# TortillasAlfred/NeuralBarkCalculator

Hardware: AMD Instinct MI355X
Metric: 1024x1024 images/sec (whole node) + per-pixel label match vs CPU ref (higher is better)
Workload: dtype f16x2

## Files before the change

### include/nbc.h

```cpp
#ifndef NBC_H
#define NBC_H

#include <stddef.h>
#include <stdint.h>

#ifdef __cplusplus
extern "C" {
#endif

typedef struct nbc_ctx nbc_ctx;

enum {
  NBC_OK = 0,
  NBC_ERR_INVALID = -1,
  NBC_ERR_KEYS = -2,
  NBC_ERR_HIP = -3,
  NBC_ERR_STATE = -4,
  NBC_ERR_NOMEM = -5
};

enum {
  NBC_PREC_FP32 = 0,
  NBC_PREC_BF16 = 1,
  NBC_PREC_F16X2 = 2
};

enum {
  NBC_PACK_ROW_CLAMPED = 1,
  NBC_PACK_SCALE_RANGE = 2
};

enum {
  NBC_ARCH_FCN_RESNET50 = 0,
  NBC_ARCH_DEEPLABV3_RESNET50 = 1,
  NBC_ARCH_FCN_EFFICIENTNET_B0 = 16,
  NBC_ARCH_DEEPLABV3_EFFICIENTNET_B0 = 24
};

enum {
  NBC_BN_RUNNING = 0,
  NBC_BN_PER_IMAGE = 1
};

enum {
  NBC_IN_F32_NCHW = 0,
  NBC_IN_U8_NHWC = 1
};

enum {
  NBC_LABEL_U8 = 0,
  NBC_LABEL_I64 = 1
};

typedef struct {
  const char* name;
  const void* data;
  int64_t shape[4];
  int32_t ndim;
  int32_t dtype;
} nbc_tensor;

typedef struct {
  char name[64];
  char bn[64];
  int32_t cin, cout, k, stride, pad, dil;
  int32_t relu, bias, residual;
} nbc_conv_desc;

typedef struct {
  int32_t kind;
  int32_t pad_before;
  int32_t pad_after;
  int32_t act;
  int32_t cin_pad, cout_pad;
  int32_t block;
  int32_t in_swish;
  float eps;
} nbc_conv_ext;

typedef struct {
  char name[64];
  char kernel[32];
  float ms;
  int32_t calls;
  double flops;
  double bytes;
  int32_t kh, kw;
  int32_t cout;
  int32_t launches;
} nbc_op_record;

const char* nbc_last_error(void);
const char* nbc_version(void);

int nbc_num_convs(void);
int nbc_conv_info(int index, nbc_conv_desc* out);
int nbc_num_state_keys(void);
int nbc_state_key(int index, const char** name, int64_t shape[4], int32_t* ndim, int32_t* dtype);
int nbc_arch_num_convs(int arch);
int nbc_arch_conv_info(int arch, int index, nbc_conv_desc* out);
int nbc_arch_num_state_keys(int arch);
int nbc_arch_state_key(int arch, int index, const char** name, int64_t shape[4], int32_t* ndim, int32_t* dtype);
int nbc_arch_of_state_dict(const nbc_tensor* tensors, int n);
int nbc_lowres_size(int H, int W, int* h, int* w);
int nbc_arch_lowres_size(int arch, int H, int W, int* h, int* w);
int nbc_arch_conv_ext(int arch, int index, nbc_conv_ext* out);

int nbc_split_f16x2(const float* x, size_t n, uint16_t* h0, uint16_t* h1);

size_t nbc_packed_weights_bytes(int precision);
int nbc_pack_weights(const nbc_tensor* tensors, int n, int precision, void* blob, size_t blob_bytes);
int nbc_packed_weights_flags(const void* blob, size_t blob_bytes, int precision);
size_t nbc_arch_packed_weights_bytes(int precision, int arch);
int nbc_pack_weights_arch(const nbc_tensor* tensors, int n, int precision, int arch, void* blob, size_t blob_bytes);
int nbc_packed_weights_flags_arch(const void* blob, size_t blob_bytes, int precision, int arch);
int nbc_packed_weights_arch(const void* blob, size_t blob_bytes, int precision);

size_t nbc_arch_bn_affine_floats(int arch);
int nbc_pack_bn_affine(const nbc_tensor* tensors, int n, int arch, float* out, size_t count);

int nbc_create(nbc_ctx** out, int hip_device);
int nbc_destroy(nbc_ctx* ctx);
int nbc_attach_weights(nbc_ctx* ctx, const void* dev_blob, size_t bytes, int precision);
int nbc_attach_weights_arch(nbc_ctx* ctx, const void* dev_blob, size_t bytes, int precision, int arch);
int nbc_load_weights(nbc_ctx* ctx, const nbc_tensor* tensors, int n, int precision);
int nbc_load_weights_arch(nbc_ctx* ctx, const nbc_tensor* tensors, int n, int precision, int arch);
int nbc_weights_flags(nbc_ctx* ctx);
int nbc_activation_exponent(nbc_ctx* ctx, const char* name, int32_t* exponent);
int nbc_bcast_weights(nbc_ctx* ctx, void* rccl_comm, int root, int precision, void* hip_stream);
int nbc_attach_bn_affine(nbc_ctx* ctx, const float* dev_affine, size_t count);
int nbc_set_bn_statistics(nbc_ctx* ctx, int mode);
int nbc_set_normalization(nbc_ctx* ctx, const float mean[3], const float std[3]);
int nbc_reserve(nbc_ctx* ctx, int N, int H, int W);

int nbc_forward(nbc_ctx* ctx, const void* x_dev, int x_dtype, int N, int H, int W,
                float* logits_lowres_dev, float* logits_full_dev,
                void* labels_dev, int labels_dtype, int64_t* counts_dev,
                int exclude_nodes, void* hip_stream);

int nbc_upsample_argmax(nbc_ctx* ctx, const float* logits_lowres_dev, int N, int h, int w, int H, int W,
                        float* logits_full_dev, void* labels_dev, int labels_dtype,
                        int64_t* counts_dev, int exclude_nodes, void* hip_stream);

int nbc_remove_small_zones(nbc_ctx* ctx, void* labels_dev, int labels_dtype, int N, int H, int W, int min_pixels,
                           int exclude_nodes, int64_t* counts_dev, void* hip_stream);

int nbc_confusion(const void* labels_dev, int labels_dtype, const uint8_t* target_dev,
                  int N, int H, int W, int64_t* conf_dev, void* hip_stream);

int nbc_image_moments(const uint8_t* x_dev, int N, int H, int W, uint64_t* moments_dev, void* hip_stream);

int nbc_target_counts(const uint8_t* target_dev, int N, int H, int W, int64_t* counts_dev, void* hip_stream);

size_t nbc_lovasz_workspace_bytes(int N, int H, int W);
int nbc_lovasz_softmax(const float* logits_full_dev, const uint8_t* target_dev, int N, int H, int W,
                       void* workspace_dev, size_t workspace_bytes, double* terms_dev, int64_t* fg_counts_dev,
                       void* hip_stream);

size_t nbc_pixel_ce_workspace_bytes(int N, int H, int W);
int nbc_pixel_cross_entropy(const float* logits_full_dev, const uint8_t* target_dev, int N, int H, int W,
                            void* workspace_dev, size_t workspace_bytes, double* sums_dev, int64_t* counts_dev,
                            void* hip_stream);


int nbc_dropout_mask(uint64_t seed, uint64_t image_id, int draw, double p, uint64_t first_element, size_t count,
                     uint8_t* keep_host);
size_t nbc_dropout_workspace_bytes(int N, int H, int W, int draws_per_pass);
int nbc_dropout_draws(nbc_ctx* ctx, int N, int H, int W, const uint64_t* image_ids_host, double p, uint64_t seed,
                      int first_draw, int draws, int min_pixels, int exclude_nodes, float* logits_lowres_dev,
                      int64_t* counts_dev, void* workspace_dev, size_t workspace_bytes, void* hip_stream);

int nbc_resize_cubic_u8(nbc_ctx* ctx, const uint8_t* src_dev, int H, int W, float* dst_dev, int out_h, int out_w,
                        void* hip_stream);
int nbc_preprocess_u8(nbc_ctx* ctx, const uint8_t* src_dev, int H, int W, uint8_t* dst_u8_dev, int32_t* row_lit_dev,
                      int out_h, int out_w, void* hip_stream);

int nbc_set_conv_tile(nbc_ctx* ctx, int tile);

int nbc_autotune(nbc_ctx* ctx, const void* x_dev, int x_dtype, int N, int H, int W, int reps, int objective,
                 void* hip_stream);
int nbc_get_plan_tiles(nbc_ctx* ctx, int32_t* tiles, int capacity);
int nbc_default_conv_tile(int M, int Cout, int K, int precision);
int nbc_set_plan_tiles(nbc_ctx* ctx, const int32_t* tiles, int n);

int nbc_nonfinite_seen(nbc_ctx* ctx, int reset);
int nbc_nonfinite_peek_async(nbc_ctx* ctx, uint32_t* host_dst, void* hip_stream);

int nbc_set_keep_activations(nbc_ctx* ctx, int on);
int nbc_activation_peaks(nbc_ctx* ctx, float* peaks_host, int capacity);
int nbc_read_activation(nbc_ctx* ctx, const char* name, float* dst_host, size_t capacity,
                        int64_t shape[4]);
int nbc_set_profiling(nbc_ctx* ctx, int on);
int nbc_num_op_records(nbc_ctx* ctx);
int nbc_get_op_record(nbc_ctx* ctx, int index, nbc_op_record* out);

#ifdef __cplusplus
}
#endif
#endif
```

### neuralbarkcalculator_amd/_lib.py

```python
from __future__ import annotations

import ctypes as C
import os
from typing import Optional

_PKG = os.path.dirname(os.path.abspath(__file__))
LIB_PATH = os.path.join(_PKG, "libnbc_hip.so")

NBC_OK = 0
NBC_ERR_INVALID, NBC_ERR_KEYS, NBC_ERR_HIP, NBC_ERR_STATE, NBC_ERR_NOMEM = -1, -2, -3, -4, -5
PREC_FP32, PREC_BF16, PREC_F16X2 = 0, 1, 2
IN_F32_NCHW, IN_U8_NHWC = 0, 1
LABEL_U8, LABEL_I64 = 0, 1
PACK_ROW_CLAMPED, PACK_SCALE_RANGE = 1, 2
ARCH_FCN_RESNET50, ARCH_DEEPLABV3_RESNET50 = 0, 1
ARCH_FCN_EFFICIENTNET_B0, ARCH_DEEPLABV3_EFFICIENTNET_B0 = 16, 24
BN_RUNNING, BN_PER_IMAGE = 0, 1


class NbcTensor(C.Structure):
    _fields_ = [("name", C.c_char_p), ("data", C.c_void_p), ("shape", C.c_int64 * 4),
                ("ndim", C.c_int32), ("dtype", C.c_int32)]


class NbcConvDesc(C.Structure):
    _fields_ = [("name", C.c_char * 64), ("bn", C.c_char * 64),
                ("cin", C.c_int32), ("cout", C.c_int32), ("k", C.c_int32), ("stride", C.c_int32),
                ("pad", C.c_int32), ("dil", C.c_int32),
                ("relu", C.c_int32), ("bias", C.c_int32), ("residual", C.c_int32)]


class NbcConvExt(C.Structure):
    _fields_ = [("kind", C.c_int32), ("pad_before", C.c_int32), ("pad_after", C.c_int32), ("act", C.c_int32),
                ("cin_pad", C.c_int32), ("cout_pad", C.c_int32), ("block", C.c_int32), ("in_swish", C.c_int32),
                ("eps", C.c_float)]


class NbcOpRecord(C.Structure):
    _fields_ = [("name", C.c_char * 64), ("kernel", C.c_char * 32), ("ms", C.c_float), ("calls", C.c_int32),
                ("flops", C.c_double), ("bytes", C.c_double), ("kh", C.c_int32), ("kw", C.c_int32),
                ("cout", C.c_int32), ("launches", C.c_int32)]


SIGNATURES = {
    "nbc_last_error": (C.c_char_p, []),
    "nbc_version": (C.c_char_p, []),
    "nbc_num_convs": (C.c_int, []),
    "nbc_conv_info": (C.c_int, [C.c_int, C.POINTER(NbcConvDesc)]),
    "nbc_num_state_keys": (C.c_int, []),
    "nbc_state_key": (C.c_int, [C.c_int, C.POINTER(C.c_char_p), C.POINTER(C.c_int64 * 4),
                                C.POINTER(C.c_int32), C.POINTER(C.c_int32)]),
    "nbc_arch_num_convs": (C.c_int, [C.c_int]),
    "nbc_arch_conv_info": (C.c_int, [C.c_int, C.c_int, C.POINTER(NbcConvDesc)]),
    "nbc_arch_num_state_keys": (C.c_int, [C.c_int]),
    "nbc_arch_state_key": (C.c_int, [C.c_int, C.c_int, C.POINTER(C.c_char_p), C.POINTER(C.c_int64 * 4),
                                     C.POINTER(C.c_int32), C.POINTER(C.c_int32)]),
    "nbc_arch_of_state_dict": (C.c_int, [C.POINTER(NbcTensor), C.c_int]),
    "nbc_lowres_size": (C.c_int, [C.c_int, C.c_int, C.POINTER(C.c_int), C.POINTER(C.c_int)]),
    "nbc_arch_lowres_size": (C.c_int, [C.c_int, C.c_int, C.c_int, C.POINTER(C.c_int), C.POINTER(C.c_int)]),
    "nbc_arch_conv_ext": (C.c_int, [C.c_int, C.c_int, C.POINTER(NbcConvExt)]),
    "nbc_packed_weights_bytes": (C.c_size_t, [C.c_int]),
    "nbc_split_f16x2": (C.c_int, [C.c_void_p, C.c_size_t, C.c_void_p, C.c_void_p]),
    "nbc_pack_weights": (C.c_int, [C.POINTER(NbcTensor), C.c_int, C.c_int, C.c_void_p, C.c_size_t]),
    "nbc_packed_weights_flags": (C.c_int, [C.c_void_p, C.c_size_t, C.c_int]),
    "nbc_arch_packed_weights_bytes": (C.c_size_t, [C.c_int, C.c_int]),
    "nbc_pack_weights_arch": (C.c_int, [C.POINTER(NbcTensor), C.c_int, C.c_int, C.c_int, C.c_void_p, C.c_size_t]),
    "nbc_packed_weights_flags_arch": (C.c_int, [C.c_void_p, C.c_size_t, C.c_int, C.c_int]),
    "nbc_packed_weights_arch": (C.c_int, [C.c_void_p, C.c_size_t, C.c_int]),
    "nbc_arch_bn_affine_floats": (C.c_size_t, [C.c_int]),
    "nbc_pack_bn_affine": (C.c_int, [C.POINTER(NbcTensor), C.c_int, C.c_int, C.c_void_p, C.c_size_t]),
    "nbc_attach_bn_affine": (C.c_int, [C.c_void_p, C.c_void_p, C.c_size_t]),
    "nbc_set_bn_statistics": (C.c_int, [C.c_void_p, C.c_int]),
    "nbc_weights_flags": (C.c_int, [C.c_void_p]),
    "nbc_activation_exponent": (C.c_int, [C.c_void_p, C.c_char_p, C.POINTER(C.c_int32)]),
    "nbc_create": (C.c_int, [C.POINTER(C.c_void_p), C.c_int]),
    "nbc_destroy": (C.c_int, [C.c_void_p]),
    "nbc_attach_weights": (C.c_int, [C.c_void_p, C.c_void_p, C.c_size_t, C.c_int]),
    "nbc_load_weights": (C.c_int, [C.c_void_p, C.POINTER(NbcTensor), C.c_int, C.c_int]),
    "nbc_attach_weights_arch": (C.c_int, [C.c_void_p, C.c_void_p, C.c_size_t, C.c_int, C.c_int]),
    "nbc_load_weights_arch": (C.c_int, [C.c_void_p, C.POINTER(NbcTensor), C.c_int, C.c_int, C.c_int]),
    "nbc_set_normalization": (C.c_int, [C.c_void_p, C.POINTER(C.c_float), C.POINTER(C.c_float)]),
    "nbc_reserve": (C.c_int, [C.c_void_p, C.c_int, C.c_int, C.c_int]),
    "nbc_nonfinite_seen": (C.c_int, [C.c_void_p, C.c_int]),
    "nbc_nonfinite_peek_async": (C.c_int, [C.c_void_p, C.c_void_p, C.c_void_p]),
    "nbc_forward": (C.c_int, [C.c_void_p, C.c_void_p, C.c_int, C.c_int, C.c_int, C.c_int,
                              C.c_void_p, C.c_void_p, C.c_void_p, C.c_int, C.c_void_p, C.c_int,
                              C.c_void_p]),
    "nbc_upsample_argmax": (C.c_int, [C.c_void_p, C.c_void_p, C.c_int, C.c_int, C.c_int, C.c_int, C.c_int,
                                      C.c_void_p, C.c_void_p, C.c_int, C.c_void_p, C.c_int, C.c_void_p]),
    "nbc_remove_small_zones": (C.c_int, [C.c_void_p, C.c_void_p, C.c_int, C.c_int, C.c_int, C.c_int, C.c_int, C.c_int,
                                         C.c_void_p, C.c_void_p]),
    "nbc_confusion": (C.c_int, [C.c_void_p, C.c_int, C.c_void_p, C.c_int, C.c_int, C.c_int, C.c_void_p, C.c_void_p]),
    "nbc_image_moments": (C.c_int, [C.c_void_p, C.c_int, C.c_int, C.c_int, C.c_void_p, C.c_void_p]),
    "nbc_target_counts": (C.c_int, [C.c_void_p, C.c_int, C.c_int, C.c_int, C.c_void_p, C.c_void_p]),
    "nbc_lovasz_workspace_bytes": (C.c_size_t, [C.c_int, C.c_int, C.c_int]),
    "nbc_lovasz_softmax": (C.c_int, [C.c_void_p, C.c_void_p, C.c_int, C.c_int, C.c_int, C.c_void_p, C.c_size_t, C.c_void_p,
                                     C.c_void_p, C.c_void_p]),
    "nbc_pixel_ce_workspace_bytes": (C.c_size_t, [C.c_int, C.c_int, C.c_int]),
    "nbc_pixel_cross_entropy": (C.c_int, [C.c_void_p, C.c_void_p, C.c_int, C.c_int, C.c_int, C.c_void_p, C.c_size_t, C.c_void_p,
                                          C.c_void_p, C.c_void_p]),
    "nbc_dropout_mask": (C.c_int, [C.c_uint64, C.c_uint64, C.c_int, C.c_double, C.c_uint64, C.c_size_t, C.c_void_p]),
    "nbc_dropout_workspace_bytes": (C.c_size_t, [C.c_int, C.c_int, C.c_int, C.c_int]),
    "nbc_dropout_draws": (C.c_int, [C.c_void_p, C.c_int, C.c_int, C.c_int, C.c_void_p, C.c_double, C.c_uint64, C.c_int, C.c_int,
                                    C.c_int, C.c_int, C.c_void_p, C.c_void_p, C.c_void_p, C.c_size_t, C.c_void_p]),
    "nbc_resize_cubic_u8": (C.c_int, [C.c_void_p, C.c_void_p, C.c_int, C.c_int, C.c_void_p, C.c_int, C.c_int, C.c_void_p]),
    "nbc_preprocess_u8": (C.c_int, [C.c_void_p, C.c_void_p, C.c_int, C.c_int, C.c_void_p, C.c_void_p, C.c_int, C.c_int,
                                    C.c_void_p]),
    "nbc_autotune": (C.c_int, [C.c_void_p, C.c_void_p, C.c_int, C.c_int, C.c_int, C.c_int, C.c_int, C.c_int,
                               C.c_void_p]),
    "nbc_get_plan_tiles": (C.c_int, [C.c_void_p, C.POINTER(C.c_int32), C.c_int]),
    "nbc_set_plan_tiles": (C.c_int, [C.c_void_p, C.POINTER(C.c_int32), C.c_int]),
    "nbc_default_conv_tile": (C.c_int, [C.c_int, C.c_int, C.c_int, C.c_int]),
    "nbc_bcast_weights": (C.c_int, [C.c_void_p, C.c_void_p, C.c_int, C.c_int, C.c_void_p]),
    "nbc_set_conv_tile": (C.c_int, [C.c_void_p, C.c_int]),
    "nbc_set_keep_activations": (C.c_int, [C.c_void_p, C.c_int]),
    "nbc_activation_peaks": (C.c_int, [C.c_void_p, C.POINTER(C.c_float), C.c_int]),
    "nbc_read_activation": (C.c_int, [C.c_void_p, C.c_char_p, C.c_void_p, C.c_size_t,
                                      C.POINTER(C.c_int64 * 4)]),
    "nbc_set_profiling": (C.c_int, [C.c_void_p, C.c_int]),
    "nbc_num_op_records": (C.c_int, [C.c_void_p]),
    "nbc_get_op_record": (C.c_int, [C.c_void_p, C.c_int, C.POINTER(NbcOpRecord)]),
}

_lib: Optional[C.CDLL] = None


def load() -> C.CDLL:
    global _lib
    if _lib is not None:
        return _lib
    if not os.path.exists(LIB_PATH):
        raise RuntimeError(
            f"{LIB_PATH} is missing: the HIP library is the only implementation of this path. "
            "Build it with `python -m neuralbarkcalculator_amd.build` (needs hipcc).")
    lib = C.CDLL(LIB_PATH)
    for name, (res, args) in SIGNATURES.items():
        fn = getattr(lib, name)
        fn.restype = res
        fn.argtypes = args
    _lib = lib
    return lib


def last_error() -> str:
    return load().nbc_last_error().decode("utf-8", "replace")


def check(rc: int, what: str = "") -> None:
    if rc == NBC_OK:
        return
    msg = last_error()
    raise RuntimeError(f"{what + ': ' if what else ''}{msg} (nbc error {rc})")
```

### neuralbarkcalculator_amd/build.py

```python
from __future__ import annotations

import os
import shutil
import subprocess
import sys
from concurrent.futures import ThreadPoolExecutor

PKG = os.path.dirname(os.path.abspath(__file__))
CSRC = os.path.join(PKG, "csrc")
OBJ = os.path.join(CSRC, "_obj")
LIB = os.path.join(PKG, "libnbc_hip.so")
SOURCES = ["nbc_net.cpp", "nbc_plan.cpp", "conv_igemm_dma.hip", "conv3x3_rows.hip", "pointwise.hip", "small_zones.hip", "nbc_api.hip", "confusion.hip",
           "aspp.hip", "bn_stats.hip", "efficientnet.hip", "lovasz.hip", "dataset_stats.hip", "pixel_ce.hip", "dropout_head.hip"]
ARCH = "gfx950"


def _hipcc() -> str:
    exe = shutil.which("hipcc") or "/opt/rocm/bin/hipcc"
    if not os.path.exists(exe):
        raise RuntimeError("hipcc not found: cannot build libnbc_hip.so")
    return exe


def _deps_newer(target: str, deps) -> bool:
    if not os.path.exists(target):
        return True
    t = os.path.getmtime(target)
    return any(os.path.getmtime(d) > t for d in deps)


def build(force: bool = False, verbose: bool = True) -> str:
    os.makedirs(OBJ, exist_ok=True)
    hipcc = _hipcc()
    headers = [os.path.join(CSRC, f) for f in os.listdir(CSRC) if f.endswith(".hpp")]
    headers.append(os.path.join(os.path.dirname(PKG), "include", "nbc.h"))
    common = ["-O3", "-std=c++17", "-fPIC", f"--offload-arch={ARCH}", "-Wall", "-Wno-unused-function"]

    def compile_one(src: str) -> str:
        path = os.path.join(CSRC, src)
        obj = os.path.join(OBJ, src + ".o")
        if force or _deps_newer(obj, [path] + headers):
            cmd = [hipcc] + common + (["-x", "hip"] if src.endswith(".hip") else ["-ffp-contract=off"]) + ["-c", path, "-o", obj]
            if verbose:
                print("[nbc build]", " ".join(cmd), flush=True)
            subprocess.run(cmd, check=True)
        return obj

    with ThreadPoolExecutor(max_workers=6) as ex:
        objs = list(ex.map(compile_one, SOURCES))
    if force or _deps_newer(LIB, objs):
        cmd = [hipcc, "-shared", "-fPIC", f"--offload-arch={ARCH}", "-o", LIB] + objs
        if verbose:
            print("[nbc build]", " ".join(cmd), flush=True)
        subprocess.run(cmd, check=True)
    return LIB


if __name__ == "__main__":
    print(build(force="--force" in sys.argv))
```

### neuralbarkcalculator_amd/csrc/conv_igemm_dma.hip

```cpp
#include <atomic>

#include "nbc_kernels.hpp"
#include "split16.hpp"

namespace nbc {
namespace {

typedef __attribute__((ext_vector_type(8))) __bf16 bf16x8;
typedef __attribute__((ext_vector_type(16))) float f32x16;
typedef __attribute__((ext_vector_type(4))) float f32x4;

__device__ __forceinline__ int lds_off(int row, int chunk) {
  return row * 128 + ((chunk ^ ((row >> 1) & 7)) << 4);
}
__device__ __forceinline__ float bf16_bits_to_f32(unsigned short b) {
  return __builtin_bit_cast(float, (unsigned)b << 16);
}
__device__ __forceinline__ unsigned short f32_to_bf16_bits(float f) {
  __bf16 b = (__bf16)f;
  return __builtin_bit_cast(unsigned short, b);
}

__device__ __forceinline__ void dma16(const void* gsrc, unsigned lds_base) {
  unsigned keep;
  asm volatile(
      "s_mov_b32 %0, m0\n\t"
      "s_mov_b32 m0, %2\n\t"
      "s_nop 0\n\t"
      "global_load_lds_dwordx4 %1, off\n\t"
      "s_mov_b32 m0, %0"
      : "=&s"(keep)
      : "v"(gsrc), "s"(lds_base)
      : "memory");
}

typedef __amdgpu_buffer_rsrc_t rsrc_t;
constexpr unsigned kOutOfRange = 0x80000000u;
__device__ __forceinline__ void dma16_buf(unsigned voff, rsrc_t rsrc, unsigned lds_base, unsigned soff) {
  asm volatile(
      "s_mov_b32 m0, %2\n\t"
      "s_nop 0\n\t"
      "buffer_load_dwordx4 %0, %1, %3 offen lds"
      :
      : "v"(voff), "s"(rsrc), "s"(lds_base), "s"(soff)
      : "memory");
}

#ifdef NBC_STAMPS
#define NBC_STAMP(i)                                                                                   \
  do {                                                                                                 \
    if (p.stamps && threadIdx.x == 0) p.stamps[(size_t)blockIdx.x * 64 + (i)] = __builtin_amdgcn_s_memrealtime(); \
  } while (0)
#define NBC_STAMP_CLK(i)                                                                               \
  do {                                                                                                 \
    if (p.stamps && threadIdx.x == 0) p.stamps[(size_t)blockIdx.x * 64 + (i)] = __builtin_amdgcn_s_memtime(); \
  } while (0)
#define NBC_WAIT_COUNTERS() unsigned long long st_vm = 0, st_bar = 0
#define NBC_WAIT_BEGIN() const unsigned long long st0 = __builtin_amdgcn_s_memtime()
#define NBC_WAIT_MID() const unsigned long long st1 = __builtin_amdgcn_s_memtime()
#define NBC_WAIT_END(count)                                                                            \
  do {                                                                                                 \
    if (count) { st_vm += st1 - st0; st_bar += __builtin_amdgcn_s_memtime() - st1; }                  \
  } while (0)
#define NBC_STAMP_WAVE_WAITS()                                                                         \
  do {                                                                                                 \
    if (p.stamps && lane == 0) { p.stamps[(size_t)blockIdx.x * 64 + 16 + wave] = st_vm; p.stamps[(size_t)blockIdx.x * 64 + 32 + wave] = st_bar; } \
  } while (0)
#define NBC_STAMP_BLOCK_END()                                                                          \
  do {                                                                                                 \
    NBC_STAMP(5);                                                          \
    wait_vmcnt<0>();                                                                                   \
    NBC_STAMP(6);                                                    \
    if (p.stamps && threadIdx.x == 0)                       \
      p.stamps[(size_t)blockIdx.x * 64 + 7] =                                                          \
          ((unsigned long long)__builtin_amdgcn_s_getreg(20 | (31 << 11)) << 32) | __builtin_amdgcn_s_getreg(4 | (31 << 11)); \
  } while (0)
#else
#define NBC_STAMP(i) do { } while (0)
#define NBC_STAMP_CLK(i) do { } while (0)
#define NBC_WAIT_COUNTERS()
#define NBC_WAIT_BEGIN()
#define NBC_WAIT_MID()
#define NBC_WAIT_END(count) do { } while (0)
#define NBC_STAMP_WAVE_WAITS() do { } while (0)
#define NBC_STAMP_BLOCK_END() do { } while (0)
#endif

template <int N>
__device__ __forceinline__ void wait_vmcnt() {
  asm volatile("s_waitcnt vmcnt(%0)" ::"n"(N) : "memory");
}

constexpr int ring_bytes(int prec, int wm, int wn, int mt, int nt, int s) {
  const int ring = s * (wm * mt * 32 + wn * nt * 32) * 128;
  const int scratch = wm * wn * 32 * (nt * 32 * 4 + 16);
  return ring > scratch ? ring : scratch;
}
constexpr int min_waves_per_simd(int prec, int wm, int wn, int mt, int nt, int s) {
  return (wm * wn >= 8 && (wm * wn >= 16 || ring_bytes(prec, wm, wn, mt, nt, s) + 2048 <= 80 * 1024)) ? 4 : 2;
}

constexpr int kVarDefault = 0;
constexpr int kVarBf16Mfma32 = 1;
constexpr int kVarLoaderWaves = 8;

typedef unsigned nt_u32x4 __attribute__((ext_vector_type(4)));
constexpr int loader_waves(int var) { return var == kVarLoaderWaves ? 4 : 0; }
template <int PREC, int WM, int WN, int MT, int NT, int S, bool STEM, int VAR, bool BIGW>
__global__ __launch_bounds__((WM * WN + loader_waves(VAR)) * 64, VAR == kVarLoaderWaves ? (WM * WN + loader_waves(VAR)) / 4 : min_waves_per_simd(PREC, WM, WN, MT, NT, S)) void conv_dma_kernel(const ConvArgs p) {
  extern __shared__ __attribute__((aligned(16))) unsigned char smem[];
  constexpr int EB = PREC == 1 ? 2 : 4;
  constexpr bool X2 = (PREC == 2);
  constexpr int CW = WM * WN;
  constexpr int LW = loader_waves(VAR);
  constexpr bool SPEC = LW > 0;
  constexpr int THREADS = (SPEC ? LW : CW) * 64;
  constexpr int BM = WM * MT * 32;
  constexpr int BN = WN * NT * 32;
  constexpr int A_BYTES = BM * 128;
  constexpr int B_BYTES = BN * 128;
  constexpr int STAGE_BYTES = A_BYTES + B_BYTES;
  constexpr int TABLE_OFF = ring_bytes(PREC, WM, WN, MT, NT, S);
  constexpr int ROWS_PER_PASS = THREADS / 8;
  constexpr int A_PASSES = BM / ROWS_PER_PASS;
  constexpr int B_PASSES = BN / ROWS_PER_PASS;
  constexpr int L = A_PASSES + B_PASSES;
  static_assert(BM % ROWS_PER_PASS == 0 && BN % ROWS_PER_PASS == 0, "tile rows must fill whole passes");
  static_assert(S >= 2 && S <= 4, "2..4 LDS stages");

  const int tid = threadIdx.x;
  const int lane = tid & 63;
  const int wave = __builtin_amdgcn_readfirstlane(tid >> 6);
  const bool is_loader = SPEC && wave >= CW;
  const bool loads = !SPEC || is_loader, computes = !SPEC || !is_loader;
  constexpr bool STAGGER = (PREC == 2) && !STEM && CW >= 8 && (LW > 0 || MT * NT >= 4);
  const bool late_half = STAGGER && wave >= CW / 2 && wave < CW;
  NBC_STAMP(0);

  const int tiles_n = p.Co / BN;
  const int tiles_m = (p.M + BM - 1) / BM;
  const int nblk = tiles_m * tiles_n;
  int bid = blockIdx.x;
  {
    const int q = nblk >> 3, rr = nblk & 7, xcd = bid & 7;
    bid = (xcd < rr ? xcd * (q + 1) : rr * (q + 1) + (xcd - rr) * q) + (bid >> 3);
  }
  int tile_n = bid % tiles_n, tile_m = bid / tiles_n;
  if (BIGW && (tiles_n & 1) == 0 && (tiles_m & 3) == 0) {
    const int xcd = blockIdx.x & 7, li = blockIdx.x >> 3, rows = tiles_m >> 2, hc = tiles_n >> 1;
    tile_m = (xcd >> 1) * rows + li / hc;
    tile_n = (xcd & 1) * hc + li % hc;
  }
  const int m0 = tile_m * BM;
  const int n0 = tile_n * BN;

  const int ltid = SPEC ? ((tid - CW * 64) & (THREADS - 1)) : tid;
  const int ps = ltid & 7;
  const int lr = ltid >> 3;
  const rsrc_t xrsrc = __builtin_amdgcn_make_buffer_rsrc(const_cast<void*>(p.x), 0, p.x_bytes, 0x00020000);
  const rsrc_t wrsrc = __builtin_amdgcn_make_buffer_rsrc(const_cast<void*>(p.w), 0, p.w_bytes, 0x00020000);
  const int pix_bytes = p.Ci * EB;
  const unsigned wrow_bytes = (unsigned)p.ksteps * 128u;

  int a_iy0[A_PASSES], a_ix0[A_PASSES], a_img[A_PASSES], a_coff[A_PASSES];
  {
    const int hw = p.Ho * p.Wo;
#pragma unroll
    for (int i = 0; i < A_PASSES; ++i) {
      const int row = lr + ROWS_PER_PASS * i;
      const int m = m0 + row;
      a_coff[i] = (ps ^ ((row >> 1) & 7)) * 16;
      if (m < p.M) {
        const int img = p.N == 1 ? 0 : (p.hw_shift >= 0 ? (m >> p.hw_shift) : m / hw);
        const int rem = m - img * hw;
        const int oy = p.wo_shift >= 0 ? (rem >> p.wo_shift) : rem / p.Wo;
        const int ox = rem - oy * p.Wo;
        a_iy0[i] = oy * p.stride - p.pad;
        a_ix0[i] = ox * p.stride - p.pad;
        a_img[i] = img * p.Hi * p.Wi;
      } else {
        a_iy0[i] = -(1 << 24);
        a_ix0[i] = 0;
        a_img[i] = 0;
      }
    }
  }
  unsigned w_off[B_PASSES];
#pragma unroll
  for (int i = 0; i < B_PASSES; ++i) {
    const int row = lr + ROWS_PER_PASS * i;
    w_off[i] = (unsigned)(n0 + row) * wrow_bytes + (unsigned)(ps ^ ((row >> 1) & 7)) * 16u;
  }

  typedef __attribute__((address_space(3))) unsigned char lds_u8;
  const unsigned smem_base = (unsigned)(size_t)(lds_u8*)smem;
  const unsigned wave_off = (unsigned)(SPEC ? ((wave - CW) & (LW - 1)) : wave) * 1024u;
  const int cblocks = STEM ? 1 : pix_bytes / 128;
  int ld_kh = 0, ld_kw = 0, ld_cb = 0;
  int st_kh = 0, st_kw = 0;
  if constexpr (STEM) st_kw = a_coff[0] >> 4;

  unsigned a_off[A_PASSES];
  auto set_tap = [&](int kh, int kw) __attribute__((always_inline)) {
    const int dy = kh * p.dil, dx = kw * p.dil;
#pragma unroll
    for (int i = 0; i < A_PASSES; ++i) {
      const int iy = a_iy0[i] + dy, ix = a_ix0[i] + dx;
      const bool ok = (unsigned)iy < (unsigned)p.Hi && (unsigned)ix < (unsigned)p.Wi;
      const unsigned off = (unsigned)(a_img[i] + iy * p.Wi + ix) * (unsigned)pix_bytes + (unsigned)a_coff[i];
      a_off[i] = ok ? off : kOutOfRange;
    }
  };
  if constexpr (!STEM) set_tap(0, 0);

  auto issue_one = [&](int d, int t, unsigned sa) __attribute__((always_inline)) {
    if (d < A_PASSES) {
      const int i = d;
      if constexpr (!STEM) {
        dma16_buf(a_off[i], xrsrc, sa + (unsigned)(ROWS_PER_PASS * 128 * i), (unsigned)ld_cb * 128u);
      } else {
        const int iy = a_iy0[i] + st_kh * p.dil, ix = a_ix0[i] + st_kw * p.dil;
        const bool ok = st_kw < p.KW && (unsigned)iy < (unsigned)p.Hi && (unsigned)ix < (unsigned)p.Wi;
        const unsigned off = (unsigned)(a_img[i] + iy * p.Wi + ix) * 16u;
        dma16_buf(ok ? off : kOutOfRange, xrsrc, sa + (unsigned)(ROWS_PER_PASS * 128 * i), 0u);
      }
    } else {
      const int i = d - A_PASSES;
      dma16_buf(w_off[i], wrsrc, sa + (unsigned)(A_BYTES + ROWS_PER_PASS * 128 * i), (unsigned)t * 128u);
    }
  };
  auto issue_part = [&](int part, int t, int stage) __attribute__((always_inline)) {
    const unsigned sa = smem_base + (unsigned)stage * STAGE_BYTES + wave_off;
#pragma unroll
    for (int d = 0; d < L; ++d)
      if (d * 4 / L == part) issue_one(d, t, sa);
    if constexpr (STEM) {
      if (part == 3) ++st_kh;
    }
    if constexpr (!STEM) {
      if (part == 3) {
        if (++ld_cb == cblocks) {
          ld_cb = 0;
          if (++ld_kw == p.KW) { ld_kw = 0; ++ld_kh; }
          if (ld_kh < p.KH) set_tap(ld_kh, ld_kw);
        }
      }
    }
  };
  auto issue_step = [&](int t, int stage) __attribute__((always_inline)) {
#pragma unroll
    for (int part = 0; part < 4; ++part) issue_part(part, t, stage);
  };

  const int r = lane & 31, h = lane >> 5;
  const int wm = wave % WM, wn = wave / WM;
  constexpr bool M16 = (PREC == 1 && VAR == kVarDefault) || X2;
  constexpr int MT16 = 2 * MT, NT16 = 2 * NT;
  const int r16 = lane & 15, q16 = lane >> 4;
  constexpr bool F32 = (PREC == 0);
  constexpr bool PREFETCH = F32 && S >= 3;
  f32x16 acc[M16 ? 1 : NT][M16 ? 1 : MT];
  f32x16 accI[F32 ? NT : 1][F32 ? MT : 1];
  f32x4 acc16[M16 ? NT16 : 1][M16 ? MT16 : 1];
  f32x4 accI2[X2 ? NT16 : 1][X2 ? MT16 : 1];
  if constexpr (X2) {
#pragma unroll
    for (int j = 0; j < NT16; ++j)
#pragma unroll
      for (int i = 0; i < MT16; ++i)
#pragma unroll
        for (int e = 0; e < 4; ++e) accI2[j][i][e] = 0.f;
  }
  if constexpr (M16) {
#pragma unroll
    for (int j = 0; j < NT16; ++j)
#pragma unroll
      for (int i = 0; i < MT16; ++i)
#pragma unroll
        for (int e = 0; e < 4; ++e) acc16[j][i][e] = 0.f;
  } else {
#pragma unroll
    for (int j = 0; j < NT; ++j)
#pragma unroll
      for (int i = 0; i < MT; ++i)
#pragma unroll
        for (int e = 0; e < 16; ++e) acc[j][i][e] = 0.f;
  }

  NBC_WAIT_COUNTERS();
  uint4 fpf[F32 ? 2 : 1][F32 ? MT : 1], fwf[F32 ? 2 : 1][F32 ? NT : 1];
  auto load_frags32 = [&](int stage, int ks, uint4 (&pfr)[F32 ? MT : 1], uint4 (&wfr)[F32 ? NT : 1]) __attribute__((always_inline)) {
    if constexpr (F32) {
      const unsigned char* sa = smem + stage * STAGE_BYTES;
      const unsigned char* sb = sa + A_BYTES;
      const int chunk = 2 * ks + h;
#pragma unroll
      for (int i = 0; i < MT; ++i)
        pfr[i] = *reinterpret_cast<const uint4*>(sa + lds_off((wm * MT + i) * 32 + r, chunk));
#pragma unroll
      for (int j = 0; j < NT; ++j)
        wfr[j] = *reinterpret_cast<const uint4*>(sb + lds_off((wn * NT + j) * 32 + r, chunk));
    }
  };
  constexpr int NTILES = NT * MT;
  constexpr int FLUSH = 8;
  const bool late = WM * WN >= 8 && wave >= WM * WN / 2;
  if constexpr (F32) {
#pragma unroll
    for (int n = 0; n < NTILES; ++n)
#pragma unroll
      for (int e = 0; e < 16; ++e) accI[n / MT][n % MT][e] = 0.f;
  }
  auto compute32 = [&](bool flush, int stage, bool more, bool all_issued, int next_stage, bool do_issue, int t_issue, int issue_stage)
      __attribute__((always_inline)) {
    if constexpr (F32) {
      if constexpr (!PREFETCH) load_frags32(stage, 0, fpf[0], fwf[0]);
      if (flush) {
#pragma unroll
        for (int n = 0; n < NTILES; ++n) {
          acc[n / MT][n % MT] += accI[n / MT][n % MT];
#pragma unroll
          for (int e = 0; e < 16; ++e) accI[n / MT][n % MT][e] = 0.f;
        }
      }
#pragma unroll
      for (int ks = 0; ks < 4; ++ks) {
        if (PREFETCH && ks == 2 && more) {
          NBC_WAIT_BEGIN();
          if (S > 3 && all_issued) wait_vmcnt<(S - 3) * L>();
          else wait_vmcnt<0>();
          NBC_WAIT_MID();
          __builtin_amdgcn_s_barrier();
          NBC_WAIT_END(true);
        }
        if (ks + 1 < 4) load_frags32(stage, ks + 1, fpf[(ks + 1) & 1], fwf[(ks + 1) & 1]);
        else if (PREFETCH && more) load_frags32(next_stage, 0, fpf[0], fwf[0]);
#pragma unroll
        for (int n = 0; n < NTILES; ++n) {
          const int j = n / MT, i = n % MT;
          const float4 wv = __builtin_bit_cast(float4, fwf[ks & 1][j]);
          const float4 pv = __builtin_bit_cast(float4, fpf[ks & 1][i]);
          accI[j][i] = __builtin_amdgcn_mfma_f32_32x32x2f32(wv.x, pv.x, accI[j][i], 0, 0, 0);
          accI[j][i] = __builtin_amdgcn_mfma_f32_32x32x2f32(wv.y, pv.y, accI[j][i], 0, 0, 0);
          accI[j][i] = __builtin_amdgcn_mfma_f32_32x32x2f32(wv.z, pv.z, accI[j][i], 0, 0, 0);
          accI[j][i] = __builtin_amdgcn_mfma_f32_32x32x2f32(wv.w, pv.w, accI[j][i], 0, 0, 0);
          if (PREFETCH && ks >= 2 && do_issue && (ks == 3) == late) {
#pragma unroll
            for (int part = 0; part < 4; ++part)
              if (part * NTILES / 4 == n) issue_part(part, t_issue, issue_stage);
          }
        }
      }
    }
  };
  auto step32 = [&](int t, int stage, bool more, bool all_issued, int next_stage, bool do_issue, int t_issue, int issue_stage)
      __attribute__((always_inline)) {
    compute32(t > 0 && (t & (FLUSH - 1)) == 0, stage, more, all_issued, next_stage, do_issue, t_issue, issue_stage);
  };

  constexpr bool X2F = X2 && !STEM;
  constexpr int XM = X2F ? MT16 : 1, XN = X2F ? NT16 : 1;
  constexpr bool X2_STAG = STAGGER;
  uint4 sp0[X2_STAG ? XM : 1], sp1[X2_STAG ? XM : 1], sw0[X2_STAG ? XN : 1], sw1[X2_STAG ? XN : 1];
  auto x2_flush = [&](int t) __attribute__((always_inline)) {
    if constexpr (X2) {
      if (t > 0 && (t & 7) == 0) {
#pragma unroll
        for (int n = 0; n < NT16 * MT16; ++n) {
          acc16[n / MT16][n % MT16] += accI2[n / MT16][n % MT16];
#pragma unroll
          for (int e = 0; e < 4; ++e) accI2[n / MT16][n % MT16][e] = 0.f;
        }
      }
    }
  };
  auto x2_read = [&](int stage, uint4 (&xp0)[XM], uint4 (&xp1)[XM], uint4 (&xw0)[XN], uint4 (&xw1)[XN]) __attribute__((always_inline)) {
    if constexpr (X2F) {
      const unsigned char* sa = smem + stage * STAGE_BYTES;
      const unsigned char* sb = sa + A_BYTES;
#pragma unroll
      for (int i = 0; i < MT16; ++i) {
        xp0[i] = *reinterpret_cast<const uint4*>(sa + lds_off(wm * MT * 32 + i * 16 + r16, q16));
        xp1[i] = *reinterpret_cast<const uint4*>(sa + lds_off(wm * MT * 32 + i * 16 + r16, 4 + q16));
      }
#pragma unroll
      for (int j = 0; j < NT16; ++j) {
        xw0[j] = *reinterpret_cast<const uint4*>(sb + lds_off(wn * NT * 32 + j * 16 + r16, q16));
        xw1[j] = *reinterpret_cast<const uint4*>(sb + lds_off(wn * NT * 32 + j * 16 + r16, 4 + q16));
      }
    }
  };
  auto x2_mfma = [&](int t, bool do_issue, int t_issue, int issue_stage, uint4 (&xp0)[XM], uint4 (&xp1)[XM], uint4 (&xw0)[XN], uint4 (&xw1)[XN])
      __attribute__((always_inline)) {
    if constexpr (X2F) {
      constexpr int NTI = NT16 * MT16;
      const f16x8 kLow = {kH1UnscaleH, kH1UnscaleH, kH1UnscaleH, kH1UnscaleH, kH1UnscaleH, kH1UnscaleH, kH1UnscaleH, kH1UnscaleH};
#pragma unroll
      for (int idx = 0; idx < 3 * NTI; ++idx) {
        const int prod = idx / NTI, n = idx % NTI, j = n / MT16, i = n % MT16;
        if (prod == 0)
          accI2[j][i] = __builtin_amdgcn_mfma_f32_16x16x32_f16(__builtin_bit_cast(f16x8, xw0[j]), __builtin_bit_cast(f16x8, xp0[i]), accI2[j][i], 0, 0, 0);
        else if (prod == 1)
          accI2[j][i] = __builtin_amdgcn_mfma_f32_16x16x32_f16(__builtin_bit_cast(f16x8, xw1[j]), __builtin_bit_cast(f16x8, xp0[i]), accI2[j][i], 0, 0, 0);
        else {
          if (i == 0) xw0[j] = __builtin_bit_cast(uint4, __builtin_bit_cast(f16x8, xw0[j]) * kLow);
          accI2[j][i] = __builtin_amdgcn_mfma_f32_16x16x32_f16(__builtin_bit_cast(f16x8, xw0[j]), __builtin_bit_cast(f16x8, xp1[i]), accI2[j][i], 0, 0, 0);
        }
        if (do_issue && (idx + 1) % (3 * NTI / 4) == 0) issue_part((idx + 1) / (3 * NTI / 4) - 1, t_issue, issue_stage);
      }
    }
  };

  auto compute = [&](int t, int stage, bool do_issue, int t_issue, int issue_stage) __attribute__((always_inline)) {
    const unsigned char* sa = smem + stage * STAGE_BYTES;
    const unsigned char* sb = sa + A_BYTES;
    if constexpr (X2) {
      constexpr int NTI = NT16 * MT16;
      if constexpr (!STEM) {
        uint4 p0[XM], p1[XM], w0[XN], w1[XN];
        x2_flush(t);
        x2_read(stage, p0, p1, w0, w1);
        x2_mfma(t, do_issue, t_issue, issue_stage, p0, p1, w0, w1);
      } else {
        x2_flush(t);
        const f16x8 kLow = {kH1UnscaleH, kH1UnscaleH, kH1UnscaleH, kH1UnscaleH, kH1UnscaleH, kH1UnscaleH, kH1UnscaleH, kH1UnscaleH};
#pragma unroll
        for (int half = 0; half < 2; ++half) {
          uint4 px[MT16], wa[NT16], wb[NT16];
#pragma unroll
          for (int i = 0; i < MT16; ++i) px[i] = *reinterpret_cast<const uint4*>(sa + lds_off(wm * MT * 32 + i * 16 + r16, 4 * half + q16));
#pragma unroll
          for (int j = 0; j < NT16; ++j) {
            const uint4 wv = *reinterpret_cast<const uint4*>(sb + lds_off(wn * NT * 32 + j * 16 + r16, 4 * half + q16));
            const uint4 lo = __builtin_bit_cast(uint4, __builtin_bit_cast(f16x8, wv) * kLow);
            wa[j] = make_uint4(wv.x, wv.y, lo.x, lo.y);
            wb[j] = make_uint4(wv.z, wv.w, 0u, 0u);
          }
#pragma unroll
          for (int idx = 0; idx < 2 * NTI; ++idx) {
            const int prod = idx / NTI, n = idx % NTI, j = n / MT16, i = n % MT16;
            accI2[j][i] = __builtin_amdgcn_mfma_f32_16x16x32_f16(__builtin_bit_cast(f16x8, prod == 0 ? wa[j] : wb[j]), __builtin_bit_cast(f16x8, px[i]), accI2[j][i], 0, 0, 0);
            if (do_issue && (idx + 1) % NTI == 0) issue_part(2 * half + (idx + 1) / NTI - 1, t_issue, issue_stage);
          }
        }
      }
      return;
    }
    if constexpr (M16) {
      constexpr bool DBUF = (MT16 + NT16) * 8 <= 64;
      uint4 pf[DBUF ? 2 : 1][MT16], wf[DBUF ? 2 : 1][NT16];
      auto load_half = [&](int half, uint4 (&pfr)[MT16], uint4 (&wfr)[NT16]) {
        const int chunk = 4 * half + q16;
#pragma unroll
        for (int i = 0; i < MT16; ++i)
          pfr[i] = *reinterpret_cast<const uint4*>(sa + lds_off(wm * MT * 32 + i * 16 + r16, chunk));
#pragma unroll
        for (int j = 0; j < NT16; ++j)
          wfr[j] = *reinterpret_cast<const uint4*>(sb + lds_off(wn * NT * 32 + j * 16 + r16, chunk));
      };
      load_half(0, pf[0], wf[0]);
#pragma unroll
      for (int half = 0; half < 2; ++half) {
        const int cur = DBUF ? half : 0;
        if (DBUF && half == 0) load_half(1, pf[DBUF ? 1 : 0], wf[DBUF ? 1 : 0]);
#pragma unroll
        for (int sub = 0; sub < 2; ++sub) {
#pragma unroll
          for (int j = sub * NT16 / 2; j < (sub + 1) * NT16 / 2; ++j)
#pragma unroll
            for (int i = 0; i < MT16; ++i)
              acc16[j][i] = __builtin_amdgcn_mfma_f32_16x16x32_bf16(
                  __builtin_bit_cast(bf16x8, wf[cur][j]), __builtin_bit_cast(bf16x8, pf[cur][i]), acc16[j][i], 0, 0, 0);
          if (do_issue) issue_part(2 * half + sub, t_issue, issue_stage);
        }
        if (!DBUF && half == 0) load_half(1, pf[0], wf[0]);
      }
      return;
    }
    uint4 pf[2][MT], wf[2][NT];
    auto load_frags = [&](int ks, uint4 (&pfr)[MT], uint4 (&wfr)[NT]) {
      const int chunk = 2 * ks + h;
#pragma unroll
      for (int i = 0; i < MT; ++i)
        pfr[i] = *reinterpret_cast<const uint4*>(sa + lds_off((wm * MT + i) * 32 + r, chunk));
#pragma unroll
      for (int j = 0; j < NT; ++j)
        wfr[j] = *reinterpret_cast<const uint4*>(sb + lds_off((wn * NT + j) * 32 + r, chunk));
    };
    load_frags(0, pf[0], wf[0]);
#pragma unroll
    for (int ks = 0; ks < 4; ++ks) {
      if (ks + 1 < 4) load_frags(ks + 1, pf[(ks + 1) & 1], wf[(ks + 1) & 1]);
#pragma unroll
      for (int j = 0; j < NT; ++j)
#pragma unroll
        for (int i = 0; i < MT; ++i) {
          acc[j][i] = __builtin_amdgcn_mfma_f32_32x32x16_bf16(
              __builtin_bit_cast(bf16x8, wf[ks & 1][j]), __builtin_bit_cast(bf16x8, pf[ks & 1][i]),
              acc[j][i], 0, 0, 0);
        }
      if (do_issue) issue_part(ks, t_issue, issue_stage);
    }
  };

  constexpr int SLAB_CH = NT * 32;
  constexpr int PITCH = SLAB_CH * 4 + 16;
  constexpr int OUT_CH = X2 ? 8 : 16 / EB;
  constexpr int CPR = SLAB_CH / OUT_CH;
  constexpr int PIX_PER_PASS = 64 / CPR;
  constexpr int PASSES = 32 / PIX_PER_PASS;
  constexpr bool RES_PREFETCH = (MT * PASSES <= 16) && !(PREC == 1 && VAR == kVarDefault && MT * NT >= 8) && !X2;
  static_assert(WM * WN * 32 * PITCH <= TABLE_OFF, "epilogue scratch must fit below the scale/shift table");
  const int o_pix = lane / CPR, o_chunk = lane % CPR;
  const int n_slab = n0 + wn * SLAB_CH;
  const unsigned row_bytes = (unsigned)p.Co * EB;
  const size_t tile_off = ((size_t)m0 * p.Co + n_slab) * EB;
  unsigned char* ytile = static_cast<unsigned char*>(p.y) + tile_off;
  const unsigned char* rtile = p.res ? static_cast<const unsigned char*>(p.res) + tile_off : nullptr;
  const int rows_valid = p.M - m0;
  const int row0 = wm * MT * 32 + o_pix;
  const unsigned lane_chunk = X2 ? (unsigned)(o_chunk >> 2) * 128u + (unsigned)(o_chunk & 3) * 16u : (unsigned)o_chunk * 16u;
  uint4 rpre[RES_PREFETCH ? MT : 1][RES_PREFETCH ? PASSES : 1];
  constexpr bool RES_PREFETCH2 = X2 && MT * PASSES * 2 <= 16;
  uint4 rpre2[RES_PREFETCH2 ? MT : 1][RES_PREFETCH2 ? PASSES : 1][2];

  const int T = p.ksteps;
  auto prefetch_identity = [&]() {
    if constexpr (RES_PREFETCH) {
      if (rtile) {
#pragma unroll
        for (int i = 0; i < MT; ++i)
#pragma unroll
          for (int ps2 = 0; ps2 < PASSES; ++ps2) {
            int row = row0 + i * 32 + ps2 * PIX_PER_PASS;
            row = row < rows_valid ? row : rows_valid - 1;
            rpre[i][ps2] = *reinterpret_cast<const uint4*>(rtile + ((unsigned)row * row_bytes + lane_chunk));
          }
      }
    }
  };

  NBC_STAMP(8);
  if (wave == (SPEC ? CW : 0) && lane < BN / 4) {
    dma16(p.scale + n0 + lane * 4, smem_base + (unsigned)TABLE_OFF);
    dma16(p.shift + n0 + lane * 4, smem_base + (unsigned)TABLE_OFF + 1024u);
  }
  if (loads) {
#pragma unroll
    for (int s = 0; s < S - 1; ++s)
      if (s < T) issue_step(s, s);
  }
  NBC_STAMP(1);
  if constexpr (PREFETCH) {
    if (S - 2 < T) wait_vmcnt<(S - 2) * L>();
    else wait_vmcnt<0>();
    __builtin_amdgcn_s_barrier();
    load_frags32(0, 0, fpf[0], fwf[0]);
    NBC_STAMP(2); NBC_STAMP_CLK(11);
    for (int t = 0; t < T - 1; ++t)
      step32(t, t % S, true, t + S - 2 < T, (t + 1) % S, t + S - 1 < T, t + S - 1, (t + S - 1) % S);
    NBC_STAMP(3);
    NBC_STAMP_CLK(12);
    NBC_STAMP_WAVE_WAITS();
    prefetch_identity();
    step32(T - 1, (T - 1) % S, false, false, 0, false, 0, 0);
  } else {
  auto loop_top = [&](int t) __attribute__((always_inline)) {
    NBC_WAIT_BEGIN();
    if (t + (S - 2) < T) wait_vmcnt<(S - 2) * L>();
    else wait_vmcnt<0>();
    NBC_WAIT_MID();
    __builtin_amdgcn_s_barrier();
    NBC_WAIT_END(t > 0);
    if (t == 0) { NBC_STAMP(2); NBC_STAMP_CLK(11); }
  };
  if constexpr (STAGGER) {
    if (is_loader) {
      for (int t = 0; t < T - 1; ++t) {
        loop_top(t);
        if (t + S - 1 < T) issue_step(t + S - 1, (t + S - 1) % S);
      }
    } else if (!late_half) {
      for (int t = 0; t < T - 1; ++t) {
        loop_top(t);
        if constexpr (!SPEC && S == 2) { if (t + S - 1 < T) issue_step(t + S - 1, (t + S - 1) % S); }
        x2_flush(t);
        x2_read(t % S, sp0, sp1, sw0, sw1);
        x2_mfma(t, !SPEC && S > 2 && t + S - 1 < T, t + S - 1, (t + S - 1) % S, sp0, sp1, sw0, sw1);
      }
    } else {
      if constexpr (MT * NT >= 2) __builtin_amdgcn_s_setprio(1);
      if (T > 1) {
        loop_top(0);
        if constexpr (!SPEC) { if (S - 1 < T) issue_step(S - 1, (S - 1) % S); }
        x2_read(0, sp0, sp1, sw0, sw1);
        asm volatile("s_waitcnt lgkmcnt(0)" ::: "memory");
      }
      for (int t = 1; t < T - 1; ++t) {
        loop_top(t);
        if constexpr (!SPEC && S == 2) { if (t + S - 1 < T) issue_step(t + S - 1, (t + S - 1) % S); }
        x2_flush(t - 1);
        x2_mfma(t - 1, !SPEC && S > 2 && t + S - 1 < T, t + S - 1, (t + S - 1) % S, sp0, sp1, sw0, sw1);
        x2_read(t % S, sp0, sp1, sw0, sw1);
        asm volatile("s_waitcnt lgkmcnt(0)" ::: "memory");
      }
      if constexpr (MT * NT >= 2) __builtin_amdgcn_s_setprio(0);
    }
  } else {
  for (int t = 0; t < T - 1; ++t) {
    loop_top(t);
    if constexpr (SPEC) {
      if (is_loader) { if (t + S - 1 < T) issue_step(t + S - 1, (t + S - 1) % S); }
      else compute(t, t % S, false, 0, 0);
    } else if constexpr (S == 2) {
      if (t + S - 1 < T) issue_step(t + S - 1, (t + S - 1) % S);
      if constexpr (F32) step32(t, t % S, false, false, 0, false, 0, 0);
      else compute(t, t % S, false, 0, 0);
    } else {
      compute(t, t % S, t + S - 1 < T, t + S - 1, (t + S - 1) % S);
    }
  }
  }
  wait_vmcnt<0>();
  __builtin_amdgcn_s_barrier();
  NBC_STAMP(3);
  NBC_STAMP_CLK(12);
  NBC_STAMP_WAVE_WAITS();
  if (computes) prefetch_identity();
  if constexpr (F32) step32(T - 1, (T - 1) % S, false, false, 0, false, 0, 0);
  else if constexpr (STAGGER) {
    if (computes) {
      if (late_half && T > 1) { x2_flush(T - 2); x2_mfma(T - 2, false, 0, 0, sp0, sp1, sw0, sw1); }
      x2_flush(T - 1);
      x2_read((T - 1) % S, sp0, sp1, sw0, sw1);
      x2_mfma(T - 1, false, 0, 0, sp0, sp1, sw0, sw1);
    }
  } else if (computes) compute(T - 1, (T - 1) % S, false, 0, 0);
  }
  if constexpr (RES_PREFETCH2) {
    if (rtile && computes) {
#pragma unroll
      for (int i = 0; i < MT; ++i)
#pragma unroll
        for (int ps2 = 0; ps2 < PASSES; ++ps2) {
          int row = row0 + i * 32 + ps2 * PIX_PER_PASS;
          row = row < rows_valid ? row : rows_valid - 1;
          const unsigned char* rp = rtile + ((unsigned)row * row_bytes + lane_chunk);
          if constexpr (BIGW) {
            rpre2[i][ps2][0] = __builtin_bit_cast(uint4, __builtin_nontemporal_load(reinterpret_cast<const nt_u32x4*>(rp)));
            rpre2[i][ps2][1] = __builtin_bit_cast(uint4, __builtin_nontemporal_load(reinterpret_cast<const nt_u32x4*>(rp + 64)));
          } else {
            rpre2[i][ps2][0] = *reinterpret_cast<const uint4*>(rp);
            rpre2[i][ps2][1] = *reinterpret_cast<const uint4*>(rp + 64);
          }
        }
    }
  }

  if constexpr (F32) {
#pragma unroll
    for (int n = 0; n < NTILES; ++n) acc[n / MT][n % MT] += accI[n / MT][n % MT];
  }
  if constexpr (X2) {
#pragma unroll
    for (int n = 0; n < NT16 * MT16; ++n) acc16[n / MT16][n % MT16] += accI2[n / MT16][n % MT16];
  }

  __syncthreads();
  if (!computes) return;
  NBC_STAMP(4);
  unsigned char* scr = smem + wave * (32 * PITCH);
  const unsigned char* table = smem + TABLE_OFF + wn * SLAB_CH * 4;
  const bool relu = p.relu != 0;
  typedef __attribute__((ext_vector_type(2))) float f32x2;
  typedef __attribute__((ext_vector_type(2))) __bf16 bf16x2;
#pragma unroll
  for (int i = 0; i < MT; ++i) {
    if constexpr (M16) {
#pragma unroll
      for (int j0 = 0; j0 < NT16; j0 += 4) {
        float4 sc[4], sh[4];
#pragma unroll
        for (int jj = 0; jj < 4 && j0 + jj < NT16; ++jj) {
          const int nl = (j0 + jj) * 16 + 4 * q16;
          sc[jj] = *reinterpret_cast<const float4*>(table + nl * 4);
          sh[jj] = *reinterpret_cast<const float4*>(table + 1024 + nl * 4);
        }
#pragma unroll
        for (int i2 = 0; i2 < 2; ++i2)
#pragma unroll
          for (int jj = 0; jj < 4 && j0 + jj < NT16; ++jj) {
            const int nl = (j0 + jj) * 16 + 4 * q16;
            const f32x4 a = acc16[j0 + jj][2 * i + i2];
            float4 v;
            v.x = __builtin_fmaf(a[0], sc[jj].x, sh[jj].x);
            v.y = __builtin_fmaf(a[1], sc[jj].y, sh[jj].y);
            v.z = __builtin_fmaf(a[2], sc[jj].z, sh[jj].z);
            v.w = __builtin_fmaf(a[3], sc[jj].w, sh[jj].w);
            *reinterpret_cast<float4*>(scr + (i2 * 16 + r16) * PITCH + nl * 4) = v;
          }
      }
    } else {
#pragma unroll
      for (int j = 0; j < NT; ++j) {
        float4 sc[4], sh[4];
#pragma unroll
        for (int g = 0; g < 4; ++g) {
          const int nl = j * 32 + 8 * g + 4 * h;
          sc[g] = *reinterpret_cast<const float4*>(table + nl * 4);
          sh[g] = *reinterpret_cast<const float4*>(table + 1024 + nl * 4);
        }
#pragma unroll
        for (int g = 0; g < 4; ++g) {
          const int nl = j * 32 + 8 * g + 4 * h;
          float4 v;
          v.x = __builtin_fmaf(acc[j][i][4 * g + 0], sc[g].x, sh[g].x);
          v.y = __builtin_fmaf(acc[j][i][4 * g + 1], sc[g].y, sh[g].y);
          v.z = __builtin_fmaf(acc[j][i][4 * g + 2], sc[g].z, sh[g].z);
          v.w = __builtin_fmaf(acc[j][i][4 * g + 3], sc[g].w, sh[g].w);
          *reinterpret_cast<float4*>(scr + r * PITCH + nl * 4) = v;
        }
      }
    }
    if (i == 0) NBC_STAMP(9);
    float v[PASSES][OUT_CH];
#pragma unroll
    for (int ps2 = 0; ps2 < PASSES; ++ps2) {
      const float4* sp = reinterpret_cast<const float4*>(scr + (ps2 * PIX_PER_PASS + o_pix) * PITCH + o_chunk * OUT_CH * 4);
#pragma unroll
      for (int q = 0; q < OUT_CH / 4; ++q) {
        const float4 t4 = sp[q];
        v[ps2][4 * q] = t4.x; v[ps2][4 * q + 1] = t4.y; v[ps2][4 * q + 2] = t4.z; v[ps2][4 * q + 3] = t4.w;
      }
    }
#pragma unroll
    for (int ps2 = 0; ps2 < PASSES; ++ps2) {
      const int row = row0 + i * 32 + ps2 * PIX_PER_PASS;
      const unsigned loff = (unsigned)row * row_bytes + lane_chunk;
      if constexpr (X2) {
        if (rtile) {
          float idv[8];
          if constexpr (RES_PREFETCH2) {
            join16x8(rpre2[i][ps2][0], rpre2[i][ps2][1], idv);
          } else {
            const unsigned char* rp = rtile + ((unsigned)(row < rows_valid ? row : rows_valid - 1) * row_bytes + lane_chunk);
            join16x8(*reinterpret_cast<const uint4*>(rp), *reinterpret_cast<const uint4*>(rp + 64), idv);
          }
#pragma unroll
          for (int q = 0; q < 8; ++q) v[ps2][q] += idv[q];
        }
      } else if (rtile) {
        uint4 rv;
        if constexpr (RES_PREFETCH) rv = rpre[i][ps2];
        else rv = *reinterpret_cast<const uint4*>(rtile + ((unsigned)(row < rows_valid ? row : rows_valid - 1) * row_bytes + lane_chunk));
        const unsigned u[4] = {rv.x, rv.y, rv.z, rv.w};
        if constexpr (PREC == 0) {
#pragma unroll
          for (int q = 0; q < 4; ++q) v[ps2][q] += __builtin_bit_cast(float, u[q]);
        } else {
#pragma unroll
          for (int q = 0; q < 4; ++q) {
            v[ps2][2 * q] += __builtin_bit_cast(float, u[q] << 16);
            v[ps2][2 * q + 1] += __builtin_bit_cast(float, u[q] & 0xffff0000u);
          }
        }
      }
      if (relu) {
#pragma unroll
        for (int e = 0; e < OUT_CH; ++e) v[ps2][e] = __builtin_elementwise_maximum(v[ps2][e], 0.f);
      }
      uint4 o;
      if constexpr (X2) {
        uint4 o1;
        split16x8(v[ps2], o, o1);
        if (row < rows_valid) *reinterpret_cast<uint4*>(ytile + loff + 64) = o1;
      } else if constexpr (PREC == 0) {
        o.x = __builtin_bit_cast(unsigned, v[ps2][0]); o.y = __builtin_bit_cast(unsigned, v[ps2][1]);
        o.z = __builtin_bit_cast(unsigned, v[ps2][2]); o.w = __builtin_bit_cast(unsigned, v[ps2][3]);
      } else {
        unsigned pk[4];
#pragma unroll
        for (int q = 0; q < 4; ++q) {
          const f32x2 pr = {v[ps2][(2 * q) % OUT_CH], v[ps2][(2 * q + 1) % OUT_CH]};
          pk[q] = __builtin_bit_cast(unsigned, __builtin_convertvector(pr, bf16x2));
        }
        o.x = pk[0]; o.y = pk[1]; o.z = pk[2]; o.w = pk[3];
      }
      if (row < rows_valid) *reinterpret_cast<uint4*>(ytile + loff) = o;
    }
    if (i == 0) NBC_STAMP(10);
  }
  NBC_STAMP_BLOCK_END();
}

template <int PREC, int WM, int WN, int MT, int NT, int S, bool STEM, int VAR = kVarDefault, bool BIGW = false>
hipError_t launch_cfg(const ConvArgs& a, hipStream_t s) {
  constexpr int BM = WM * MT * 32, BN = WN * NT * 32;
  constexpr int smem = ring_bytes(PREC, WM, WN, MT, NT, S) + 2048;
  static std::atomic<unsigned long long> attr_done{0};
  auto kern = &conv_dma_kernel<PREC, WM, WN, MT, NT, S, STEM, VAR, BIGW>;
  int dev = 0;
  if (hipGetDevice(&dev) != hipSuccess || dev < 0 || dev > 63) return hipErrorInvalidDevice;
  if (!((attr_done.load(std::memory_order_acquire) >> dev) & 1ull)) {
    hipError_t e = hipFuncSetAttribute(reinterpret_cast<const void*>(kern),
                                       hipFuncAttributeMaxDynamicSharedMemorySize, smem);
    if (e != hipSuccess) return e;
    attr_done.fetch_or(1ull << dev, std::memory_order_release);
  }
  if (a.Co % BN != 0) return hipErrorInvalidValue;
  const int tiles = ((a.M + BM - 1) / BM) * (a.Co / BN);
  hipLaunchKernelGGL(kern, dim3(tiles), dim3((WM * WN + loader_waves(VAR)) * 64), smem, s, a);
  return hipGetLastError();
}

template <int PREC, bool STEM, int VAR>
hipError_t launch_tile(const ConvArgs& a, int tile, hipStream_t s) {
  if constexpr (PREC == 2) {
    if constexpr (!STEM) {
      if (a.res != nullptr && a.w_bytes >= (3u << 20)) {
        if (tile == 17) return launch_cfg<PREC, 2, 4, 2, 1, 2, false, VAR, true>(a, s);
        if (tile == 1) return launch_cfg<PREC, 2, 2, 2, 2, 2, false, VAR, true>(a, s);
        if (tile == 14) return launch_cfg<PREC, 2, 4, 2, 1, 3, false, kVarLoaderWaves, true>(a, s);
      }
    }
    switch (tile) {
      case 0: return launch_cfg<PREC, 2, 2, 2, 1, 3, STEM, VAR>(a, s);
      case 1: return launch_cfg<PREC, 2, 2, 2, 2, 2, STEM, VAR>(a, s);
      case 5: return launch_cfg<PREC, 2, 4, 2, 2, 3, STEM, VAR>(a, s);
      case 16: return launch_cfg<PREC, 2, 2, 2, 2, 3, STEM, STEM ? VAR : kVarLoaderWaves>(a, s);
      case 17: return launch_cfg<PREC, 2, 4, 2, 1, 2, STEM, VAR>(a, s);
      case 6: return launch_cfg<PREC, 4, 2, 2, 1, 3, STEM, VAR>(a, s);
      case 7: return launch_cfg<PREC, 2, 2, 2, 1, 2, STEM, VAR>(a, s);
      case 8: return launch_cfg<PREC, 1, 4, 2, 1, 2, STEM, VAR>(a, s);
      case 9: return launch_cfg<PREC, 4, 2, 1, 2, 3, STEM, VAR>(a, s);
      case 10: return launch_cfg<PREC, 4, 2, 1, 1, 3, STEM, VAR>(a, s);
      case 13: return launch_cfg<PREC, 2, 4, 2, 1, 3, STEM, VAR>(a, s);
      case 14: return launch_cfg<PREC, 2, 4, 2, 1, 3, STEM, STEM ? VAR : kVarLoaderWaves>(a, s);
      case 15: return launch_cfg<PREC, 4, 2, 1, 1, 3, STEM, STEM ? VAR : kVarLoaderWaves>(a, s);
      default: return hipErrorInvalidValue;
    }
  } else
  switch (tile) {
    case 0: return launch_cfg<PREC, 2, 2, 2, 1, 3, STEM, VAR>(a, s);
    case 1: return launch_cfg<PREC, 2, 2, 2, 2, 2, STEM, VAR>(a, s);
    case 2: return launch_cfg<PREC, 4, 2, 2, 2, 3, STEM, VAR>(a, s);
    case 3:
      if constexpr (PREC == 0) return hipErrorInvalidValue;
      else return launch_cfg<PREC, 2, 4, 4, 2, 2, STEM, VAR>(a, s);
    case 4: return launch_cfg<PREC, 2, 2, 2, 2, 4, STEM, VAR>(a, s);
    case 5: return launch_cfg<PREC, 2, 4, 2, 2, 3, STEM, VAR>(a, s);
    case 6: return launch_cfg<PREC, 4, 2, 2, 1, 3, STEM, VAR>(a, s);
    case 7: return launch_cfg<PREC, 2, 2, 2, 1, 2, STEM, VAR>(a, s);
    case 8: return launch_cfg<PREC, 1, 4, 2, 1, 2, STEM, VAR>(a, s);
    case 9: return launch_cfg<PREC, 4, 2, 1, 2, PREC == 0 ? 3 : 2, STEM, VAR>(a, s);
    case 10: return launch_cfg<PREC, 4, 2, 1, 1, PREC == 0 ? 3 : 2, STEM, VAR>(a, s);
    case 11: return launch_cfg<PREC, 4, 4, 2, 1, 2, STEM, VAR>(a, s);
    case 12:
      if constexpr (PREC == 0) return hipErrorInvalidValue;
      else return launch_cfg<PREC, 4, 4, 2, 2, 2, STEM, VAR>(a, s);
    case 13: return launch_cfg<PREC, 2, 4, 2, 1, 3, STEM, VAR>(a, s);
    default: return hipErrorInvalidValue;
  }
}

constexpr int kTileRows[CONV_TILE_COUNT] = {128, 128, 256, 256, 128, 128, 256, 128, 64, 128, 128, 256, 256, 128, 128, 128, 128, 128, 128, 128, 256};
constexpr int kTileCols[CONV_TILE_COUNT] = {64, 128, 128, 256, 128, 256, 64, 64, 128, 128, 64, 128, 256, 128, 128, 64, 128, 128, 128, 64, 64};

}

int conv_tile_rows(int tile) { return tile >= 0 && tile < CONV_TILE_COUNT ? kTileRows[tile] : 0; }
int conv_tile_cols(int tile) { return tile >= 0 && tile < CONV_TILE_COUNT ? kTileCols[tile] : 0; }

bool conv_tile_ok(int precision, int tile, int Co, int rows_kind) {
  if (tile < 0 || tile >= CONV_TILE_COUNT) return false;
  const int tile_kind = tile < CONV_TILE_ROWS_FIRST ? 0 : tile == 19 ? 2 : 1;
  if (rows_kind != tile_kind) return false;
  if (rows_kind != 0) return precision == 2 && Co % kTileCols[tile] == 0;
  if (precision == 0 && (tile == 3 || tile == 12)) return false;
  if (precision == 2 && (tile == 2 || tile == 3 || tile == 4 || tile == 11 || tile == 12)) return false;
  if (precision != 2 && tile >= 14) return false;
  return Co % kTileCols[tile] == 0;
}

namespace {
struct TileModel {
  double cu_flops_per_us;
  double eff[CONV_TILE_COUNT], eff1[CONV_TILE_COUNT], ovh_us[CONV_TILE_COUNT], cb[CONV_TILE_COUNT];
  int cap[CONV_TILE_COUNT];
};
constexpr TileModel kTileModel[3] = {
    {157.3e6 / 256.0,
     {0.85, 0.85, 0.85, 0.85, 0.85, 0.896, 0.722, 0.811, 0.894, 0.85, 0.85, 0.85, 0.85, 0.80, 0.80, 0.80, 0.80, 0.80, 0.80, 0.80, 0.80},
     {0.85, 0.85, 0.85, 0.85, 0.85, 0.896, 0.722, 0.811, 0.894, 0.85, 0.85, 0.85, 0.85, 0.80, 0.80, 0.80, 0.80, 0.80, 0.80, 0.80, 0.80},
     {4.0, 4.0, 4.0, 4.0, 4.0, 4.0, 5.08, 3.14, 0.76, 4.0, 4.0, 4.0, 4.0, 4.0, 4.0, 4.0, 4.0, 4.0, 4.0, 4.0, 4.0},
     {0, 0, 0, 0, 0, 0, 0, 0, 0, 0, 0, 0, 0, 0, 0, 0, 0, 0, 0, 0, 0},
     {1, 1, 1, 1, 1, 1, 1, 1, 1, 1, 1, 1, 1, 1, 1, 1, 1, 1, 1, 1, 1}},
    {1400.0e6 / 256.0,
     {0.888, 0.85, 0.85, 0.897, 0.85, 0.911, 0.85, 0.85, 0.85, 0.754, 0.85, 0.85, 0.85, 0.80, 0.80, 0.80, 0.80, 0.80, 0.80, 0.80, 0.80},
     {0.888, 0.85, 0.85, 0.897, 0.85, 0.911, 0.85, 0.85, 0.85, 0.754, 0.85, 0.85, 0.85, 0.80, 0.80, 0.80, 0.80, 0.80, 0.80, 0.80, 0.80},
     {1.19, 4.0, 4.0, 2.78, 4.0, 4.0, 4.0, 0.0, 4.0, 0.5, 4.0, 4.0, 3.61, 4.0, 4.0, 4.0, 4.0, 4.0, 4.0, 4.0, 4.0},
     {0.91, 1.0, 1.0, 1.07, 1.0, 0.78, 1.0, 1.03, 1.0, 0.68, 1.0, 1.0, 1.0, 1.0, 1.0, 1.0, 1.0, 1.0, 1.0, 1.0, 1.0},
     {1, 1, 1, 1, 1, 1, 1, 1, 1, 1, 1, 1, 1, 1, 1, 1, 1, 1, 1, 1, 1}},
    {839.0e6 / 256.0,
     {0.421, 0.52, 0.5, 0.5, 0.5, 0.535, 0.42, 0.476, 0.42, 0.42, 0.455, 0.5, 0.5, 0.44, 0.47, 0.4, 0.448, 0.501, 0.50, 0.45, 0.515},
     {0.38, 0.36, 0.5, 0.5, 0.5, 0.535, 0.42, 0.383, 0.36, 0.42, 0.392, 0.5, 0.5, 0.44, 0.47, 0.4, 0.448, 0.36, 0.50, 0.45, 0.515},
     {3, 3, 3, 3, 3, 3.45, 3.007, 3, 2.746, 3, 2.868, 3, 3, 2.518, 3.874, 3, 3, 3.321, 4.0, 3.0, 4.0},
     {0.3, 0.3, 0.3, 0.3, 0.3, 0.3, 0.309, 0.31, 0.272, 0.3, 0.3, 0.3, 0.3, 0.3, 0.3, 0.3, 0.3, 0.195, 0.2, 0.3, 0.2},
     {2, 2, 1, 1, 1, 1, 1, 3, 3, 1, 2, 1, 1, 1, 1, 1, 1, 2, 1, 1, 1}}};
}

int choose_conv_tile(int M, int Co, int K, int precision, int rows_kind) {
  if (precision < 0 || precision > 2) return -1;
  const TileModel& tm = kTileModel[precision];
  const double eb = precision == 1 ? 2.0 : 4.0;
  int best = -1;
  double best_cost = 0.0;
  for (int t = 0; t < CONV_TILE_COUNT; ++t) {
    if (!conv_tile_ok(precision, t, Co, rows_kind)) continue;
    const double trows = kTileRows[t], cols = kTileCols[t];
    const long long blocks = (long long)((M + kTileRows[t] - 1) / kTileRows[t]) * (Co / kTileCols[t]);
    const long long b = (blocks + 255) / 256;
    const int cap = tm.cap[t];
    const long long g = b / cap, rest = b % cap;
    const double eff_r = cap > 1 && rest > 0 ? tm.eff1[t] + (tm.eff[t] - tm.eff1[t]) * (double)(rest - 1) / (double)(cap - 1) : tm.eff[t];
    const double flops = trows * cols * 2.0 * K;
    const double prows = t == 20 ? trows / 4.0 * 1.125 : t >= CONV_TILE_ROWS_FIRST ? trows / 3.0 * 1.125 : trows;
    const double bytes = (prows + cols) * K * eb + trows * cols * eb * 2.0;
    const double cost = ((double)(g * cap) / tm.eff[t] + (double)rest / eff_r) * flops / tm.cu_flops_per_us +
                        (double)b * bytes * tm.cb[t] / 50.0e3 + (double)((b + cap - 1) / cap) * tm.ovh_us[t];
    if (best < 0 || cost < best_cost * (1.0 - 1e-9) ||
        (cost <= best_cost * (1.0 + 1e-9) && trows * cols > (double)kTileRows[best] * kTileCols[best])) {
      best = t;
      best_cost = cost;
    }
  }
  return best;
}

hipError_t launch_conv_dma(const ConvArgs& a, int precision, int tile, hipStream_t s) {
  const int eb = precision == 1 ? 2 : 4;
  if (a.M <= 0 || a.Co % 64 != 0 || a.ksteps <= 0 || a.x_bytes == 0 || a.x_bytes >= kOutOfRange || a.w_bytes == 0 ||
      a.w_bytes >= kOutOfRange)
    return hipErrorInvalidValue;
  if (a.stem) {
    if (a.Ci * eb != 16 || a.ksteps != a.KH || a.KW > 8) return hipErrorInvalidValue;
  } else {
    if ((a.Ci * eb) % 128 != 0 || a.ksteps != a.KH * a.KW * (a.Ci * eb / 128)) return hipErrorInvalidValue;
  }
  const int rows = (!a.stem && a.KW == a.KH && a.M == a.N * a.Ho * a.Wo)
                       ? conv_rows_kind(precision, a.KH, a.stride, a.pad, a.dil, a.Hi, a.Wi, a.Ho, a.Wo, a.Ci, a.Co, a.res != nullptr) : 0;
  if (tile < 0) tile = choose_conv_tile(a.M, a.Co, a.ksteps * (128 / eb), precision, rows);
  if (!conv_tile_ok(precision, tile, a.Co, rows)) return hipErrorInvalidValue;
  if (rows != 0) return launch_conv3x3_rows(a, tile - CONV_TILE_ROWS_FIRST, s);
  if (precision == 0) return a.stem ? launch_tile<0, true, kVarDefault>(a, tile, s) : launch_tile<0, false, kVarDefault>(a, tile, s);
  if (precision == 2) return a.stem ? launch_tile<2, true, kVarDefault>(a, tile, s) : launch_tile<2, false, kVarDefault>(a, tile, s);
  if (a.stem) return launch_tile<1, true, kVarDefault>(a, tile, s);
  if (a.res != nullptr) return launch_tile<1, false, kVarBf16Mfma32>(a, tile, s);
  return launch_tile<1, false, kVarDefault>(a, tile, s);
}

}
```

### neuralbarkcalculator_amd/csrc/nbc_api.hip

```cpp
#include <dlfcn.h>
#include <hip/hip_runtime.h>

#include <algorithm>
#include <cmath>
#include <cstdio>
#include <cstring>
#include <map>
#include <string>
#include <vector>

#include "../../include/nbc.h"
#include "nbc_internal.hpp"
#include "nbc_kernels.hpp"
#include "nbc_net.hpp"
#include "nbc_plan.hpp"
#include "philox.hpp"
#include "reduce.hpp"

using namespace nbc;

#define NBC_HIP(expr)                                                                         \
  do {                                                                                        \
    hipError_t _e = (expr);                                                                   \
    if (_e != hipSuccess)                                                                     \
      return set_error(NBC_ERR_HIP, std::string(#expr) + ": " + hipGetErrorString(_e));       \
  } while (0)

struct nbc_ctx {
  int device = 0;
  int precision = -1;
  int arch = kArchFcn;
  const unsigned char* weights = nullptr;
  void* owned_weights = nullptr;
  PackedLayout layout;
  float mean[3] = {0.7399f, 0.6139f, 0.4401f};
  float stdv[3] = {0.1068f, 0.1272f, 0.1271f};
  Plan plan;
  std::vector<Plan> plan_cache;
  std::vector<void*> bufs;
  std::vector<size_t> buf_cap;
  float* lowres = nullptr;
  size_t lowres_cap = 0;
  int conv_tile = -1;
  bool keep = false;
  bool profiling = false;
  std::vector<std::vector<hipEvent_t>> prof_sets;
  size_t prof_used = 0;
  std::vector<Op> prof_ops;
  int prof_arch = kArchFcn;
  std::vector<nbc_op_record> records;
  std::map<std::string, int> act_of;
  void* scratch256 = nullptr;
  int pack_flags = 0;
  std::vector<int> act_exp;
  unsigned* nonfinite = nullptr;
  void* zones_ws = nullptr;
  size_t zones_px = 0;
  int bn_mode = NBC_BN_RUNNING;
  const float* bn_affine = nullptr;
  size_t bn_affine_count = 0;
  void* owned_affine = nullptr;
  float* bn_unit = nullptr;
  void* bn_ws = nullptr;
  size_t bn_ws_cap = 0;
  bool fwd_valid = false;
  int fwd_N = 0, fwd_H = 0, fwd_W = 0;
};

namespace {

constexpr size_t kPlanCacheEntries = 64;

PlanKey plan_key(const nbc_ctx* c, int N, int H, int W) {
  PlanKey k;
  k.N = N; k.H = H; k.W = W; k.precision = c->precision; k.arch = c->arch; k.keep = c->keep; k.bn = c->bn_mode;
  return k;
}

void stash_plan(nbc_ctx* c) {
  Plan& cur = c->plan;
  c->fwd_valid = false;
  if (cur.N == 0) return;
  for (Plan& p : c->plan_cache)
    if (same_shape(p, cur)) {
      p = cur; cur = Plan(); return;
    }
  if (c->plan_cache.size() >= kPlanCacheEntries) c->plan_cache.erase(c->plan_cache.begin());
  c->plan_cache.push_back(cur);
  cur = Plan();
}

int ensure_buffers(nbc_ctx* c) {
  const Plan& P = c->plan;
  if (c->bufs.size() < P.buf_bytes.size()) { c->bufs.resize(P.buf_bytes.size(), nullptr); c->buf_cap.resize(P.buf_bytes.size(), 0); }
  for (size_t i = 0; i < P.buf_bytes.size(); ++i) {
    if (c->buf_cap[i] < P.buf_bytes[i]) {
      const size_t grown = c->buf_cap[i] + c->buf_cap[i] / 2;
      if (c->bufs[i]) NBC_HIP(hipFree(c->bufs[i]));
      c->bufs[i] = nullptr; c->buf_cap[i] = 0;
      size_t want = std::max(P.buf_bytes[i], grown);
      hipError_t e = hipMalloc(&c->bufs[i], want);
      if (e != hipSuccess && want > P.buf_bytes[i]) {
        (void)hipGetLastError();
        want = P.buf_bytes[i];
        e = hipMalloc(&c->bufs[i], want);
      }
      if (e != hipSuccess) return set_error(NBC_ERR_NOMEM, std::string("hipMalloc(workspace): ") + hipGetErrorString(e));
      c->buf_cap[i] = want;
    }
  }
  if (P.bn == NBC_BN_PER_IMAGE) {
    if (!c->bn_unit) {
      std::vector<float> unit(4096, 0.f);
      std::fill(unit.begin(), unit.begin() + 2048, 1.f);
      NBC_HIP(hipMalloc((void**)&c->bn_unit, unit.size() * sizeof(float)));
      NBC_HIP(hipMemcpy(c->bn_unit, unit.data(), unit.size() * sizeof(float), hipMemcpyHostToDevice));
    }
    if (c->bn_ws_cap < P.bn_ws_bytes) {
      if (c->bn_ws) NBC_HIP(hipFree(c->bn_ws));
      c->bn_ws = nullptr; c->bn_ws_cap = 0;
      NBC_HIP(hipMalloc(&c->bn_ws, P.bn_ws_bytes));
      c->bn_ws_cap = P.bn_ws_bytes;
    }
  }
  const size_t lr = (size_t)P.N * kNumClasses * P.h * P.w * sizeof(float);
  if (c->lowres_cap < lr) {
    if (c->lowres) NBC_HIP(hipFree(c->lowres));
    c->lowres = nullptr; c->lowres_cap = 0;
    NBC_HIP(hipMalloc((void**)&c->lowres, lr));
    c->lowres_cap = lr;
  }
  c->act_of.clear();
  for (size_t i = 0; i < P.ops.size(); ++i) c->act_of[P.ops[i].name] = (int)i;
  return NBC_OK;
}

struct UnitPtrs {
  const float* w;
  const float* scale;
  const float* shift;
};
UnitPtrs unit_ptrs(const nbc_ctx* c, int unit) {
  const PackedConv& pc = c->layout.convs[unit];
  return {reinterpret_cast<const float*>(c->weights + pc.w_off), reinterpret_cast<const float*>(c->weights + pc.scale_off),
          reinterpret_cast<const float*>(c->weights + pc.shift_off)};
}

int launch_conv_op(nbc_ctx* c, const Op& o, int N, int tile, hipStream_t s, hipError_t* err) {
  const ConvUnit& u = conv_units(c->arch)[o.unit];
  const PackedConv& pc = c->layout.convs[o.unit];
  const UnitPtrs p = unit_ptrs(c, o.unit);
  const int prec = c->precision;
  const size_t eb = elem_bytes(prec);
  ConvArgs a{};
  a.x = c->bufs[o.in_buf];
  a.w = p.w;
  a.scale = p.scale;
  a.shift = p.shift;
  a.res = o.res_buf >= 0 ? c->bufs[o.res_buf] : nullptr;
  if (o.raw) {
    if (o.Co > 2048) return set_error(NBC_ERR_STATE, "raw convolution wider than the unit table at " + o.name);
    a.scale = c->bn_unit;
    a.shift = c->bn_unit + 2048;
    a.res = nullptr;
  }
  a.y = c->bufs[o.out_buf];
  a.N = N; a.Hi = o.Hi; a.Wi = o.Wi; a.Ci = o.Ci;
  a.Ho = o.Ho; a.Wo = o.Wo; a.Co = o.Co;
  a.KH = u.k; a.KW = u.k; a.stride = u.stride; a.pad = u.pad; a.dil = u.dil;
  a.M = N * o.Ho * o.Wo;
  a.ksteps = pc.ksteps;
  a.relu = u.relu && !o.raw ? 1 : 0;
  a.stem = pc.stem ? 1 : 0;
  a.wo_shift = -1;
  a.hw_shift = -1;
  for (int sft = 0; sft < 31; ++sft) {
    if ((1 << sft) == o.Wo) a.wo_shift = sft;
    if ((1 << sft) == o.Ho * o.Wo) a.hw_shift = sft;
  }
  if (o.Ci != pc.cin_pad) return set_error(NBC_ERR_STATE, "plan/channel mismatch at " + o.name);
  const size_t xb = (size_t)N * o.Hi * o.Wi * o.Ci * eb;
  const size_t wbts = (size_t)o.Co * pc.ksteps * kKStepBytes;
  if (xb >= 0x80000000ull || wbts >= 0x80000000ull)
    return set_error(NBC_ERR_INVALID, "activation of " + o.name + " exceeds 2 GiB: lower the batch size");
  a.x_bytes = (unsigned)xb;
  a.w_bytes = (unsigned)wbts;
  if (o.gate_buf >= 0) {
    const size_t xi = (size_t)o.Hi * o.Wi * o.Ci * eb, yi = (size_t)o.Ho * o.Wo * o.Co * eb;
    a.N = 1;
    a.M = o.Ho * o.Wo;
    a.x_bytes = (unsigned)xi;
    for (int n = 0; n < N; ++n) {
      a.x = static_cast<const unsigned char*>(c->bufs[o.in_buf]) + n * xi;
      a.w = static_cast<const unsigned char*>(c->bufs[o.gate_buf]) + n * wbts;
      a.res = o.res_buf >= 0 ? static_cast<const unsigned char*>(c->bufs[o.res_buf]) + n * yi : nullptr;
      a.y = static_cast<unsigned char*>(c->bufs[o.out_buf]) + n * yi;
      *err = launch_conv_dma(a, prec, tile, s);
      if (*err != hipSuccess) break;
    }
    return NBC_OK;
  }
  *err = launch_conv_dma(a, prec, tile, s);
  return NBC_OK;
}

const char* kernel_name(OpKind k) {
  switch (k) {
    case OP_INGEST: return "ingest";
    case OP_CONV: return "conv_dma";
    case OP_MAXPOOL: return "maxpool";
    case OP_HEAD1X1: return "head1x1";
    case OP_ASPP_POOL: return "aspp_pool";
    case OP_CONCAT: return "concat";
    case OP_BN_STATS: return "bn_stats";
    case OP_BN_APPLY: return "bn_apply";
    case OP_DWCONV: return "dwconv";
    case OP_SE_EXCITE: return "se_excite";
    case OP_GATE_WEIGHTS: return "gate_weights";
    case OP_SWISH: return "swish";
    case OP_POOL_ANY: return "pool";
    default: return "upsample_argmax";
  }
}

}

extern "C" {

int nbc_create(nbc_ctx** out, int hip_device) {
  if (!out) return set_error(NBC_ERR_INVALID, "nbc_create: null out");
  int ndev = 0;
  hipError_t e = hipGetDeviceCount(&ndev);
  if (e != hipSuccess || ndev <= 0)
    return set_error(NBC_ERR_HIP, std::string("nbc_create: no HIP device (") + hipGetErrorString(e) + ")");
  if (hip_device < 0 || hip_device >= ndev) return set_error(NBC_ERR_INVALID, "nbc_create: bad device index");
  NBC_HIP(hipSetDevice(hip_device));
  hipDeviceProp_t prop;
  NBC_HIP(hipGetDeviceProperties(&prop, hip_device));
  if (std::strncmp(prop.gcnArchName, "gfx950", 6) != 0)
    return set_error(NBC_ERR_HIP, std::string("nbc_create: kernels are built for gfx950 only, device is ") + prop.gcnArchName);
  nbc_ctx* c = new nbc_ctx();
  c->device = hip_device;
  *out = c;
  return NBC_OK;
}

int nbc_destroy(nbc_ctx* c) {
  if (!c) return NBC_OK;
  (void)hipSetDevice(c->device);
  for (void* b : c->bufs) if (b) (void)hipFree(b);
  if (c->lowres) (void)hipFree(c->lowres);
  if (c->zones_ws) (void)hipFree(c->zones_ws);
  if (c->scratch256) (void)hipFree(c->scratch256);
  if (c->nonfinite) (void)hipFree(c->nonfinite);
  if (c->owned_weights) (void)hipFree(c->owned_weights);
  if (c->owned_affine) (void)hipFree(c->owned_affine);
  if (c->bn_unit) (void)hipFree(c->bn_unit);
  if (c->bn_ws) (void)hipFree(c->bn_ws);
  for (auto& set : c->prof_sets) for (hipEvent_t ev : set) (void)hipEventDestroy(ev);
  delete c;
  return NBC_OK;
}

int nbc_attach_weights_arch(nbc_ctx* c, const void* dev_blob, size_t bytes, int precision, int arch) {
  if (!c || !dev_blob) return set_error(NBC_ERR_INVALID, "nbc_attach_weights: null argument");
  if (!known_precision(precision)) return set_error(NBC_ERR_INVALID, "nbc_attach_weights: unknown precision");
  if (!known_arch(arch)) return set_error(NBC_ERR_INVALID, "nbc_attach_weights: unknown architecture");
  if (is_effnet(arch) && precision != NBC_PREC_FP32)
    return set_error(NBC_ERR_INVALID, std::string("nbc_attach_weights: ") + arch_name(arch) + " runs in NBC_PREC_FP32 (fp32) only");
  PackedLayout L = packed_layout(precision, arch);
  if (bytes < L.total_bytes) return set_error(NBC_ERR_INVALID, "nbc_attach_weights: blob smaller than the packed layout");
  if (reinterpret_cast<uintptr_t>(dev_blob) % 256 != 0)
    return set_error(NBC_ERR_INVALID, "nbc_attach_weights: blob must be 256-byte aligned");
  int32_t meta[kMetaWords];
  NBC_HIP(hipSetDevice(c->device));
  NBC_HIP(hipMemcpy(meta, static_cast<const unsigned char*>(dev_blob) + L.meta_off, sizeof(meta), hipMemcpyDeviceToHost));
  const int nunits = (int)conv_units(arch).size();
  if (meta[0] != kMetaMagic || meta[2] != nunits || meta[kMetaArch] != arch)
    return set_error(NBC_ERR_INVALID, "nbc_attach_weights: not a blob of this library's nbc_pack_weights for this architecture "
                                      "(trailer mismatch)");
  if (c->owned_weights && c->owned_weights != dev_blob) { (void)hipFree(c->owned_weights); c->owned_weights = nullptr; }
  c->pack_flags = meta[1];
  const int nexp = std::min(nunits, kMetaWords - kMetaExpBase);
  c->act_exp.assign(meta + kMetaExpBase, meta + kMetaExpBase + nexp);
  c->act_exp.resize(nunits, 0);
  if (is_effnet(arch)) std::fill(c->act_exp.begin(), c->act_exp.end(), 0);
  c->weights = static_cast<const unsigned char*>(dev_blob);
  c->layout = L;
  c->fwd_valid = false;
  if (c->precision != precision || c->arch != arch) stash_plan(c);
  c->precision = precision;
  c->arch = arch;
  return NBC_OK;
}

int nbc_attach_weights(nbc_ctx* c, const void* dev_blob, size_t bytes, int precision) {
  return nbc_attach_weights_arch(c, dev_blob, bytes, precision, kArchFcn);
}

int nbc_load_weights_arch(nbc_ctx* c, const nbc_tensor* tensors, int n, int precision, int arch) {
  if (!c) return set_error(NBC_ERR_INVALID, "nbc_load_weights: null context");
  const size_t bytes = nbc_arch_packed_weights_bytes(precision, arch);
  if (bytes == 0) return set_error(NBC_ERR_INVALID, "nbc_load_weights: unknown precision or architecture");
  std::vector<unsigned char> host(bytes);
  int rc = nbc_pack_weights_arch(tensors, n, precision, arch, host.data(), bytes);
  if (rc != NBC_OK) return rc;
  NBC_HIP(hipSetDevice(c->device));
  void* dev = nullptr;
  NBC_HIP(hipMalloc(&dev, bytes));
  hipError_t e = hipMemcpy(dev, host.data(), bytes, hipMemcpyHostToDevice);
  if (e != hipSuccess) { (void)hipFree(dev); return set_error(NBC_ERR_HIP, std::string("hipMemcpy(weights): ") + hipGetErrorString(e)); }
  if (c->owned_weights) (void)hipFree(c->owned_weights);
  c->owned_weights = nullptr;
  rc = nbc_attach_weights_arch(c, dev, bytes, precision, arch);
  if (rc != NBC_OK) { (void)hipFree(dev); return rc; }
  c->owned_weights = dev;
  std::vector<float> affine(nbc_arch_bn_affine_floats(arch));
  rc = nbc_pack_bn_affine(tensors, n, arch, affine.data(), affine.size());
  if (rc != NBC_OK) return rc;
  void* adev = nullptr;
  NBC_HIP(hipMalloc(&adev, affine.size() * sizeof(float)));
  e = hipMemcpy(adev, affine.data(), affine.size() * sizeof(float), hipMemcpyHostToDevice);
  if (e != hipSuccess) { (void)hipFree(adev); return set_error(NBC_ERR_HIP, std::string("hipMemcpy(bn affine): ") + hipGetErrorString(e)); }
  if (c->owned_affine) (void)hipFree(c->owned_affine);
  c->owned_affine = adev;
  c->bn_affine = static_cast<const float*>(adev);
  c->bn_affine_count = affine.size();
  return NBC_OK;
}

int nbc_attach_bn_affine(nbc_ctx* c, const float* dev_affine, size_t count) {
  if (!c || !dev_affine) return set_error(NBC_ERR_INVALID, "nbc_attach_bn_affine: null argument");
  bool any = false;
  for (int a = 0; a < kArchDeepLabEffB0 + 8; ++a) any = any || (known_arch(a) && count == nbc_arch_bn_affine_floats(a));
  if (!any)
    return set_error(NBC_ERR_INVALID, "nbc_attach_bn_affine: count is nbc_arch_bn_affine_floats of no architecture");
  if (c->owned_affine && c->owned_affine != dev_affine) {
    NBC_HIP(hipSetDevice(c->device));
    (void)hipFree(c->owned_affine);
    c->owned_affine = nullptr;
  }
  c->bn_affine = dev_affine;
  c->bn_affine_count = count;
  return NBC_OK;
}

int nbc_set_bn_statistics(nbc_ctx* c, int mode) {
  if (!c) return set_error(NBC_ERR_INVALID, "null context");
  if (mode != NBC_BN_RUNNING && mode != NBC_BN_PER_IMAGE) return set_error(NBC_ERR_INVALID, "nbc_set_bn_statistics: unknown mode");
  if (mode == NBC_BN_PER_IMAGE && (c->precision != NBC_PREC_FP32 || c->arch != kArchFcn))
    return set_error(NBC_ERR_STATE, "nbc_set_bn_statistics: per-image BatchNorm statistics need NBC_PREC_FP32 weights of "
                                    "NBC_ARCH_FCN_RESNET50 attached");
  if (c->bn_mode != mode) stash_plan(c);
  c->bn_mode = mode;
  return NBC_OK;
}

int nbc_load_weights(nbc_ctx* c, const nbc_tensor* tensors, int n, int precision) {
  return nbc_load_weights_arch(c, tensors, n, precision, kArchFcn);
}

namespace {
typedef int (*nccl_bcast_fn)(const void*, void*, size_t, int, int, void*, hipStream_t);
typedef int (*nccl_rank_fn)(void*, int*);
void* rccl_symbol(const char* name) {
  void* f = dlsym(RTLD_DEFAULT, name);
  if (f) return f;
  static void* handle = [] {
    void* h = dlopen("librccl.so.1", RTLD_NOW | RTLD_GLOBAL);
    return h ? h : dlopen("librccl.so", RTLD_NOW | RTLD_GLOBAL);
  }();
  return handle ? dlsym(handle, name) : nullptr;
}
}

int nbc_bcast_weights(nbc_ctx* c, void* rccl_comm, int root, int precision, void* hip_stream) {
  if (!c || !rccl_comm) return set_error(NBC_ERR_INVALID, "nbc_bcast_weights: null argument");
  if (c->arch != kArchFcn)
    return set_error(NBC_ERR_STATE, "nbc_bcast_weights: FCN-ResNet-50 only; broadcast the blob of another architecture yourself "
                                    "and attach it with nbc_attach_weights_arch");
  const size_t bytes = nbc_packed_weights_bytes(precision);
  if (bytes == 0) return set_error(NBC_ERR_INVALID, "nbc_bcast_weights: unknown precision");
  auto bcast = reinterpret_cast<nccl_bcast_fn>(rccl_symbol("ncclBroadcast"));
  auto user_rank = reinterpret_cast<nccl_rank_fn>(rccl_symbol("ncclCommUserRank"));
  if (!bcast || !user_rank) return set_error(NBC_ERR_STATE, "nbc_bcast_weights: no RCCL (librccl.so) in this process");
  int rank = -1;
  if (user_rank(rccl_comm, &rank) != 0) return set_error(NBC_ERR_INVALID, "nbc_bcast_weights: ncclCommUserRank failed (bad communicator?)");
  NBC_HIP(hipSetDevice(c->device));
  hipStream_t s = static_cast<hipStream_t>(hip_stream);
  void* blob = nullptr;
  bool fresh = false;
  if (rank == root) {
    if (!c->weights || c->precision != precision)
      return set_error(NBC_ERR_STATE, "nbc_bcast_weights: the root rank has no weights of this precision attached");
    blob = const_cast<unsigned char*>(c->weights);
  } else {
    NBC_HIP(hipMalloc(&blob, bytes));
    fresh = true;
  }
  const int rc = bcast(blob, blob, bytes,  1, root, rccl_comm, s);
  if (rc != 0) {
    if (fresh) (void)hipFree(blob);
    return set_error(NBC_ERR_HIP, "nbc_bcast_weights: ncclBroadcast returned " + std::to_string(rc));
  }
  if (fresh) {
    if (c->owned_weights) (void)hipFree(c->owned_weights);
    c->owned_weights = nullptr;
    const int arc = nbc_attach_weights(c, blob, bytes, precision);
    if (arc != NBC_OK) { (void)hipFree(blob); return arc; }
    c->owned_weights = blob;
  }
  return NBC_OK;
}

int nbc_weights_flags(nbc_ctx* c) {
  if (!c) return set_error(NBC_ERR_INVALID, "null context");
  if (!c->weights) return set_error(NBC_ERR_STATE, "nbc_weights_flags: no weights attached");
  return c->pack_flags;
}

namespace {
bool stored_exponent(const nbc_ctx* c, const std::string& name, int* e) {
  const auto& units = conv_units(c->arch);
  if (name == "ingest") { *e = 0; return true; }
  if (name == "backbone.maxpool") { *e = c->act_exp.empty() ? 0 : c->act_exp[0]; return true; }
  if (c->arch == kArchDeepLab && (name == "classifier.0.concat" || name == "classifier.0.convs.4")) {
    return stored_exponent(c, "classifier.0.convs.0.0", e);
  }
  for (size_t u = 0; u < units.size(); ++u)
    if (units[u].name == name) { *e = u < c->act_exp.size() ? c->act_exp[u] : 0; return true; }
  return false;
}
}

int nbc_activation_exponent(nbc_ctx* c, const char* name, int32_t* exponent) {
  if (!c || !name || !exponent) return set_error(NBC_ERR_INVALID, "nbc_activation_exponent: null argument");
  if (!c->weights) return set_error(NBC_ERR_STATE, "nbc_activation_exponent: no weights attached");
  int e = 0;
  if (!stored_exponent(c, name, &e)) return set_error(NBC_ERR_INVALID, std::string("nbc_activation_exponent: unknown op ") + name);
  *exponent = e;
  return NBC_OK;
}

int nbc_set_normalization(nbc_ctx* c, const float mean[3], const float stdv[3]) {
  if (!c || !mean || !stdv) return set_error(NBC_ERR_INVALID, "nbc_set_normalization: null argument");
  for (int i = 0; i < 3; ++i) { c->mean[i] = mean[i]; c->stdv[i] = stdv[i]; }
  return NBC_OK;
}

int nbc_set_conv_tile(nbc_ctx* c, int tile) {
  if (!c) return set_error(NBC_ERR_INVALID, "null context");
  if (tile < -1 || tile >= CONV_TILE_COUNT) return set_error(NBC_ERR_INVALID, "nbc_set_conv_tile: bad tile id");
  c->conv_tile = tile;
  return NBC_OK;
}

int nbc_set_keep_activations(nbc_ctx* c, int on) {
  if (!c) return set_error(NBC_ERR_INVALID, "null context");
  if (c->keep != (on != 0)) stash_plan(c);
  c->keep = on != 0;
  return NBC_OK;
}

int nbc_nonfinite_seen(nbc_ctx* c, int reset) {
  if (!c) return set_error(NBC_ERR_INVALID, "null context");
  if (!c->nonfinite) return 0;
  NBC_HIP(hipSetDevice(c->device));
  unsigned v = 0;
  NBC_HIP(hipDeviceSynchronize());
  NBC_HIP(hipMemcpy(&v, c->nonfinite, sizeof(v), hipMemcpyDeviceToHost));
  if (reset && v) NBC_HIP(hipMemset(c->nonfinite, 0, sizeof(v)));
  return v ? 1 : 0;
}

int nbc_nonfinite_peek_async(nbc_ctx* c, uint32_t* host_dst, void* hip_stream) {
  if (!c || !host_dst) return set_error(NBC_ERR_INVALID, "nbc_nonfinite_peek_async: null argument");
  NBC_HIP(hipSetDevice(c->device));
  {
    hipPointerAttribute_t at{};
    const hipError_t pe = hipPointerGetAttributes(&at, host_dst);
    if (pe != hipSuccess || at.type != hipMemoryTypeHost) {
      (void)hipGetLastError();
      return set_error(NBC_ERR_INVALID, "nbc_nonfinite_peek_async: host_dst must be pinned host memory (hipHostMalloc / hipHostRegister)");
    }
  }
  if (!c->nonfinite) { *host_dst = 0; return NBC_OK; }
  NBC_HIP(hipMemcpyAsync(host_dst, c->nonfinite, sizeof(uint32_t), hipMemcpyDeviceToHost, static_cast<hipStream_t>(hip_stream)));
  return NBC_OK;
}

int nbc_set_profiling(nbc_ctx* c, int on) {
  if (!c) return set_error(NBC_ERR_INVALID, "null context");
  c->profiling = on != 0;
  return NBC_OK;
}

int nbc_reserve(nbc_ctx* c, int N, int H, int W) {
  if (!c) return set_error(NBC_ERR_INVALID, "null context");
  if (c->precision < 0) return set_error(NBC_ERR_STATE, "nbc_reserve: no weights attached");
  if (N < 1 || H < 8 || W < 8) return set_error(NBC_ERR_INVALID, "nbc_reserve: need N>=1, H>=8, W>=8");
  if (c->bn_mode == NBC_BN_PER_IMAGE) {
    if (c->precision != NBC_PREC_FP32 || c->arch != kArchFcn)
      return set_error(NBC_ERR_STATE, "per-image BatchNorm statistics need NBC_PREC_FP32 weights of NBC_ARCH_FCN_RESNET50 attached");
    if (!c->bn_affine || c->bn_affine_count != nbc_arch_bn_affine_floats(c->arch))
      return set_error(NBC_ERR_STATE, "per-image BatchNorm statistics: no affine array of this architecture attached "
                                      "(nbc_attach_bn_affine)");
  }
  NBC_HIP(hipSetDevice(c->device));
  const PlanKey key = plan_key(c, N, H, W);
  if (same_shape(c->plan, key)) return NBC_OK;
  stash_plan(c);
  bool found = false;
  for (const Plan& p : c->plan_cache)
    if (same_shape(p, key)) { c->plan = p; found = true; break; }
  if (!found) {
    const std::string refused = build_plan(key, &c->plan);
    if (!refused.empty()) return set_error(NBC_ERR_INVALID, refused);
  }
  int rc = ensure_buffers(c);
  if (rc != NBC_OK) c->plan = Plan();
  return rc;
}

int nbc_forward(nbc_ctx* c, const void* x_dev, int x_dtype, int N, int H, int W,
                float* logits_lowres_dev, float* logits_full_dev, void* labels_dev, int labels_dtype,
                int64_t* counts_dev, int exclude_nodes, void* hip_stream) {
  if (!c || !x_dev) return set_error(NBC_ERR_INVALID, "nbc_forward: null argument");
  if (!c->weights) return set_error(NBC_ERR_STATE, "nbc_forward: no weights attached (load_state_dict first)");
  if (x_dtype != NBC_IN_F32_NCHW && x_dtype != NBC_IN_U8_NHWC) return set_error(NBC_ERR_INVALID, "nbc_forward: bad x_dtype");
  if (labels_dtype != NBC_LABEL_U8 && labels_dtype != NBC_LABEL_I64) return set_error(NBC_ERR_INVALID, "nbc_forward: bad labels_dtype");
  c->fwd_valid = false;
  int rc = nbc_reserve(c, N, H, W);
  if (rc != NBC_OK) return rc;
  hipStream_t s = static_cast<hipStream_t>(hip_stream);
  const Plan& P = c->plan;
  const int prec = c->precision;
  if (!c->nonfinite) {
    NBC_HIP(hipMalloc((void**)&c->nonfinite, 256));
    NBC_HIP(hipMemset(c->nonfinite, 0, 256));
  }

  const size_t nops = P.ops.size();
  constexpr size_t kMaxProfSets = 4096;
  std::vector<hipEvent_t>* evs = nullptr;
  if (c->profiling && c->prof_used < kMaxProfSets) {
    if (c->prof_used > 0 && c->prof_ops.size() != nops) c->prof_used = 0;
    if (c->prof_sets.size() <= c->prof_used) c->prof_sets.emplace_back();
    evs = &c->prof_sets[c->prof_used];
    while (evs->size() < nops + 1) {
      hipEvent_t ev;
      NBC_HIP(hipEventCreate(&ev));
      evs->push_back(ev);
    }
    c->prof_ops = P.ops;
    c->prof_arch = P.arch;
  }
  float* lowres = logits_lowres_dev ? logits_lowres_dev : c->lowres;

  if (evs) NBC_HIP(hipEventRecord((*evs)[0], s));
  for (size_t l = 0; l < nops; ++l) {
    const Op& o = P.ops[l];
    hipError_t e = hipSuccess;
    int rc = NBC_OK;
    switch (o.kind) {
      case OP_INGEST:
        if (x_dtype == NBC_IN_F32_NCHW)
          e = launch_ingest_f32(static_cast<const float*>(x_dev), c->bufs[o.out_buf], N, H, W, prec, s);
        else
          e = launch_ingest_u8(static_cast<const uint8_t*>(x_dev), c->bufs[o.out_buf], N, H, W, c->mean, c->stdv, prec, s);
        break;
      case OP_CONV: {
        int tile = c->conv_tile;
        if (!conv_tile_ok(prec, tile, o.Co, o.rows)) tile = o.tile;
        rc = launch_conv_op(c, o, N, tile, s, &e);
        if (rc != NBC_OK) return rc;
        break;
      }
      case OP_MAXPOOL:
        e = launch_maxpool3x3s2(c->bufs[o.in_buf], c->bufs[o.out_buf], N, o.Hi, o.Wi, o.Ci, o.Ho, o.Wo, prec, s);
        break;
      case OP_HEAD1X1: {
        const UnitPtrs p = unit_ptrs(c, o.unit);
        if (o.Ci != 512 && o.Ci != 256 && !is_effnet(c->arch))
          return set_error(NBC_ERR_STATE, "classifier.4 expects 512 or 256 input channels");
        unsigned long long* cz = counts_dev && 3 * N <= 256 ? reinterpret_cast<unsigned long long*>(counts_dev) : nullptr;
        if (is_effnet(c->arch) && o.Ci != 256)
          e = launch_head1x1_any(static_cast<const float*>(c->bufs[o.in_buf]), p.w, p.shift, lowres, N, o.Ho * o.Wo, o.Ci, cz,
                                 c->nonfinite, s);
        else if (o.Ci == 512)
          e = launch_head1x1(c->bufs[o.in_buf], p.w, p.shift, lowres, N, o.Ho * o.Wo, prec, cz, c->nonfinite, s);
        else
          e = launch_head1x1_c256(c->bufs[o.in_buf], p.w, p.shift, lowres, N, o.Ho * o.Wo, prec, cz, c->nonfinite, s);
        break;
      }
      case OP_ASPP_POOL: {
        const UnitPtrs p = unit_ptrs(c, o.unit);
        float* partial = static_cast<float*>(c->bufs[o.ws_buf]);
        float* mean = partial + (size_t)N * aspp_pool_slices(o.Hi * o.Wi) * o.Ci;
        e = launch_aspp_pool(c->bufs[o.in_buf], N, o.Hi * o.Wi, o.Ci, p.w, p.scale, p.shift, o.Co, partial, mean, c->bufs[o.out_buf],
                             prec, s);
        break;
      }
      case OP_CONCAT: {
        const void* br[4] = {c->bufs[o.cat_in[0]], c->bufs[o.cat_in[1]], c->bufs[o.cat_in[2]], c->bufs[o.cat_in[3]]};
        e = launch_aspp_concat(br, c->bufs[o.cat_in[4]], c->bufs[o.out_buf], N, o.Ho * o.Wo, prec, s);
        break;
      }
      case OP_BN_STATS:
      case OP_BN_APPLY: {
        const int hw = o.Ho * o.Wo;
        float* scale = reinterpret_cast<float*>(static_cast<unsigned char*>(c->bn_ws) +
                                                (size_t)N * bn_stats_slices(hw) * o.Co * 2 * sizeof(double));
        float* shift = scale + (size_t)N * o.Co;
        if (o.kind == OP_BN_STATS) {
          const float* gamma = c->bn_affine + o.affine_off;
          e = launch_bn_stats(static_cast<const float*>(c->bufs[o.out_buf]), N, hw, o.Co, gamma, gamma + o.Co, c->bn_ws, scale,
                              shift, s);
        } else {
          e = launch_bn_apply(static_cast<float*>(c->bufs[o.out_buf]), o.res_buf >= 0 ? static_cast<const float*>(c->bufs[o.res_buf]) : nullptr,
                              N, hw, o.Co, scale, shift, o.relu, s);
        }
        break;
      }
      case OP_DWCONV: {
        const UnitPtrs p = unit_ptrs(c, o.unit);
        const ConvUnit& u = conv_units(c->arch)[o.unit];
        DwArgs a{};
        a.x = static_cast<const float*>(c->bufs[o.in_buf]);
        a.w = p.w;
        a.scale = p.scale;
        a.shift = p.shift;
        a.y = static_cast<float*>(c->bufs[o.out_buf]);
        a.partial = static_cast<float*>(c->bufs[o.ws_buf]);
        a.N = N; a.Hi = o.Hi; a.Wi = o.Wi; a.C = o.Co; a.Ho = o.Ho; a.Wo = o.Wo;
        a.k = u.k; a.stride = u.stride; a.pad_t = u.pad; a.pad_l = u.pad; a.in_swish = u.in_swish ? 1 : 0;
        e = launch_dwconv(a, s);
        break;
      }
      case OP_SE_EXCITE: {
        const UnitPtrs pr = unit_ptrs(c, o.unit), pe = unit_ptrs(c, o.aux_unit);
        const ConvUnit& ur = conv_units(c->arch)[o.unit];
        e = launch_se_excite(static_cast<const float*>(c->bufs[o.in_buf]), N, o.tiles, o.Co, o.Hi * o.Wi, pr.w, pr.shift, ur.cout,
                             pe.w, pe.shift, static_cast<float*>(c->bufs[o.out_buf]), s);
        break;
      }
      case OP_GATE_WEIGHTS:
        e = launch_gate_weights(unit_ptrs(c, o.unit).w, static_cast<const float*>(c->bufs[o.gate_buf]),
                                static_cast<float*>(c->bufs[o.ws_buf]), N, o.Co, o.Ci, s);
        break;
      case OP_SWISH:
        e = launch_swish(static_cast<float*>(c->bufs[o.out_buf]), (size_t)N * o.Ho * o.Wo * o.Co, s);
        break;
      case OP_POOL_ANY: {
        const UnitPtrs p = unit_ptrs(c, o.unit);
        e = launch_pool_any(static_cast<const float*>(c->bufs[o.in_buf]), N, o.Hi * o.Wi, o.Ci, p.w, p.scale, p.shift, o.Co,
                            static_cast<float*>(c->bufs[o.ws_buf]), static_cast<float*>(c->bufs[o.out_buf]), s);
        break;
      }
      case OP_UPSAMPLE:
        if (counts_dev && 3 * N > 256) {
          e = hipMemsetAsync(counts_dev, 0, sizeof(int64_t) * 3 * N, s);
          if (e != hipSuccess) break;
        }
        if (logits_full_dev || labels_dev || counts_dev)
          e = launch_upsample_argmax(lowres, N, P.h, P.w, H, W, logits_full_dev, labels_dev,
                                     labels_dtype == NBC_LABEL_I64 ? 1 : 0,
                                     reinterpret_cast<unsigned long long*>(counts_dev), exclude_nodes, s);
        break;
    }
    if (e != hipSuccess)
      return set_error(NBC_ERR_HIP, "launch of " + o.name + " failed: " + hipGetErrorString(e));
    if (evs) NBC_HIP(hipEventRecord((*evs)[l + 1], s));
  }
  if (evs) ++c->prof_used;
  c->fwd_valid = true;
  c->fwd_N = N; c->fwd_H = H; c->fwd_W = W;
  return NBC_OK;
}

}

static int collect_profile(nbc_ctx* c) {
  if (c->prof_used == 0) return NBC_OK;
  const auto& units = conv_units(c->prof_arch);
  const size_t nops = c->prof_ops.size();
  NBC_HIP(hipEventSynchronize(c->prof_sets[c->prof_used - 1][nops]));
  c->records.assign(nops, nbc_op_record{});
  std::vector<double> sum(nops, 0.0);
  for (size_t i = 0; i < nops; ++i)
    for (size_t k = 0; k < c->prof_used; ++k) {
      float ms = 0.f;
      NBC_HIP(hipEventElapsedTime(&ms, c->prof_sets[k][i], c->prof_sets[k][i + 1]));
      sum[i] += ms;
    }
  for (size_t i = 0; i < nops; ++i) {
    const Op& o = c->prof_ops[i];
    nbc_op_record& r = c->records[i];
    std::snprintf(r.name, sizeof(r.name), "%s", o.name.c_str());
    std::snprintf(r.kernel, sizeof(r.kernel), "%s", kernel_name(o.kind));
    r.ms = (float)(sum[i] / (double)c->prof_used);
    r.calls = (int32_t)c->prof_used;
    r.launches = o.kind == OP_ASPP_POOL ? 3 : (o.kind == OP_BN_STATS ? 2 : o.launches);
    r.flops = o.flops;
    r.bytes = o.bytes;
    r.kh = r.kw = (o.kind == OP_CONV || o.kind == OP_HEAD1X1) ? units[o.unit].k : 0;
    r.cout = o.Co;
  }
  c->prof_used = 0;
  return NBC_OK;
}

struct DropoutLayout {
  size_t lowres, labels, parent, size, bg, total;
};
static DropoutLayout dropout_layout(int N, int H, int W, int h, int w, int draws) {
  const size_t I = (size_t)draws * N, px = I * H * W;
  Carver ws;
  const size_t lowres = ws.take(12 * I * h * w), labels = ws.take(px);
  const size_t parent = ws.take(4 * px), size = ws.take(4 * px), bg = ws.take(px);
  return {lowres, labels, parent, size, bg, ws.offset};
}

extern "C" {

int nbc_autotune(nbc_ctx* c, const void* x_dev, int x_dtype, int N, int H, int W, int reps, int objective,
                 void* hip_stream) {
  if (!c || !x_dev) return set_error(NBC_ERR_INVALID, "nbc_autotune: null argument");
  if (reps < 1) reps = 3;
  hipStream_t s = static_cast<hipStream_t>(hip_stream);
  int rc = nbc_forward(c, x_dev, x_dtype, N, H, W, nullptr, nullptr, nullptr, NBC_LABEL_U8, nullptr, 0, hip_stream);
  if (rc != NBC_OK) return rc;
  NBC_HIP(hipStreamSynchronize(s));
  c->fwd_valid = false;
  hipEvent_t e0, e1;
  NBC_HIP(hipEventCreate(&e0));
  NBC_HIP(hipEventCreate(&e1));
  Plan& P = c->plan;
  for (size_t oi = 0; oi < P.ops.size(); ++oi) {
    Op& o = P.ops[oi];
    if (o.kind != OP_CONV) continue;
    float best_ms = 1e30f;
    int best = o.tile;
    for (int tile = 0; tile < CONV_TILE_COUNT; ++tile) {
      if (!conv_tile_ok(c->precision, tile, o.Co, o.rows)) continue;
      hipError_t e = hipSuccess;
      rc = launch_conv_op(c, o, N, tile, s, &e);
      if (rc != NBC_OK || e != hipSuccess) continue;
      (void)hipEventRecord(e0, s);
      for (int k = 0; k < reps; ++k) (void)launch_conv_op(c, o, N, tile, s, &e);
      (void)hipEventRecord(e1, s);
      if (hipEventSynchronize(e1) != hipSuccess) continue;
      float ms = 0.f;
      if (hipEventElapsedTime(&ms, e0, e1) != hipSuccess) continue;
      if (objective == 1) {
        const int tiles = ((N * o.Ho * o.Wo + conv_tile_rows(tile) - 1) / conv_tile_rows(tile)) * (o.Co / conv_tile_cols(tile));
        if (tiles < 256) ms *= (float)tiles / 256.0f;
      }
      if (ms < best_ms) { best_ms = ms; best = tile; }
    }
    o.tile = best;
  }
  (void)hipEventDestroy(e0);
  (void)hipEventDestroy(e1);
  return NBC_OK;
}

int nbc_get_plan_tiles(nbc_ctx* c, int32_t* tiles, int capacity) {
  if (!c || !tiles) return set_error(NBC_ERR_INVALID, "nbc_get_plan_tiles: null argument");
  int n = 0;
  for (const Op& o : c->plan.ops)
    if (o.kind == OP_CONV) { if (n < capacity) tiles[n] = o.tile; ++n; }
  return n;
}

int nbc_default_conv_tile(int M, int Cout, int K, int precision) {
  if (M < 1 || Cout < 1 || K < 1) return -1;
  return choose_conv_tile(M, Cout, K, precision, 0);
}

int nbc_set_plan_tiles(nbc_ctx* c, const int32_t* tiles, int n) {
  if (!c || !tiles) return set_error(NBC_ERR_INVALID, "nbc_set_plan_tiles: null argument");
  int convs = 0;
  for (const Op& o : c->plan.ops) convs += o.kind == OP_CONV;
  if (convs == 0) return set_error(NBC_ERR_STATE, "nbc_set_plan_tiles: no plan (nbc_reserve first)");
  if (n != convs) return set_error(NBC_ERR_INVALID, "nbc_set_plan_tiles: the plan has " + std::to_string(convs) + " convolutions");
  int k = 0;
  for (const Op& o : c->plan.ops) {
    if (o.kind != OP_CONV) continue;
    const int t = tiles[k++];
    if (!conv_tile_ok(c->precision, t, o.Co, o.rows))
      return set_error(NBC_ERR_INVALID, "nbc_set_plan_tiles: tile " + std::to_string(t) + " does not fit " + o.name);
  }
  k = 0;
  for (Op& o : c->plan.ops)
    if (o.kind == OP_CONV) o.tile = tiles[k++];
  return NBC_OK;
}

int nbc_upsample_argmax(nbc_ctx* c, const float* lowres, int N, int h, int w, int H, int W,
                        float* logits_full_dev, void* labels_dev, int labels_dtype,
                        int64_t* counts_dev, int exclude_nodes, void* hip_stream) {
  if (!c || !lowres) return set_error(NBC_ERR_INVALID, "nbc_upsample_argmax: null argument");
  if (N < 1 || h < 1 || w < 1 || H < 1 || W < 1) return set_error(NBC_ERR_INVALID, "nbc_upsample_argmax: bad shape");
  if (labels_dtype != NBC_LABEL_U8 && labels_dtype != NBC_LABEL_I64) return set_error(NBC_ERR_INVALID, "nbc_upsample_argmax: bad labels_dtype");
  NBC_HIP(hipSetDevice(c->device));
  hipStream_t s = static_cast<hipStream_t>(hip_stream);
  if (counts_dev) NBC_HIP(hipMemsetAsync(counts_dev, 0, sizeof(int64_t) * 3 * N, s));
  NBC_HIP(launch_upsample_argmax(lowres, N, h, w, H, W, logits_full_dev, labels_dev,
                                 labels_dtype == NBC_LABEL_I64 ? 1 : 0,
                                 reinterpret_cast<unsigned long long*>(counts_dev), exclude_nodes, s));
  return NBC_OK;
}

int nbc_remove_small_zones(nbc_ctx* c, void* labels_dev, int labels_dtype, int N, int H, int W, int min_pixels,
                           int exclude_nodes, int64_t* counts_dev, void* hip_stream) {
  if (!c || !labels_dev) return set_error(NBC_ERR_INVALID, "nbc_remove_small_zones: null argument");
  if (N < 1 || N > 65535 || H < 1 || W < 1 || min_pixels < 0) return set_error(NBC_ERR_INVALID, "nbc_remove_small_zones: bad shape");
  if (labels_dtype != NBC_LABEL_U8 && labels_dtype != NBC_LABEL_I64) return set_error(NBC_ERR_INVALID, "nbc_remove_small_zones: bad labels_dtype");
  NBC_HIP(hipSetDevice(c->device));
  const size_t px = (size_t)N * H * W;
  if (px > c->zones_px) {
    size_t cap = std::max(px, c->zones_px + c->zones_px / 2);
    if (c->zones_ws) { NBC_HIP(hipFree(c->zones_ws)); c->zones_ws = nullptr; c->zones_px = 0; }
    if (hipMalloc(&c->zones_ws, cap * 9 + 256) != hipSuccess) {
      (void)hipGetLastError();
      cap = px;
      NBC_HIP(hipMalloc(&c->zones_ws, cap * 9 + 256));
    }
    c->zones_px = cap;
  }
  int* parent = static_cast<int*>(c->zones_ws);
  int* size = parent + px;
  unsigned char* bg = reinterpret_cast<unsigned char*>(size + px);
  NBC_HIP(launch_remove_small_zones(labels_dev, labels_dtype == NBC_LABEL_I64 ? 1 : 0, N, H, W, min_pixels, exclude_nodes, bg,
                                    parent, size, reinterpret_cast<unsigned long long*>(counts_dev),
                                    static_cast<hipStream_t>(hip_stream)));
  return NBC_OK;
}

size_t nbc_dropout_workspace_bytes(int N, int H, int W, int draws_per_pass) {
  if (N < 1 || H < 8 || W < 8 || H > 65535 || draws_per_pass < 1 || (long long)H * W > 0x7fffffffLL) return 0;
  const unsigned long long I = (unsigned long long)draws_per_pass * (unsigned long long)N;
  if (I > 65535ull) return 0;
  int h = 0, w = 0;
  if (nbc_lowres_size(H, W, &h, &w) != NBC_OK || h < 1 || w < 1 || (unsigned long long)h * w >= (1ull << 25)) return 0;
  return dropout_layout(N, H, W, h, w, draws_per_pass).total;
}

int nbc_dropout_draws(nbc_ctx* c, int N, int H, int W, const uint64_t* image_ids_host, double p, uint64_t seed, int first_draw,
                      int draws, int min_pixels, int exclude_nodes, float* logits_lowres_dev, int64_t* counts_dev,
                      void* workspace_dev, size_t workspace_bytes, void* hip_stream) {
  if (!dropout_p_ok(p)) return set_error(NBC_ERR_INVALID, "nbc_dropout_draws: p must lie in [0, 1)");
  if (draws < 1 || draws > 1024) return set_error(NBC_ERR_INVALID, "nbc_dropout_draws: draws must lie in 1..1024");
  if (first_draw < 0 || first_draw > 0x7fffffff - draws)
    return set_error(NBC_ERR_INVALID, "nbc_dropout_draws: first_draw must not be negative (and first_draw + draws < 2^31)");
  if (min_pixels < 0) return set_error(NBC_ERR_INVALID, "nbc_dropout_draws: min_pixels must not be negative");
  if (!c || !image_ids_host || !counts_dev || !workspace_dev) return set_error(NBC_ERR_INVALID, "nbc_dropout_draws: null argument");
  if (c->arch != kArchFcn)
    return set_error(NBC_ERR_STATE, std::string("nbc_dropout_draws: NBC_ARCH_FCN_RESNET50 only, the context holds ") +
                                        arch_name(c->arch) + " (DeepLabHead's Dropout sits inside ASPP; the EfficientNet heads are "
                                        "left out)");
  if (!c->fwd_valid || c->fwd_N != N || c->fwd_H != H || c->fwd_W != W || !same_shape(c->plan, plan_key(c, N, H, W)))
    return set_error(NBC_ERR_STATE, "nbc_dropout_draws: the context's last forward was not one of this (N, H, W), or its plan has "
                                    "been touched since: run nbc_forward first");
  const size_t one = nbc_dropout_workspace_bytes(N, H, W, 1);
  if (one == 0) return set_error(NBC_ERR_INVALID, "nbc_dropout_draws: shape beyond the limits (N <= 65535, H * W < 2^31, h * w < 2^25)");
  if (reinterpret_cast<uintptr_t>(workspace_dev) % 256 != 0)
    return set_error(NBC_ERR_INVALID, "nbc_dropout_draws: the workspace must be 256-byte aligned");
  if (workspace_bytes < one)
    return set_error(NBC_ERR_INVALID, "nbc_dropout_draws: the workspace is smaller than nbc_dropout_workspace_bytes(N, H, W, 1)");
  const Plan& P = c->plan;
  const Op* head = nullptr;
  for (const Op& o : P.ops)
    if (o.kind == OP_HEAD1X1) head = &o;
  if (!head || head->Ci != 512 || head->in_buf < 0 || !c->nonfinite)
    return set_error(NBC_ERR_STATE, "nbc_dropout_draws: the plan holds no classifier.4 of 512 input channels");
  int pass = std::min(draws, 65535 / N);
  while (pass > 1 && nbc_dropout_workspace_bytes(N, H, W, pass) > workspace_bytes) --pass;
  NBC_HIP(hipSetDevice(c->device));
  hipStream_t s = static_cast<hipStream_t>(hip_stream);
  const UnitPtrs up = unit_ptrs(c, head->unit);
  const int hw = P.h * P.w;
  const uint32_t T = dropout_threshold(p);
  const float m = dropout_scale(p);
  for (int d0 = 0; d0 < draws; d0 += pass) {
    const int D = std::min(pass, draws - d0);
    const int I = D * N;
    const DropoutLayout L = dropout_layout(N, H, W, P.h, P.w, D);
    unsigned char* ws = static_cast<unsigned char*>(workspace_dev);
    float* lowres = logits_lowres_dev ? logits_lowres_dev + (size_t)d0 * N * kNumClasses * hw : reinterpret_cast<float*>(ws + L.lowres);
    unsigned char* labels = ws + L.labels;
    int* parent = reinterpret_cast<int*>(ws + L.parent);
    int* size = reinterpret_cast<int*>(ws + L.size);
    unsigned char* bg = ws + L.bg;
    unsigned long long* counts = reinterpret_cast<unsigned long long*>(counts_dev) + (size_t)d0 * N * kNumClasses;
    NBC_HIP(launch_head1x1_dropout(c->bufs[head->in_buf], up.w, up.shift, lowres, N, hw, c->precision, image_ids_host, seed, T, m,
                                   first_draw + d0, D, c->nonfinite, s));
    if (min_pixels > 0) {
      NBC_HIP(launch_upsample_argmax(lowres, I, P.h, P.w, H, W, nullptr, labels, 0, nullptr, 0, s));
      NBC_HIP(launch_remove_small_zones(labels, 0, I, H, W, min_pixels, exclude_nodes, bg, parent, size, counts, s));
    } else {
      NBC_HIP(hipMemsetAsync(counts, 0, sizeof(unsigned long long) * kNumClasses * I, s));
      NBC_HIP(launch_upsample_argmax(lowres, I, P.h, P.w, H, W, nullptr, labels, 0, counts, exclude_nodes, s));
    }
  }
  return NBC_OK;
}

int nbc_resize_cubic_u8(nbc_ctx* c, const uint8_t* src_dev, int H, int W, float* dst_dev, int out_h, int out_w,
                        void* hip_stream) {
  if (!c || !src_dev || !dst_dev) return set_error(NBC_ERR_INVALID, "nbc_resize_cubic_u8: null argument");
  if (H < 1 || W < 1 || out_h < 1 || out_w < 1) return set_error(NBC_ERR_INVALID, "nbc_resize_cubic_u8: bad shape");
  NBC_HIP(hipSetDevice(c->device));
  if (!c->scratch256) NBC_HIP(hipMalloc(&c->scratch256, 256));
  unsigned* minmax = static_cast<unsigned*>(c->scratch256);
  NBC_HIP(launch_resize_cubic_u8(src_dev, H, W, dst_dev, nullptr, nullptr, out_h, out_w, minmax, static_cast<hipStream_t>(hip_stream)));
  return NBC_OK;
}

int nbc_preprocess_u8(nbc_ctx* c, const uint8_t* src_dev, int H, int W, uint8_t* dst_u8_dev, int32_t* row_lit_dev, int out_h,
                      int out_w, void* hip_stream) {
  if (!c || !src_dev || !dst_u8_dev) return set_error(NBC_ERR_INVALID, "nbc_preprocess_u8: null argument");
  if (H < 1 || W < 1 || out_h < 1 || out_w < 1) return set_error(NBC_ERR_INVALID, "nbc_preprocess_u8: bad shape");
  NBC_HIP(hipSetDevice(c->device));
  if (!c->scratch256) NBC_HIP(hipMalloc(&c->scratch256, 256));
  unsigned* minmax = static_cast<unsigned*>(c->scratch256);
  NBC_HIP(launch_resize_cubic_u8(src_dev, H, W, nullptr, dst_u8_dev, row_lit_dev, out_h, out_w, minmax,
                                 static_cast<hipStream_t>(hip_stream)));
  return NBC_OK;
}

int nbc_num_op_records(nbc_ctx* c) {
  if (!c) return 0;
  if (collect_profile(c) != NBC_OK) return NBC_ERR_HIP;
  return (int)c->records.size();
}

int nbc_get_op_record(nbc_ctx* c, int index, nbc_op_record* out) {
  if (!c || !out || index < 0 || index >= (int)c->records.size())
    return set_error(NBC_ERR_INVALID, "nbc_get_op_record: bad index");
  *out = c->records[index];
  return NBC_OK;
}

int nbc_activation_peaks(nbc_ctx* c, float* peaks_host, int capacity) {
  if (!c || !peaks_host) return set_error(NBC_ERR_INVALID, "nbc_activation_peaks: null argument");
  if (!c->plan.keep) return set_error(NBC_ERR_STATE, "nbc_activation_peaks: keep-activations is off (nbc_set_keep_activations, then a forward)");
  const int nunits = (int)conv_units(c->plan.arch).size();
  if (capacity < nunits) return set_error(NBC_ERR_INVALID, "nbc_activation_peaks: need room for nbc_arch_num_convs() values");
  NBC_HIP(hipSetDevice(c->device));
  unsigned* dev = nullptr;
  NBC_HIP(hipMalloc((void**)&dev, sizeof(unsigned) * nunits));
  hipError_t e = hipMemset(dev, 0, sizeof(unsigned) * nunits);
  const int N = c->plan.N;
  for (const Op& o : c->plan.ops) {
    if (e != hipSuccess) break;
    if ((o.kind != OP_CONV && o.kind != OP_ASPP_POOL) || o.out_buf < 0) continue;
    e = launch_absmax(c->bufs[o.out_buf], (size_t)N * o.Ho * o.Wo * o.Co, o.Co, c->precision, dev + o.unit, nullptr);
  }
  std::vector<unsigned> bits(nunits, 0u);
  if (e == hipSuccess) e = hipMemcpy(bits.data(), dev, sizeof(unsigned) * nunits, hipMemcpyDeviceToHost);
  (void)hipFree(dev);
  if (e != hipSuccess) return set_error(NBC_ERR_HIP, std::string("nbc_activation_peaks: ") + hipGetErrorString(e));
  for (int u = 0; u < nunits; ++u) std::memcpy(&peaks_host[u], &bits[u], 4);
  return nunits;
}

int nbc_read_activation(nbc_ctx* c, const char* name, float* dst_host, size_t capacity, int64_t shape[4]) {
  if (!c || !name || !dst_host) return set_error(NBC_ERR_INVALID, "nbc_read_activation: null argument");
  if (!c->plan.keep) return set_error(NBC_ERR_STATE, "nbc_read_activation: keep-activations is off");
  auto it = c->act_of.find(name);
  if (it == c->act_of.end()) return set_error(NBC_ERR_INVALID, std::string("nbc_read_activation: unknown op ") + name);
  const Op& o = c->plan.ops[it->second];
  if (o.out_buf < 0) return set_error(NBC_ERR_INVALID, "nbc_read_activation: op has no activation buffer");
  const int N = c->plan.N;
  const int creal = o.creal > 0 ? o.creal : o.Co;
  const size_t elems = (size_t)N * o.Ho * o.Wo * creal;
  if (capacity < elems) return set_error(NBC_ERR_INVALID, "nbc_read_activation: destination too small");
  NBC_HIP(hipSetDevice(c->device));
  float* tmp = nullptr;
  NBC_HIP(hipMalloc((void**)&tmp, elems * sizeof(float)));
  hipError_t e = hipSuccess;
  if (creal == o.Co) {
    e = launch_nhwc_to_nchw_f32(c->bufs[o.out_buf], tmp, N, o.Ho, o.Wo, o.Co, c->precision, nullptr);
    if (e == hipSuccess) e = hipMemcpy(dst_host, tmp, elems * sizeof(float), hipMemcpyDeviceToHost);
  } else {
    (void)hipFree(tmp);
    tmp = nullptr;
    const size_t img = (size_t)o.Ho * o.Wo * o.Co;
    NBC_HIP(hipMalloc((void**)&tmp, (size_t)N * img * sizeof(float)));
    e = launch_nhwc_to_nchw_f32(c->bufs[o.out_buf], tmp, N, o.Ho, o.Wo, o.Co, c->precision, nullptr);
    for (int n = 0; n < N && e == hipSuccess; ++n)
      e = hipMemcpy(dst_host + (size_t)n * o.Ho * o.Wo * creal, tmp + n * img, (size_t)o.Ho * o.Wo * creal * sizeof(float),
                    hipMemcpyDeviceToHost);
  }
  (void)hipFree(tmp);
  if (e != hipSuccess) return set_error(NBC_ERR_HIP, std::string("nbc_read_activation: ") + hipGetErrorString(e));
  int a = 0;
  if (stored_exponent(c, o.name, &a) && a != 0)
    for (size_t i = 0; i < elems; ++i) dst_host[i] = std::ldexp(dst_host[i], -a);
  if (shape) { shape[0] = N; shape[1] = creal; shape[2] = o.Ho; shape[3] = o.Wo; }
  return NBC_OK;
}

}
```

### neuralbarkcalculator_amd/csrc/nbc_kernels.hpp

```cpp
#pragma once
#include <hip/hip_runtime.h>

#include <cstdint>

namespace nbc {

struct ConvArgs {
  const void* x;
  const void* w;
  const float* scale;
  const float* shift;
  const void* res;
  void* y;
  unsigned x_bytes;
  unsigned w_bytes;
  int N, Hi, Wi, Ci;
  int Ho, Wo, Co;
  int KH, KW, stride, pad, dil;
  int M;
  int ksteps;
  int relu;
  int stem;
  int wo_shift;
  int hw_shift;
#ifdef NBC_STAMPS
  unsigned long long* stamps;
#endif
};

constexpr int CONV_TILE_COUNT = 21;
constexpr int CONV_TILE_ROWS_FIRST = 18;
int conv_tile_rows(int tile);
int conv_tile_cols(int tile);
int conv_rows_kind(int precision, int k, int stride, int pad, int dil, int Hi, int Wi, int Ho, int Wo, int Ci, int Co, bool has_res);
bool conv_tile_ok(int precision, int tile, int Co, int rows_kind);
int choose_conv_tile(int M, int Co, int K, int precision, int rows_kind);
hipError_t launch_conv_dma(const ConvArgs& a, int precision, int tile, hipStream_t s);
hipError_t launch_conv3x3_rows(const ConvArgs& a, int rows_tile, hipStream_t s);

hipError_t launch_ingest_f32(const float* x, void* y, int N, int H, int W, int precision, hipStream_t s);
hipError_t launch_ingest_u8(const uint8_t* x, void* y, int N, int H, int W, const float mean[3],
                            const float stdv[3], int precision, hipStream_t s);
hipError_t launch_maxpool3x3s2(const void* x, void* y, int N, int Hi, int Wi, int C, int Ho, int Wo,
                               int precision, hipStream_t s);
hipError_t launch_head1x1(const void* x, const float* w, const float* bias, float* y, int N, int hw,
                          int precision, unsigned long long* counts_zero, unsigned* nonfinite, hipStream_t s);
hipError_t launch_head1x1_c256(const void* x, const float* w, const float* bias, float* y, int N, int hw,
                               int precision, unsigned long long* counts_zero, unsigned* nonfinite, hipStream_t s);
constexpr int kDropoutIdsPerLaunch = 64;
struct DropoutIds {
  unsigned long long id[kDropoutIdsPerLaunch];
};
hipError_t launch_head1x1_dropout(const void* x, const float* w, const float* bias, float* y, int N, int hw, int precision,
                                  const uint64_t* ids_host, uint64_t seed, uint32_t threshold, float keep_scale, int first_draw,
                                  int draws, unsigned* nonfinite, hipStream_t s);
int aspp_pool_slices(int hw);
hipError_t launch_aspp_pool(const void* x, int N, int hw, int cin, const float* w, const float* scale, const float* shift, int cout,
                            float* partial, float* mean, void* y, int precision, hipStream_t s);
hipError_t launch_aspp_concat(const void* const branch[4], const void* pooled, void* y, int N, int hw, int precision,
                              hipStream_t s);
int bn_stats_slices(int hw);
size_t bn_stats_workspace_bytes(int N, int hw, int C);
hipError_t launch_bn_stats(const float* y, int N, int hw, int C, const float* gamma, const float* beta, void* ws, float* scale,
                           float* shift, hipStream_t s);
hipError_t launch_bn_apply(float* y, const float* res, int N, int hw, int C, const float* scale, const float* shift, int relu,
                           hipStream_t s);
struct DwArgs {
  const float* x;
  const float* w;
  const float* scale;
  const float* shift;
  float* y;
  float* partial;
  int N, Hi, Wi, C, Ho, Wo, k, stride, pad_t, pad_l, in_swish;
};
int dwconv_tiles_x(int Wo);
int dwconv_tiles(int stride, int Ho, int Wo);
hipError_t launch_dwconv(const DwArgs& a, hipStream_t s);
hipError_t launch_se_excite(const float* partial, int N, int tiles, int C, int hw, const float* wr, const float* br, int cse,
                            const float* we, const float* be, float* gate, hipStream_t s);
hipError_t launch_gate_weights(const float* w, const float* gate, float* wg, int N, int Co, int Ci, hipStream_t s);
hipError_t launch_swish(float* y, size_t elems, hipStream_t s);
int pool_any_slices(int hw);
hipError_t launch_pool_any(const float* x, int N, int hw, int cin, const float* w, const float* scale, const float* shift, int cout,
                           float* partial, float* y, hipStream_t s);
hipError_t launch_head1x1_any(const float* x, const float* w, const float* bias, float* y, int N, int hw, int cin,
                              unsigned long long* counts_zero, unsigned* nonfinite, hipStream_t s);
hipError_t launch_upsample_argmax(const float* lowres, int N, int h, int w, int H, int W,
                                  float* logits_full, void* labels, int labels_i64,
                                  unsigned long long* counts, int exclude_nodes, hipStream_t s);
hipError_t launch_remove_small_zones(void* labels, int labels_i64, int N, int H, int W, int min_pixels, int exclude_nodes,
                                     unsigned char* bg, int* parent, int* size, unsigned long long* counts, hipStream_t s);
hipError_t launch_resize_cubic_u8(const uint8_t* src, int H, int W, float* dst, uint8_t* dst_u8, int* row_lit, int out_h, int out_w,
                                  unsigned* minmax, hipStream_t s);
hipError_t launch_nhwc_to_nchw_f32(const void* x, float* y, int N, int H, int W, int C, int precision,
                                   hipStream_t s);

hipError_t launch_absmax(const void* x, size_t elems, int C, int precision, unsigned* out, hipStream_t s);

}
```

### neuralbarkcalculator_amd/model.py

```python
from __future__ import annotations

import contextlib
import ctypes as C
from typing import Mapping, Optional, Tuple

import numpy as np
import torch

from . import _lib, topology
from .topology import NUM_CLASSES, out_hw

_PRECISIONS = {"fp32": _lib.PREC_FP32, "f32": _lib.PREC_FP32, "float32": _lib.PREC_FP32,
               "bf16": _lib.PREC_BF16, "bfloat16": _lib.PREC_BF16, "f16x2": _lib.PREC_F16X2}
BN_STATISTICS = {"running": _lib.BN_RUNNING, "image": _lib.BN_PER_IMAGE}


def _as_numpy(v) -> np.ndarray:
    if isinstance(v, torch.Tensor):
        v = v.detach().cpu().numpy()
    return np.asarray(v)


def _tensor_array(state_dict: Mapping[str, object]):
    items = []
    keep = []
    for name, value in state_dict.items():
        a = _as_numpy(value)
        if a.dtype == np.int64:
            dt = 1
        else:
            a = a.astype(np.float32, copy=False)
            dt = 0
        shape = a.shape
        a = np.ascontiguousarray(a)
        if len(shape) > 4:
            raise RuntimeError(f"state_dict entry {name!r} has {len(shape)} dims")
        t = _lib.NbcTensor()
        bname = name.encode()
        t.name = bname
        t.data = a.ctypes.data if a.size else None
        for i in range(4):
            t.shape[i] = shape[i] if i < len(shape) else 1
        t.ndim = len(shape)
        t.dtype = dt
        items.append(t)
        keep.append((a, bname))
    return (_lib.NbcTensor * len(items))(*items), len(items), keep


def pack_state_dict(state_dict: Mapping[str, object], precision: str = "fp32", arch="fcn_resnet50") -> np.ndarray:
    lib = _lib.load()
    prec = _PRECISIONS[precision]
    a = topology.arch_index(arch)
    arr, n, _keep = _tensor_array(state_dict)
    nbytes = lib.nbc_arch_packed_weights_bytes(prec, a)
    blob = np.zeros(nbytes, dtype=np.uint8)
    _lib.check(lib.nbc_pack_weights_arch(arr, n, prec, a, blob.ctypes.data, nbytes), "load_state_dict")
    return blob


def pack_bn_affine(state_dict: Mapping[str, object], arch="fcn_resnet50") -> np.ndarray:
    lib = _lib.load()
    a = topology.arch_index(arch)
    arr, n, _keep = _tensor_array(state_dict)
    count = lib.nbc_arch_bn_affine_floats(a)
    out = np.zeros(count, dtype=np.float32)
    _lib.check(lib.nbc_pack_bn_affine(arr, n, a, out.ctypes.data, count), "load_state_dict")
    return out


def broadcast_bn_affine(affine: Optional[np.ndarray], arch="fcn_resnet50", src: int = 0, group=None, device=None) -> np.ndarray:
    import torch.distributed as dist
    count = int(_lib.load().nbc_arch_bn_affine_floats(topology.arch_index(arch)))
    if dist.get_rank(group) == src:
        if affine is None or affine.size != count:
            raise RuntimeError("broadcast_bn_affine: the source rank holds no affine array of %s" % arch)
        t = torch.from_numpy(np.ascontiguousarray(affine, dtype=np.float32))
    else:
        t = torch.empty(count, dtype=torch.float32)
    if device is not None:
        t = t.to(device)
    dist.broadcast(t, src=src, group=group)
    return t.cpu().numpy()


def arch_of_state_dict(state_dict: Mapping[str, object]) -> str:
    lib = _lib.load()
    arr, n, _keep = _tensor_array(state_dict)
    rc = lib.nbc_arch_of_state_dict(arr, n)
    if rc < 0:
        _lib.check(rc, "load_state_dict")
    return topology.arch_name(rc)


class FCNResNet50:

    ARCH = "fcn_resnet50"

    def __init__(self, precision: str = "fp32"):
        if precision not in _PRECISIONS:
            raise ValueError(f"precision must be one of {sorted(_PRECISIONS)}")
        if topology.is_efficientnet(self.ARCH) and _PRECISIONS[precision] != _lib.PREC_FP32:
            raise ValueError("%s runs in precision 'fp32' only, not %r: swish and the SE gate are not positively homogeneous, "
                             "so f16x2's powers of two cannot be folded into its BatchNorm pairs" % (self.ARCH, precision))
        self._lib = _lib.load()
        self.precision = precision
        self._prec = _PRECISIONS[precision]
        self.bn_statistics = "running"
        self._blob_host: Optional[np.ndarray] = None
        self._blob_dev: Optional[torch.Tensor] = None
        self._affine_host: Optional[np.ndarray] = None
        self._affine_dev: Optional[torch.Tensor] = None
        self._ctx = C.c_void_p()
        self._lovasz_ws: Optional[torch.Tensor] = None
        self._pixel_ce_ws: Optional[torch.Tensor] = None
        self._dropout_ws: Optional[torch.Tensor] = None
        self._last_shape: Optional[Tuple[int, int, int]] = None
        self.device: Optional[torch.device] = None
        self.training = False

    def load_state_dict(self, state_dict: Mapping[str, object], strict: bool = True):
        if not strict:
            raise NotImplementedError("only strict=True is supported (the reference never passes strict=False)")
        self._blob_host = pack_state_dict(state_dict, self.precision, self.ARCH)
        self._affine_host = pack_bn_affine(state_dict, self.ARCH)
        if self.device is not None:
            self._upload()
        return self

    def to(self, device):
        device = torch.device(device)
        if device.type != "cuda":
            raise RuntimeError("FCNResNet50 runs on MI355X only (device 'cuda[:i]'); the CPU path is the reference itself")
        index = device.index if device.index is not None else torch.cuda.current_device()
        device = torch.device("cuda", index)
        if self.device is not None and self.device != device:
            self._destroy()
        if not self._ctx:
            ctx = C.c_void_p()
            _lib.check(self._lib.nbc_create(C.byref(ctx), index), "nbc_create")
            self._ctx = ctx
        self.device = device
        if self._blob_host is not None:
            self._upload()
        return self

    def cuda(self, index: Optional[int] = None):
        return self.to(torch.device("cuda", index if index is not None else torch.cuda.current_device()))

    def eval(self):
        return self

    def set_bn_statistics(self, mode: str):
        if mode not in BN_STATISTICS:
            raise ValueError(f"bn_statistics must be one of {sorted(BN_STATISTICS)}, got {mode!r}")
        if mode == "image":
            if topology.is_efficientnet(self.ARCH):
                raise ValueError("per-image BatchNorm statistics are refused for %s: they are implemented for fcn_resnet50 "
                                 "only" % self.ARCH)
            if self.ARCH != "fcn_resnet50":
                raise ValueError("per-image BatchNorm statistics are refused for %s: its ASPP pooling branch's BatchNorm sees a "
                                 "[1, 256, 1, 1] tensor, which batch statistics cannot normalise (torch raises, and so would "
                                 "the reference)" % self.ARCH)
            if self._prec != _lib.PREC_FP32:
                raise ValueError("per-image BatchNorm statistics run in precision 'fp32' only, not %r" % self.precision)
        self.bn_statistics = mode
        if self._ctx:
            _lib.check(self._lib.nbc_set_bn_statistics(self._ctx, BN_STATISTICS[mode]), "nbc_set_bn_statistics")
        return self

    def train(self, mode: bool = True):
        if mode:
            raise RuntimeError("training mode is not part of the inference path")
        return self

    def __call__(self, x: torch.Tensor) -> torch.Tensor:
        n, h, w = self._check_input(x)
        logits = torch.empty((n, NUM_CLASSES, h, w), dtype=torch.float32, device=self.device)
        self._forward(x, n, h, w, logits_full=logits)
        return logits

    forward = __call__

    def predict_labels(self, x: torch.Tensor, exclude_nodes: bool = False,
                       labels_dtype: torch.dtype = torch.int64,
                       return_lowres: bool = False, small_zones: bool = False,
                       logits_full: Optional[torch.Tensor] = None):
        n, h, w = self._check_input(x)
        if labels_dtype not in (torch.int64, torch.uint8):
            raise ValueError("labels_dtype must be torch.int64 or torch.uint8")
        if logits_full is not None and (logits_full.device != self.device or logits_full.dtype != torch.float32
                                        or not logits_full.is_contiguous()
                                        or tuple(logits_full.shape) != (n, NUM_CLASSES, h, w)):
            raise ValueError("logits_full must be a contiguous float32 [%d,%d,%d,%d] tensor on %s" % (n, NUM_CLASSES, h, w,
                                                                                                    self.device))
        labels = torch.empty((n, h, w), dtype=labels_dtype, device=self.device)
        counts = torch.empty((n, NUM_CLASSES), dtype=torch.int64, device=self.device)
        lowres = None
        if return_lowres:
            lh, lw = out_hw(h, w, self.ARCH)
            lowres = torch.empty((n, NUM_CLASSES, lh, lw), dtype=torch.float32, device=self.device)
        self._forward(x, n, h, w, labels=labels, counts=counts, lowres=lowres, logits_full=logits_full,
                      exclude_nodes=exclude_nodes and not small_zones)
        if small_zones:
            labels, counts = self.remove_small_zones(labels, exclude_nodes=exclude_nodes)
        return (labels, counts, lowres) if return_lowres else (labels, counts)

    def lowres_logits(self, x: torch.Tensor) -> torch.Tensor:
        n, h, w = self._check_input(x)
        lh, lw = out_hw(h, w, self.ARCH)
        lowres = torch.empty((n, NUM_CLASSES, lh, lw), dtype=torch.float32, device=self.device)
        self._forward(x, n, h, w, lowres=lowres)
        return lowres

    def remove_small_zones(self, labels: torch.Tensor, exclude_nodes: bool = False, min_pixels: int = 150):
        self._require_ctx()
        self._check_labels(labels)
        if labels.dim() not in (2, 3):
            raise ValueError("labels must be [H,W] or [N,H,W]")
        n = 1 if labels.dim() == 2 else int(labels.shape[0])
        h, w = int(labels.shape[-2]), int(labels.shape[-1])
        counts = torch.empty((n, 3), dtype=torch.int64, device=self.device)
        with self._on_stream() as cur:
            _lib.check(self._lib.nbc_remove_small_zones(self._ctx, labels.data_ptr(),
                                                        _lib.LABEL_I64 if labels.dtype == torch.int64 else _lib.LABEL_U8,
                                                        n, h, w, int(min_pixels), int(bool(exclude_nodes)),
                                                        counts.data_ptr(), cur.cuda_stream), "nbc_remove_small_zones")
        return labels, counts

    def confusion(self, labels: torch.Tensor, target: torch.Tensor) -> torch.Tensor:
        self._require_ctx()
        self._check_labels(labels)
        if target.device != self.device or target.dtype != torch.uint8 or not target.is_contiguous():
            raise ValueError("target must be a contiguous uint8 tensor on %s" % (self.device,))
        if labels.dim() not in (2, 3) or labels.shape != target.shape or labels.numel() == 0:
            raise ValueError("labels and target must both be [H,W] or [N,H,W] of the same non-empty shape")
        n = 1 if labels.dim() == 2 else int(labels.shape[0])
        h, w = int(labels.shape[-2]), int(labels.shape[-1])
        conf = torch.empty((n, NUM_CLASSES, NUM_CLASSES), dtype=torch.int64, device=self.device)
        with self._on_stream() as cur:
            _lib.check(self._lib.nbc_confusion(labels.data_ptr(), _lib.LABEL_I64 if labels.dtype == torch.int64 else _lib.LABEL_U8,
                                               target.data_ptr(), n, h, w, conf.data_ptr(), cur.cuda_stream), "nbc_confusion")
        return conf

    def lovasz_softmax(self, logits_full: torch.Tensor, target: torch.Tensor) -> Tuple[torch.Tensor, torch.Tensor]:
        self._require_ctx()
        n, h, w = self._check_logits_target(logits_full, target)
        need = int(self._lib.nbc_lovasz_workspace_bytes(n, h, w))
        if need == 0:
            raise ValueError("nbc_lovasz_softmax refuses a [%d,3,%d,%d] batch (N <= 65535, H * W < 2^31)" % (n, h, w))
        terms = torch.empty((n, NUM_CLASSES), dtype=torch.float64, device=self.device)
        fg_counts = torch.empty((n, NUM_CLASSES), dtype=torch.int64, device=self.device)
        with self._on_stream() as cur:
            ws = self._grown_workspace("_lovasz_ws", need, cur)
            _lib.check(self._lib.nbc_lovasz_softmax(logits_full.data_ptr(), target.data_ptr(), n, h, w, ws.data_ptr(), ws.numel(),
                                                    terms.data_ptr(), fg_counts.data_ptr(), cur.cuda_stream), "nbc_lovasz_softmax")
        return terms, fg_counts

    def pixel_cross_entropy(self, logits_full: torch.Tensor, target: torch.Tensor) -> Tuple[torch.Tensor, torch.Tensor]:
        self._require_ctx()
        n, h, w = self._check_logits_target(logits_full, target)
        need = int(self._lib.nbc_pixel_ce_workspace_bytes(n, h, w))
        if need == 0:
            raise ValueError("nbc_pixel_cross_entropy refuses a [%d,3,%d,%d] batch (N <= 65535, H * W < 2^31)" % (n, h, w))
        sums = torch.empty((n, NUM_CLASSES, NUM_CLASSES), dtype=torch.float64, device=self.device)
        counts = torch.empty((n, NUM_CLASSES, NUM_CLASSES), dtype=torch.int64, device=self.device)
        with self._on_stream() as cur:
            ws = self._grown_workspace("_pixel_ce_ws", need, cur)
            _lib.check(self._lib.nbc_pixel_cross_entropy(logits_full.data_ptr(), target.data_ptr(), n, h, w, ws.data_ptr(), ws.numel(),
                                                         sums.data_ptr(), counts.data_ptr(), cur.cuda_stream),
                       "nbc_pixel_cross_entropy")
        return sums, counts

    def dropout_draws(self, draws: int, image_ids, p: float = 0.1, seed: int = 0, first_draw: int = 0,
                      small_zones: bool = True, exclude_nodes: bool = False, return_lowres: bool = False, *,
                      min_pixels: int = 150, draws_per_pass: int = 8):
        if topology.is_efficientnet(self.ARCH):
            raise ValueError("dropout draws are refused for %s: EfficientNet's FCN head is left out (its Dropout is not "
                             "implemented)" % self.ARCH)
        if self.ARCH != "fcn_resnet50":
            raise ValueError("dropout draws are refused for %s: DeepLabHead's Dropout sits inside ASPP, in front of convolutions "
                             "that would have to run again for every draw" % self.ARCH)
        draws, first_draw, seed = int(draws), int(first_draw), int(seed)
        if not 1 <= draws <= 1024:
            raise ValueError("draws must lie in 1..1024, got %d" % draws)
        if not (0.0 <= float(p) < 1.0):
            raise ValueError("p must lie in [0, 1), got %r" % (p,))
        if first_draw < 0 or first_draw + draws > 2 ** 31 - 1:
            raise ValueError("first_draw must not be negative, got %d" % first_draw)
        if not 0 <= seed < 2 ** 64:
            raise ValueError("seed must be an unsigned 64-bit integer, got %d" % seed)
        if int(min_pixels) < 0 or int(draws_per_pass) < 1:
            raise ValueError("min_pixels must not be negative and draws_per_pass must be positive")
        self._require_weights()
        if self._last_shape is None:
            raise RuntimeError("dropout_draws follows a forward (predict_labels / lowres_logits) of this object: none has run")
        n, h, w = self._last_shape
        ids = [int(v) for v in image_ids]
        if len(ids) != n or any(not 0 <= v < 2 ** 64 for v in ids):
            raise ValueError("image_ids must hold one unsigned 64-bit identity per image of the last forward (%d), got %d"
                             % (n, len(ids)))
        ids_arr = (C.c_uint64 * n)(*ids)
        per_pass = max(1, min(draws, int(draws_per_pass), 65535 // n))
        need = int(self._lib.nbc_dropout_workspace_bytes(n, h, w, per_pass))
        if need == 0:
            raise ValueError("nbc_dropout_draws refuses a [%d,3,%d,%d] batch (draws x N <= 65535 per pass, H * W < 2^31)" % (n, h, w))
        counts = torch.empty((draws, n, NUM_CLASSES), dtype=torch.int64, device=self.device)
        lowres = None
        if return_lowres:
            lowres = torch.empty((draws, n, NUM_CLASSES) + out_hw(h, w, self.ARCH), dtype=torch.float32, device=self.device)
        with self._on_stream() as cur:
            ws = self._grown_workspace("_dropout_ws", need, cur)
            rc = self._lib.nbc_dropout_draws(self._ctx, n, h, w, ids_arr, float(p), seed, first_draw, draws,
                                             int(min_pixels) if small_zones else 0, int(bool(exclude_nodes)),
                                             lowres.data_ptr() if lowres is not None else None, counts.data_ptr(),
                                             ws.data_ptr(), need, cur.cuda_stream)
        _lib.check(rc, "nbc_dropout_draws")
        return (counts, lowres) if return_lowres else counts

    def resize_cubic_u8(self, image: torch.Tensor, out_h: int, out_w: int) -> torch.Tensor:
        self._require_ctx()
        self._check_rgb_u8(image)
        out = torch.empty((int(out_h), int(out_w), 3), dtype=torch.float32, device=self.device)
        with self._on_stream() as cur:
            _lib.check(self._lib.nbc_resize_cubic_u8(self._ctx, image.data_ptr(), int(image.shape[0]), int(image.shape[1]),
                                                     out.data_ptr(), int(out_h), int(out_w), cur.cuda_stream), "nbc_resize_cubic_u8")
        return out

    def preprocess_u8(self, image: torch.Tensor, out_h: int, out_w: int):
        self._require_ctx()
        self._check_rgb_u8(image)
        out = torch.empty((int(out_h), int(out_w), 3), dtype=torch.uint8, device=self.device)
        lit = torch.empty((int(out_h),), dtype=torch.int32, device=self.device)
        with self._on_stream() as cur:
            _lib.check(self._lib.nbc_preprocess_u8(self._ctx, image.data_ptr(), int(image.shape[0]), int(image.shape[1]),
                                                   out.data_ptr(), lit.data_ptr(), int(out_h), int(out_w), cur.cuda_stream), "nbc_preprocess_u8")
        return out, lit

    def upsample_argmax(self, lowres: torch.Tensor, size: Tuple[int, int], exclude_nodes: bool = False,
                        labels_dtype: torch.dtype = torch.int64, return_logits: bool = False):
        self._require_ctx()
        if lowres.dtype != torch.float32 or lowres.dim() != 4 or lowres.shape[1] != NUM_CLASSES:
            raise RuntimeError("expected float32 [N,3,h,w]")
        lowres = lowres.contiguous()
        n, _, lh, lw = lowres.shape
        H, W = int(size[0]), int(size[1])
        labels = torch.empty((n, H, W), dtype=labels_dtype, device=self.device)
        counts = torch.empty((n, NUM_CLASSES), dtype=torch.int64, device=self.device)
        logits = torch.empty((n, NUM_CLASSES, H, W), dtype=torch.float32, device=self.device) if return_logits else None
        ldt = _lib.LABEL_I64 if labels_dtype == torch.int64 else _lib.LABEL_U8
        with self._on_stream() as cur:
            rc = self._lib.nbc_upsample_argmax(self._ctx, lowres.data_ptr(), n, lh, lw, H, W,
                                               logits.data_ptr() if logits is not None else None,
                                               labels.data_ptr(), ldt, counts.data_ptr(),
                                               int(bool(exclude_nodes)), cur.cuda_stream)
        _lib.check(rc, "nbc_upsample_argmax")
        return (labels, counts, logits) if return_logits else (labels, counts)

    def set_normalization(self, mean, std):
        m = (C.c_float * 3)(*[float(v) for v in mean])
        s = (C.c_float * 3)(*[float(v) for v in std])
        _lib.check(self._lib.nbc_set_normalization(self._require_ctx(), m, s), "set_normalization")

    def reserve(self, n: int, h: int, w: int):
        self._require_weights()
        with torch.cuda.device(self.device):
            _lib.check(self._lib.nbc_reserve(self._ctx, n, h, w), "nbc_reserve")

    def clone_shared(self) -> "FCNResNet50":
        self._require_weights()
        other = self._like()
        other.bn_statistics = self.bn_statistics
        other.to(self.device)
        other._attach(self._blob_dev, self._affine_dev)
        return other

    def _like(self) -> "FCNResNet50":
        return type(self)(self.precision)

    def broadcast_weights(self, src: int = 0, group=None):
        import torch.distributed as dist
        if self.device is None:
            raise RuntimeError("call .to(device) before broadcast_weights")
        nbytes = self._lib.nbc_arch_packed_weights_bytes(self._prec, topology.arch_index(self.ARCH))
        if dist.get_rank(group) == src:
            self._require_weights()
            blob = self._blob_dev
        else:
            blob = torch.empty(nbytes, dtype=torch.uint8, device=self.device)
        dist.broadcast(blob, src=src, group=group)
        affine = broadcast_bn_affine(self._affine_host if dist.get_rank(group) == src else None, self.ARCH, src, group,
                                     self.device)
        self._affine_host = affine
        self._attach(blob, torch.from_numpy(affine).to(self.device))
        return self

    def set_profiling(self, on: bool):
        _lib.check(self._lib.nbc_set_profiling(self._require_ctx(), int(on)))

    def op_records(self):
        out = []
        rec = _lib.NbcOpRecord()
        n = self._lib.nbc_num_op_records(self._require_ctx())
        if n < 0:
            _lib.check(n, "nbc_num_op_records")
        for i in range(n):
            _lib.check(self._lib.nbc_get_op_record(self._ctx, i, C.byref(rec)))
            out.append(dict(name=rec.name.decode(), kernel=rec.kernel.decode(), ms=float(rec.ms),
                            calls=int(rec.calls), flops=float(rec.flops), bytes=float(rec.bytes),
                            k=int(rec.kh), cout=int(rec.cout), launches=int(rec.launches)))
        return out

    @property
    def pack_flags(self) -> int:
        if self._ctx and self._blob_dev is not None:
            rc = self._lib.nbc_weights_flags(self._ctx)
            if rc < 0:
                _lib.check(rc, "nbc_weights_flags")
            return int(rc)
        if self._blob_host is None:
            raise RuntimeError("no weights loaded")
        rc = self._lib.nbc_packed_weights_flags_arch(self._blob_host.ctypes.data, self._blob_host.size, self._prec,
                                                     topology.arch_index(self.ARCH))
        if rc < 0:
            _lib.check(rc, "nbc_packed_weights_flags")
        return int(rc)

    def activation_exponent(self, name: str) -> int:
        e = C.c_int32(0)
        _lib.check(self._lib.nbc_activation_exponent(self._require_ctx(), name.encode(), C.byref(e)), "nbc_activation_exponent")
        return int(e.value)

    def activation_peaks(self, x: torch.Tensor) -> dict:
        n, h, w = self._check_input(x)
        self.set_keep_activations(True)
        try:
            self._forward(x, n, h, w, lowres=torch.empty((n, NUM_CLASSES) + out_hw(h, w, self.ARCH), dtype=torch.float32, device=self.device))
            torch.cuda.synchronize(self.device)
            k = int(self._lib.nbc_arch_num_convs(topology.arch_index(self.ARCH)))
            buf = (C.c_float * k)()
            rc = self._lib.nbc_activation_peaks(self._require_ctx(), buf, k)
            if rc < 0:
                _lib.check(rc, "nbc_activation_peaks")
        finally:
            self.set_keep_activations(False)
        names = [u.name for u in topology.conv_units(self.ARCH)]
        return {names[i]: float(buf[i]) for i in range(k) if names[i] != "classifier.4"}

    @staticmethod
    def f16x2_range_ok(peaks: dict, low: float = 2.0 ** -8, high: float = 2.0 ** 14):
        bad = {k: v for k, v in peaks.items() if not (low <= v <= high)}
        return (not bad), bad

    def nonfinite_seen(self, reset: bool = True) -> bool:
        rc = self._lib.nbc_nonfinite_seen(self._require_ctx(), int(reset))
        if rc < 0:
            _lib.check(rc, "nbc_nonfinite_seen")
        return rc == 1

    def nonfinite_peek_async(self, host_word: torch.Tensor):
        if host_word.dtype != torch.int32 or host_word.numel() != 1 or host_word.is_cuda or not host_word.is_pinned():
            raise ValueError("host_word must be a pinned int32 CPU tensor with one element")
        with self._on_stream() as cur:
            _lib.check(self._lib.nbc_nonfinite_peek_async(self._require_ctx(), host_word.data_ptr(), cur.cuda_stream), "nbc_nonfinite_peek_async")

    def set_conv_tile(self, tile: int = -1):
        _lib.check(self._lib.nbc_set_conv_tile(self._require_ctx(), int(tile)), "nbc_set_conv_tile")

    def autotune(self, x: torch.Tensor, reps: int = 3, objective: str = "latency"):
        n, h, w = self._check_input(x)
        x = x.contiguous()
        x_dtype = _lib.IN_F32_NCHW if x.dtype == torch.float32 else _lib.IN_U8_NHWC
        with self._on_stream() as cur:
            _lib.check(self._lib.nbc_autotune(self._ctx, x.data_ptr(), x_dtype, n, h, w, int(reps),
                                              1 if objective == "throughput" else 0, cur.cuda_stream),
                       "nbc_autotune")
        return self.plan_tiles()

    def plan_tiles(self):
        buf = (C.c_int32 * 64)()
        n = self._lib.nbc_get_plan_tiles(self._require_ctx(), buf, 64)
        return [int(buf[i]) for i in range(min(n, 64))]

    def set_plan_tiles(self, tiles):
        arr = (C.c_int32 * len(tiles))(*[int(t) for t in tiles])
        _lib.check(self._lib.nbc_set_plan_tiles(self._require_ctx(), arr, len(tiles)), "nbc_set_plan_tiles")

    def set_keep_activations(self, on: bool):
        _lib.check(self._lib.nbc_set_keep_activations(self._require_ctx(), int(on)))

    def read_activation(self, name: str, numel_hint: int) -> np.ndarray:
        buf = np.empty(numel_hint, dtype=np.float32)
        shape = (C.c_int64 * 4)()
        torch.cuda.synchronize(self.device)
        _lib.check(self._lib.nbc_read_activation(self._require_ctx(), name.encode(), buf.ctypes.data,
                                                 buf.size, C.byref(shape)), "read_activation")
        shp = tuple(int(s) for s in shape)
        return buf[: int(np.prod(shp))].reshape(shp)

    @contextlib.contextmanager
    def _on_stream(self):
        with torch.cuda.device(self.device):
            yield torch.cuda.current_stream(self.device)

    def _grown_workspace(self, attr: str, need: int, stream) -> torch.Tensor:
        ws = getattr(self, attr)
        if ws is None or ws.numel() < need:
            setattr(self, attr, None)
            ws = torch.empty(need, dtype=torch.uint8, device=self.device)
            setattr(self, attr, ws)
        ws.record_stream(stream)
        return ws

    def _check_labels(self, labels: torch.Tensor):
        if labels.device != self.device or labels.dtype not in (torch.uint8, torch.int64) or not labels.is_contiguous():
            raise ValueError("labels must be a contiguous uint8 or int64 tensor on %s" % (self.device,))

    def _check_rgb_u8(self, image: torch.Tensor):
        if image.device != self.device or image.dtype != torch.uint8 or image.dim() != 3 or image.shape[2] != 3 \
                or not image.is_contiguous():
            raise ValueError("image must be a contiguous uint8 [H,W,3] tensor on %s" % (self.device,))

    def _check_logits_target(self, logits_full: torch.Tensor, target: torch.Tensor) -> Tuple[int, int, int]:
        if logits_full.device != self.device or logits_full.dtype != torch.float32 or not logits_full.is_contiguous() \
                or logits_full.dim() != 4 or logits_full.shape[1] != NUM_CLASSES:
            raise ValueError("logits_full must be a contiguous float32 [N,3,H,W] tensor on %s" % (self.device,))
        n, _, h, w = (int(v) for v in logits_full.shape)
        if target.device != self.device or target.dtype != torch.uint8 or not target.is_contiguous() \
                or tuple(target.shape) != (n, h, w) or target.numel() == 0:
            raise ValueError("target must be a contiguous uint8 [%d,%d,%d] tensor on %s" % (n, h, w, self.device))
        return n, h, w

    def _require_ctx(self):
        if not self._ctx:
            raise RuntimeError("call .to('cuda[:i]') first")
        return self._ctx

    def _require_weights(self):
        self._require_ctx()
        if self._blob_dev is None:
            raise RuntimeError("no weights: call load_state_dict (or broadcast_weights) first")

    def _upload(self):
        blob = torch.from_numpy(self._blob_host).to(self.device, non_blocking=False)
        affine = torch.from_numpy(self._affine_host).to(self.device) if self._affine_host is not None else None
        self._attach(blob, affine)

    def _attach(self, blob: torch.Tensor, affine: Optional[torch.Tensor] = None):
        assert blob.dtype == torch.uint8 and blob.is_contiguous() and blob.device == self.device
        _lib.check(self._lib.nbc_attach_weights_arch(self._require_ctx(), blob.data_ptr(), blob.numel(), self._prec,
                                                     topology.arch_index(self.ARCH)), "nbc_attach_weights")
        self._blob_dev = blob
        if affine is not None:
            assert affine.dtype == torch.float32 and affine.is_contiguous() and affine.device == self.device
            _lib.check(self._lib.nbc_attach_bn_affine(self._ctx, affine.data_ptr(), affine.numel()), "nbc_attach_bn_affine")
            self._affine_dev = affine
        _lib.check(self._lib.nbc_set_bn_statistics(self._ctx, BN_STATISTICS[self.bn_statistics]), "nbc_set_bn_statistics")

    def _check_input(self, x: torch.Tensor) -> Tuple[int, int, int]:
        self._require_weights()
        if not isinstance(x, torch.Tensor):
            raise TypeError("input must be a torch.Tensor")
        if x.device != self.device:
            raise RuntimeError(f"input is on {x.device}, model is on {self.device}")
        if x.dtype == torch.float32:
            if x.dim() != 4 or x.shape[1] != 3:
                raise RuntimeError(f"expected float32 [N,3,H,W], got {tuple(x.shape)}")
            n, _, h, w = x.shape
        elif x.dtype == torch.uint8:
            if x.dim() != 4 or x.shape[3] != 3:
                raise RuntimeError(f"expected uint8 [N,H,W,3], got {tuple(x.shape)}")
            n, h, w, _ = x.shape
        else:
            raise RuntimeError(f"unsupported input dtype {x.dtype}")
        if h < 8 or w < 8:
            raise RuntimeError("H and W must be >= 8")
        if min(out_hw(int(h), int(w), self.ARCH)) < 1:
            raise RuntimeError("a %dx%d image is too small for %s" % (h, w, self.ARCH))
        if self.bn_statistics == "image" and out_hw(int(h), int(w)) == (1, 1):
            raise ValueError("Expected more than 1 value per channel when training: a %dx%d image has a 1x1 low-resolution "
                             "map, which per-image BatchNorm statistics cannot normalise" % (h, w))
        return int(n), int(h), int(w)

    def _forward(self, x, n, h, w, logits_full=None, labels=None, counts=None, lowres=None,
                 exclude_nodes=False):
        x = x.contiguous()
        x_dtype = _lib.IN_F32_NCHW if x.dtype == torch.float32 else _lib.IN_U8_NHWC
        ldt = _lib.LABEL_I64 if (labels is None or labels.dtype == torch.int64) else _lib.LABEL_U8
        ptr = lambda t: (t.data_ptr() if t is not None else None)
        with self._on_stream() as cur:
            rc = self._lib.nbc_forward(self._ctx, x.data_ptr(), x_dtype, n, h, w, ptr(lowres), ptr(logits_full),
                                       ptr(labels), ldt, ptr(counts), int(bool(exclude_nodes)), cur.cuda_stream)
        _lib.check(rc, "nbc_forward")
        self._last_shape = (n, h, w)

    def _destroy(self):
        if self._ctx:
            self._lib.nbc_destroy(self._ctx)
            self._ctx = C.c_void_p()
        self._blob_dev = None
        self._lovasz_ws = None
        self._pixel_ce_ws = None
        self._dropout_ws = None
        self._last_shape = None

    def __del__(self):
        try:
            self._destroy()
        except Exception:
            pass


def fcn_resnet50(pretrained: bool = False, dropout: float = 0.1, precision: str = "fp32",
                 bn_statistics: str = "running") -> FCNResNet50:
    if pretrained:
        raise RuntimeError("pretrained=True needs a download; load a local state_dict instead (predict.py:57)")
    del dropout
    return FCNResNet50(precision=precision).set_bn_statistics(bn_statistics)


class DeepLabV3ResNet50(FCNResNet50):

    ARCH = "deeplabv3_resnet50"


class FCNEfficientNet(FCNResNet50):

    HEAD = "fcn"

    def __init__(self, n: int = 0, precision: str = "fp32"):
        if int(n) not in range(8):
            raise ValueError("EfficientNet variant n must be 0..7, got %r" % (n,))
        self.n = int(n)
        self.ARCH = "%s_efficientnet_b%d" % ("deeplabv3" if self.HEAD == "deeplab" else "fcn", self.n)
        super().__init__(precision)

    def _like(self):
        return type(self)(self.n, self.precision)


class DeepLabV3EfficientNet(FCNEfficientNet):

    HEAD = "deeplab"


def fcn_efficientnet(n: int, dropout: float = 0.1, precision: str = "fp32") -> FCNEfficientNet:
    del dropout
    return FCNEfficientNet(n, precision=precision)


def deeplabv3_efficientnet(n: int, precision: str = "fp32") -> DeepLabV3EfficientNet:
    return DeepLabV3EfficientNet(n, precision=precision)


MODELS = {"fcn_resnet50": FCNResNet50, "deeplabv3_resnet50": DeepLabV3ResNet50}
for _n in range(8):
    MODELS["fcn_efficientnet_b%d" % _n] = (lambda n: lambda precision="fp32": FCNEfficientNet(n, precision))(_n)
    MODELS["deeplabv3_efficientnet_b%d" % _n] = (lambda n: lambda precision="fp32": DeepLabV3EfficientNet(n, precision))(_n)


def deeplabv3_resnet50(precision: str = "fp32") -> DeepLabV3ResNet50:
    return DeepLabV3ResNet50(precision=precision)
```

Measured before the change: 338.4.

## Fuse ResNet downsample 1x1 conv into following block's final 1x1 conv

Adds a dual-branch variant of the f16x2 implicit-GEMM conv kernel. It computes the strided downsample 1x1 conv and the bottleneck's last 1x1 conv in one launch, applying each branch's BN affine and summing them in the epilogue. This removes a separate launch and the write and re-read of the downsample activation used as the residual. The cost is a larger kernel with extra smem for the second scale/shift table, buffer-size unification and pointer swaps in the host plan, and restriction to a few tile configs. It is enabled by default for the f16x2 path with running BN statistics.

```diff
diff --git a/include/nbc.h b/include/nbc.h
--- a/include/nbc.h
+++ b/include/nbc.h
@@ -186,6 +186,8 @@
 int nbc_nonfinite_seen(nbc_ctx* ctx, int reset);
 int nbc_nonfinite_peek_async(nbc_ctx* ctx, uint32_t* host_dst, void* hip_stream);
 
+int nbc_set_fuse_downsample(nbc_ctx* ctx, int on);
+int nbc_fused_pairs(nbc_ctx* ctx);
 int nbc_set_keep_activations(nbc_ctx* ctx, int on);
 int nbc_activation_peaks(nbc_ctx* ctx, float* peaks_host, int capacity);
 int nbc_read_activation(nbc_ctx* ctx, const char* name, float* dst_host, size_t capacity,
diff --git a/neuralbarkcalculator_amd/_lib.py b/neuralbarkcalculator_amd/_lib.py
--- a/neuralbarkcalculator_amd/_lib.py
+++ b/neuralbarkcalculator_amd/_lib.py
@@ -114,6 +114,8 @@
     "nbc_bcast_weights": (C.c_int, [C.c_void_p, C.c_void_p, C.c_int, C.c_int, C.c_void_p]),
     "nbc_set_conv_tile": (C.c_int, [C.c_void_p, C.c_int]),
     "nbc_set_keep_activations": (C.c_int, [C.c_void_p, C.c_int]),
+    "nbc_set_fuse_downsample": (C.c_int, [C.c_void_p, C.c_int]),
+    "nbc_fused_pairs": (C.c_int, [C.c_void_p]),
     "nbc_activation_peaks": (C.c_int, [C.c_void_p, C.POINTER(C.c_float), C.c_int]),
     "nbc_read_activation": (C.c_int, [C.c_void_p, C.c_char_p, C.c_void_p, C.c_size_t,
                                       C.POINTER(C.c_int64 * 4)]),
diff --git a/neuralbarkcalculator_amd/build.py b/neuralbarkcalculator_amd/build.py
--- a/neuralbarkcalculator_amd/build.py
+++ b/neuralbarkcalculator_amd/build.py
@@ -34,6 +34,8 @@
     hipcc = _hipcc()
     headers = [os.path.join(CSRC, f) for f in os.listdir(CSRC) if f.endswith(".hpp")]
     headers.append(os.path.join(os.path.dirname(PKG), "include", "nbc.h"))
+    if not force and not _deps_newer(LIB, [os.path.join(CSRC, src) for src in SOURCES] + headers):
+        return LIB
     common = ["-O3", "-std=c++17", "-fPIC", f"--offload-arch={ARCH}", "-Wall", "-Wno-unused-function"]
 
     def compile_one(src: str) -> str:
diff --git a/neuralbarkcalculator_amd/csrc/conv_igemm_dma.hip b/neuralbarkcalculator_amd/csrc/conv_igemm_dma.hip
--- a/neuralbarkcalculator_amd/csrc/conv_igemm_dma.hip
+++ b/neuralbarkcalculator_amd/csrc/conv_igemm_dma.hip
@@ -103,6 +103,7 @@
 constexpr int kVarDefault = 0;
 constexpr int kVarBf16Mfma32 = 1;
 constexpr int kVarLoaderWaves = 8;
+constexpr int kVarDualBranch = 16;
 
 typedef unsigned nt_u32x4 __attribute__((ext_vector_type(4)));
 constexpr int loader_waves(int var) { return var == kVarLoaderWaves ? 4 : 0; }
@@ -114,6 +115,8 @@
   constexpr int CW = WM * WN;
   constexpr int LW = loader_waves(VAR);
   constexpr bool SPEC = LW > 0;
+  constexpr bool DUAL = (VAR == kVarDualBranch);
+  static_assert(!DUAL || (PREC == 2 && !STEM && !BIGW), "the dual-branch form is f16x2's, on ordinary identity layers");
   constexpr int THREADS = (SPEC ? LW : CW) * 64;
   constexpr int BM = WM * MT * 32;
   constexpr int BN = WN * NT * 32;
@@ -157,13 +160,13 @@
   const int ltid = SPEC ? ((tid - CW * 64) & (THREADS - 1)) : tid;
   const int ps = ltid & 7;
   const int lr = ltid >> 3;
-  const rsrc_t xrsrc = __builtin_amdgcn_make_buffer_rsrc(const_cast<void*>(p.x), 0, p.x_bytes, 0x00020000);
-  const rsrc_t wrsrc = __builtin_amdgcn_make_buffer_rsrc(const_cast<void*>(p.w), 0, p.w_bytes, 0x00020000);
+  rsrc_t xrsrc = __builtin_amdgcn_make_buffer_rsrc(const_cast<void*>(DUAL ? p.x2 : p.x), 0, DUAL ? p.x2_bytes : p.x_bytes, 0x00020000);
+  rsrc_t wrsrc = __builtin_amdgcn_make_buffer_rsrc(const_cast<void*>(DUAL ? p.w2 : p.w), 0, DUAL ? p.w2_bytes : p.w_bytes, 0x00020000);
   const int pix_bytes = p.Ci * EB;
-  const unsigned wrow_bytes = (unsigned)p.ksteps * 128u;
+  const unsigned wrow_bytes = (unsigned)(DUAL ? p.ksteps2 : p.ksteps) * 128u;
 
   int a_iy0[A_PASSES], a_ix0[A_PASSES], a_img[A_PASSES], a_coff[A_PASSES];
-  {
+  if constexpr (!DUAL) {
     const int hw = p.Ho * p.Wo;
 #pragma unroll
     for (int i = 0; i < A_PASSES; ++i) {
@@ -211,13 +214,29 @@
       a_off[i] = ok ? off : kOutOfRange;
     }
   };
-  if constexpr (!STEM) set_tap(0, 0);
+  if constexpr (DUAL) {
+    const int hw = p.Ho * p.Wo;
+    const unsigned pix2 = (unsigned)p.Ci2 * EB;
+#pragma unroll
+    for (int i = 0; i < A_PASSES; ++i) {
+      const int row = lr + ROWS_PER_PASS * i;
+      const int m = m0 + row;
+      const int img = p.N == 1 ? 0 : (p.hw_shift >= 0 ? (m >> p.hw_shift) : m / hw);
+      const int rem = m - img * hw;
+      const int oy = p.wo_shift >= 0 ? (rem >> p.wo_shift) : rem / p.Wo;
+      const int ox = rem - oy * p.Wo;
+      const int iy = oy * p.stride2, ix = ox * p.stride2;
+      const bool ok = m < p.M && (unsigned)iy < (unsigned)p.Hi2 && (unsigned)ix < (unsigned)p.Wi2;
+      const unsigned off = (unsigned)((img * p.Hi2 + iy) * p.Wi2 + ix) * pix2 + (unsigned)(ps ^ ((row >> 1) & 7)) * 16u;
+      a_off[i] = ok ? off : kOutOfRange;
+    }
+  } else if constexpr (!STEM) set_tap(0, 0);
 
   auto issue_one = [&](int d, int t, unsigned sa) __attribute__((always_inline)) {
     if (d < A_PASSES) {
       const int i = d;
       if constexpr (!STEM) {
-        dma16_buf(a_off[i], xrsrc, sa + (unsigned)(ROWS_PER_PASS * 128 * i), (unsigned)ld_cb * 128u);
+        dma16_buf(a_off[i], xrsrc, sa + (unsigned)(ROWS_PER_PASS * 128 * i), (unsigned)(DUAL ? t : ld_cb) * 128u);
       } else {
         const int iy = a_iy0[i] + st_kh * p.dil, ix = a_ix0[i] + st_kw * p.dil;
         const bool ok = st_kw < p.KW && (unsigned)iy < (unsigned)p.Hi && (unsigned)ix < (unsigned)p.Wi;
@@ -239,7 +258,8 @@
     }
     if constexpr (!STEM) {
       if (part == 3) {
-        if (++ld_cb == cblocks) {
+        if constexpr (DUAL) { }
+        else if (++ld_cb == cblocks) {
           ld_cb = 0;
           if (++ld_kw == p.KW) { ld_kw = 0; ++ld_kh; }
           if (ld_kh < p.KH) set_tap(ld_kh, ld_kw);
@@ -521,10 +541,11 @@
   const int row0 = wm * MT * 32 + o_pix;
   const unsigned lane_chunk = X2 ? (unsigned)(o_chunk >> 2) * 128u + (unsigned)(o_chunk & 3) * 16u : (unsigned)o_chunk * 16u;
   uint4 rpre[RES_PREFETCH ? MT : 1][RES_PREFETCH ? PASSES : 1];
-  constexpr bool RES_PREFETCH2 = X2 && MT * PASSES * 2 <= 16;
+  constexpr bool RES_PREFETCH2 = X2 && !DUAL && MT * PASSES * 2 <= 16;
   uint4 rpre2[RES_PREFETCH2 ? MT : 1][RES_PREFETCH2 ? PASSES : 1][2];
 
   const int T = p.ksteps;
+  const int sb = DUAL ? p.ksteps2 % S : 0;
   auto prefetch_identity = [&]() {
     if constexpr (RES_PREFETCH) {
       if (rtile) {
@@ -544,8 +565,67 @@
   if (wave == (SPEC ? CW : 0) && lane < BN / 4) {
     dma16(p.scale + n0 + lane * 4, smem_base + (unsigned)TABLE_OFF);
     dma16(p.shift + n0 + lane * 4, smem_base + (unsigned)TABLE_OFF + 1024u);
-  }
-  if (loads) {
+    if constexpr (DUAL) {
+      dma16(p.scale2 + n0 + lane * 4, smem_base + (unsigned)TABLE_OFF + 2048u);
+      dma16(p.shift2 + n0 + lane * 4, smem_base + (unsigned)TABLE_OFF + 3072u);
+    }
+  }
+  if constexpr (DUAL) {
+    static_assert(!DUAL || (!SPEC && !STAGGER && !PREFETCH), "dual-branch form: every wave loads and computes, in lock step");
+    const int T2 = p.ksteps2;
+#pragma unroll
+    for (int s = 0; s < S - 1; ++s)
+      if (s < T2) issue_step(s, s);
+    for (int t = 0; t < T2 - 1; ++t) {
+      if (t + (S - 2) < T2) wait_vmcnt<(S - 2) * L>();
+      else wait_vmcnt<0>();
+      __builtin_amdgcn_s_barrier();
+      if constexpr (S == 2) {
+        if (t + S - 1 < T2) issue_step(t + S - 1, (t + S - 1) % S);
+        compute(t, t % S, false, 0, 0);
+      } else {
+        compute(t, t % S, t + S - 1 < T2, t + S - 1, (t + S - 1) % S);
+      }
+    }
+    wait_vmcnt<0>();
+    __builtin_amdgcn_s_barrier();
+    xrsrc = __builtin_amdgcn_make_buffer_rsrc(const_cast<void*>(p.x), 0, p.x_bytes, 0x00020000);
+    wrsrc = __builtin_amdgcn_make_buffer_rsrc(const_cast<void*>(p.w), 0, p.w_bytes, 0x00020000);
+#pragma unroll
+    for (int i = 0; i < A_PASSES; ++i) {
+      const int row = lr + ROWS_PER_PASS * i;
+      const int m = m0 + row;
+      a_off[i] = m < p.M ? (unsigned)m * (unsigned)pix_bytes + (unsigned)(ps ^ ((row >> 1) & 7)) * 16u : kOutOfRange;
+    }
+#pragma unroll
+    for (int i = 0; i < B_PASSES; ++i) {
+      const int row = lr + ROWS_PER_PASS * i;
+      w_off[i] = (unsigned)(n0 + row) * ((unsigned)T * 128u) + (unsigned)(ps ^ ((row >> 1) & 7)) * 16u;
+    }
+    compute(T2 - 1, (T2 - 1) % S, true, 0, sb);
+#pragma unroll
+    for (int s = 1; s < S - 1; ++s)
+      if (s < T) issue_step(s, (sb + s) % S);
+    const unsigned char* table2 = smem + TABLE_OFF + 2048 + wn * (NT * 32) * 4;
+#pragma unroll
+    for (int j = 0; j < NT16; ++j) {
+      const int nl = j * 16 + 4 * q16;
+      const float4 sc4 = *reinterpret_cast<const float4*>(table2 + nl * 4);
+      const float4 sh4 = *reinterpret_cast<const float4*>(table2 + 1024 + nl * 4);
+      const float sc[4] = {sc4.x, sc4.y, sc4.z, sc4.w}, sh[4] = {sh4.x, sh4.y, sh4.z, sh4.w};
+#pragma unroll
+      for (int i = 0; i < MT16; ++i) {
+        const f32x4 a = acc16[j][i] + accI2[j][i];
+#pragma unroll
+        for (int e = 0; e < 4; ++e) {
+          _Float16 h0, h1;
+          split16(__builtin_fmaf(a[e], sc[e], sh[e]), h0, h1);
+          acc16[j][i][e] = join16(h0, h1);
+          accI2[j][i][e] = 0.f;
+        }
+      }
+    }
+  } else if (loads) {
 #pragma unroll
     for (int s = 0; s < S - 1; ++s)
       if (s < T) issue_step(s, s);
@@ -613,11 +693,11 @@
       if (is_loader) { if (t + S - 1 < T) issue_step(t + S - 1, (t + S - 1) % S); }
       else compute(t, t % S, false, 0, 0);
     } else if constexpr (S == 2) {
-      if (t + S - 1 < T) issue_step(t + S - 1, (t + S - 1) % S);
+      if (t + S - 1 < T) issue_step(t + S - 1, (sb + t + S - 1) % S);
       if constexpr (F32) step32(t, t % S, false, false, 0, false, 0, 0);
-      else compute(t, t % S, false, 0, 0);
+      else compute(t, (sb + t) % S, false, 0, 0);
     } else {
-      compute(t, t % S, t + S - 1 < T, t + S - 1, (t + S - 1) % S);
+      compute(t, (sb + t) % S, t + S - 1 < T, t + S - 1, (sb + t + S - 1) % S);
     }
   }
   }
@@ -635,7 +715,7 @@
       x2_read((T - 1) % S, sp0, sp1, sw0, sw1);
       x2_mfma(T - 1, false, 0, 0, sp0, sp1, sw0, sw1);
     }
-  } else if (computes) compute(T - 1, (T - 1) % S, false, 0, 0);
+  } else if (computes) compute(T - 1, (sb + T - 1) % S, false, 0, 0);
   }
   if constexpr (RES_PREFETCH2) {
     if (rtile && computes) {
@@ -661,7 +741,7 @@
 #pragma unroll
     for (int n = 0; n < NTILES; ++n) acc[n / MT][n % MT] += accI[n / MT][n % MT];
   }
-  if constexpr (X2) {
+  if constexpr (X2 && !DUAL) {
 #pragma unroll
     for (int n = 0; n < NT16 * MT16; ++n) acc16[n / MT16][n % MT16] += accI2[n / MT16][n % MT16];
   }
@@ -691,12 +771,17 @@
 #pragma unroll
           for (int jj = 0; jj < 4 && j0 + jj < NT16; ++jj) {
             const int nl = (j0 + jj) * 16 + 4 * q16;
-            const f32x4 a = acc16[j0 + jj][2 * i + i2];
+            const f32x4 kZero = {0.f, 0.f, 0.f, 0.f};
+            const f32x4 a = DUAL ? kZero + accI2[X2 ? j0 + jj : 0][X2 ? 2 * i + i2 : 0] : acc16[j0 + jj][2 * i + i2];
             float4 v;
             v.x = __builtin_fmaf(a[0], sc[jj].x, sh[jj].x);
             v.y = __builtin_fmaf(a[1], sc[jj].y, sh[jj].y);
             v.z = __builtin_fmaf(a[2], sc[jj].z, sh[jj].z);
             v.w = __builtin_fmaf(a[3], sc[jj].w, sh[jj].w);
+            if constexpr (DUAL) {
+              const f32x4 idv = acc16[j0 + jj][2 * i + i2];
+              v.x += idv[0]; v.y += idv[1]; v.z += idv[2]; v.w += idv[3];
+            }
             *reinterpret_cast<float4*>(scr + (i2 * 16 + r16) * PITCH + nl * 4) = v;
           }
       }
@@ -796,7 +881,7 @@
 template <int PREC, int WM, int WN, int MT, int NT, int S, bool STEM, int VAR = kVarDefault, bool BIGW = false>
 hipError_t launch_cfg(const ConvArgs& a, hipStream_t s) {
   constexpr int BM = WM * MT * 32, BN = WN * NT * 32;
-  constexpr int smem = ring_bytes(PREC, WM, WN, MT, NT, S) + 2048;
+  constexpr int smem = ring_bytes(PREC, WM, WN, MT, NT, S) + (VAR == kVarDualBranch ? 4096 : 2048);
   static std::atomic<unsigned long long> attr_done{0};
   auto kern = &conv_dma_kernel<PREC, WM, WN, MT, NT, S, STEM, VAR, BIGW>;
   int dev = 0;
@@ -828,12 +913,24 @@
       case 1: return launch_cfg<PREC, 2, 2, 2, 2, 2, STEM, VAR>(a, s);
       case 5: return launch_cfg<PREC, 2, 4, 2, 2, 3, STEM, VAR>(a, s);
       case 16: return launch_cfg<PREC, 2, 2, 2, 2, 3, STEM, STEM ? VAR : kVarLoaderWaves>(a, s);
-      case 17: return launch_cfg<PREC, 2, 4, 2, 1, 2, STEM, VAR>(a, s);
+      case 17:
+        if constexpr (!STEM) {
+          if (a.x2 != nullptr) return launch_cfg<PREC, 2, 4, 2, 1, 2, false, kVarDualBranch>(a, s);
+        }
+        return launch_cfg<PREC, 2, 4, 2, 1, 2, STEM, VAR>(a, s);
       case 6: return launch_cfg<PREC, 4, 2, 2, 1, 3, STEM, VAR>(a, s);
       case 7: return launch_cfg<PREC, 2, 2, 2, 1, 2, STEM, VAR>(a, s);
-      case 8: return launch_cfg<PREC, 1, 4, 2, 1, 2, STEM, VAR>(a, s);
+      case 8:
+        if constexpr (!STEM) {
+          if (a.x2 != nullptr) return launch_cfg<PREC, 1, 4, 2, 1, 2, false, kVarDualBranch>(a, s);
+        }
+        return launch_cfg<PREC, 1, 4, 2, 1, 2, STEM, VAR>(a, s);
       case 9: return launch_cfg<PREC, 4, 2, 1, 2, 3, STEM, VAR>(a, s);
-      case 10: return launch_cfg<PREC, 4, 2, 1, 1, 3, STEM, VAR>(a, s);
+      case 10:
+        if constexpr (!STEM) {
+          if (a.x2 != nullptr) return launch_cfg<PREC, 4, 2, 1, 1, 3, false, kVarDualBranch>(a, s);
+        }
+        return launch_cfg<PREC, 4, 2, 1, 1, 3, STEM, VAR>(a, s);
       case 13: return launch_cfg<PREC, 2, 4, 2, 1, 3, STEM, VAR>(a, s);
       case 14: return launch_cfg<PREC, 2, 4, 2, 1, 3, STEM, STEM ? VAR : kVarLoaderWaves>(a, s);
       case 15: return launch_cfg<PREC, 4, 2, 1, 1, 3, STEM, STEM ? VAR : kVarLoaderWaves>(a, s);
@@ -881,6 +978,8 @@
   if (precision != 2 && tile >= 14) return false;
   return Co % kTileCols[tile] == 0;
 }
+
+bool conv_tile_has_dual(int precision, int tile) { return precision == 2 && (tile == 17 || tile == 8 || tile == 10); }
 
 namespace {
 struct TileModel {
@@ -947,6 +1046,15 @@
   } else {
     if ((a.Ci * eb) % 128 != 0 || a.ksteps != a.KH * a.KW * (a.Ci * eb / 128)) return hipErrorInvalidValue;
   }
+  if (a.x2 != nullptr) {
+    if (precision != 2 || a.stem || a.res != nullptr || a.KH != 1 || a.KW != 1 || a.stride != 1 || a.pad != 0 || a.Hi != a.Ho ||
+        a.Wi != a.Wo || a.ksteps > 8 || a.M != a.N * a.Ho * a.Wo || a.w2 == nullptr || a.scale2 == nullptr || a.shift2 == nullptr ||
+        a.x2_bytes == 0 || a.x2_bytes >= kOutOfRange || a.w2_bytes == 0 || a.w2_bytes >= kOutOfRange || a.ksteps2 <= 0 ||
+        a.Ci2 * eb != a.ksteps2 * 128 || a.stride2 < 1 || a.Hi2 < 1 || a.Wi2 < 1 || (a.Ho - 1) * a.stride2 >= a.Hi2 ||
+        (a.Wo - 1) * a.stride2 >= a.Wi2 || (unsigned long long)a.N * a.Hi2 * a.Wi2 * a.Ci2 * eb != a.x2_bytes ||
+        (unsigned long long)a.Co * a.ksteps2 * 128 != a.w2_bytes || !conv_tile_has_dual(precision, tile))
+      return hipErrorInvalidValue;
+  }
   const int rows = (!a.stem && a.KW == a.KH && a.M == a.N * a.Ho * a.Wo)
                        ? conv_rows_kind(precision, a.KH, a.stride, a.pad, a.dil, a.Hi, a.Wi, a.Ho, a.Wo, a.Ci, a.Co, a.res != nullptr) : 0;
   if (tile < 0) tile = choose_conv_tile(a.M, a.Co, a.ksteps * (128 / eb), precision, rows);
diff --git a/neuralbarkcalculator_amd/csrc/nbc_api.hip b/neuralbarkcalculator_amd/csrc/nbc_api.hip
--- a/neuralbarkcalculator_amd/csrc/nbc_api.hip
+++ b/neuralbarkcalculator_amd/csrc/nbc_api.hip
@@ -42,6 +42,8 @@
   float* lowres = nullptr;
   size_t lowres_cap = 0;
   int conv_tile = -1;
+  bool fuse_downsample = true;
+  int fused_pairs = 0;
   bool keep = false;
   bool profiling = false;
   std::vector<std::vector<hipEvent_t>> prof_sets;
@@ -90,19 +92,30 @@
   cur = Plan();
 }
 
+bool downsample_pair(const nbc_ctx* c, const Plan& P, size_t l);
+
 int ensure_buffers(nbc_ctx* c) {
   const Plan& P = c->plan;
   if (c->bufs.size() < P.buf_bytes.size()) { c->bufs.resize(P.buf_bytes.size(), nullptr); c->buf_cap.resize(P.buf_bytes.size(), 0); }
+  std::vector<size_t> need(P.buf_bytes);
+  {
+    std::vector<int> group;
+    size_t most = 0;
+    for (size_t l = 0; l + 1 < P.ops.size(); ++l)
+      if (downsample_pair(c, P, l))
+        for (int b : {P.ops[l].out_buf, P.ops[l + 1].out_buf}) { group.push_back(b); most = std::max(most, need[b]); }
+    for (int b : group) need[b] = most;
+  }
   for (size_t i = 0; i < P.buf_bytes.size(); ++i) {
-    if (c->buf_cap[i] < P.buf_bytes[i]) {
+    if (c->buf_cap[i] < need[i]) {
       const size_t grown = c->buf_cap[i] + c->buf_cap[i] / 2;
       if (c->bufs[i]) NBC_HIP(hipFree(c->bufs[i]));
       c->bufs[i] = nullptr; c->buf_cap[i] = 0;
-      size_t want = std::max(P.buf_bytes[i], grown);
+      size_t want = std::max(need[i], grown);
       hipError_t e = hipMalloc(&c->bufs[i], want);
-      if (e != hipSuccess && want > P.buf_bytes[i]) {
+      if (e != hipSuccess && want > need[i]) {
         (void)hipGetLastError();
-        want = P.buf_bytes[i];
+        want = need[i];
         e = hipMalloc(&c->bufs[i], want);
       }
       if (e != hipSuccess) return set_error(NBC_ERR_NOMEM, std::string("hipMalloc(workspace): ") + hipGetErrorString(e));
@@ -146,7 +159,7 @@
           reinterpret_cast<const float*>(c->weights + pc.shift_off)};
 }
 
-int launch_conv_op(nbc_ctx* c, const Op& o, int N, int tile, hipStream_t s, hipError_t* err) {
+int launch_conv_op(nbc_ctx* c, const Op& o, int N, int tile, hipStream_t s, hipError_t* err, const Op* ds = nullptr) {
   const ConvUnit& u = conv_units(c->arch)[o.unit];
   const PackedConv& pc = c->layout.convs[o.unit];
   const UnitPtrs p = unit_ptrs(c, o.unit);
@@ -185,6 +198,25 @@
     return set_error(NBC_ERR_INVALID, "activation of " + o.name + " exceeds 2 GiB: lower the batch size");
   a.x_bytes = (unsigned)xb;
   a.w_bytes = (unsigned)wbts;
+  if (ds) {
+    const ConvUnit& u2 = conv_units(c->arch)[ds->unit];
+    const PackedConv& pc2 = c->layout.convs[ds->unit];
+    const UnitPtrs p2 = unit_ptrs(c, ds->unit);
+    const size_t xb2 = (size_t)N * ds->Hi * ds->Wi * ds->Ci * eb;
+    const size_t wb2 = (size_t)ds->Co * pc2.ksteps * kKStepBytes;
+    if (ds->Ci != pc2.cin_pad) return set_error(NBC_ERR_STATE, "plan/channel mismatch at " + ds->name);
+    if (xb2 >= 0x80000000ull || wb2 >= 0x80000000ull)
+      return set_error(NBC_ERR_INVALID, "activation of " + ds->name + " exceeds 2 GiB: lower the batch size");
+    a.res = nullptr;
+    a.y = c->bufs[ds->out_buf];
+    a.x2 = c->bufs[ds->in_buf];
+    a.w2 = p2.w;
+    a.scale2 = p2.scale;
+    a.shift2 = p2.shift;
+    a.x2_bytes = (unsigned)xb2;
+    a.w2_bytes = (unsigned)wb2;
+    a.Ci2 = ds->Ci; a.Hi2 = ds->Hi; a.Wi2 = ds->Wi; a.stride2 = u2.stride; a.ksteps2 = pc2.ksteps;
+  }
   if (o.gate_buf >= 0) {
     const size_t xi = (size_t)o.Hi * o.Wi * o.Ci * eb, yi = (size_t)o.Ho * o.Wo * o.Co * eb;
     a.N = 1;
@@ -202,6 +234,28 @@
   }
   *err = launch_conv_dma(a, prec, tile, s);
   return NBC_OK;
+}
+
+bool downsample_pair(const nbc_ctx* c, const Plan& P, size_t l) {
+  if (c->precision != NBC_PREC_F16X2 || P.bn != NBC_BN_RUNNING || P.keep || l + 1 >= P.ops.size()) return false;
+  const Op& d = P.ops[l];
+  const Op& o = P.ops[l + 1];
+  if (d.kind != OP_CONV || o.kind != OP_CONV || d.raw || o.raw || d.gate_buf >= 0 || o.gate_buf >= 0) return false;
+  if (d.res_buf >= 0 || o.res_buf < 0 || o.res_buf != d.out_buf || o.rows != 0 || d.rows != 0) return false;
+  if (d.out_buf == d.in_buf || d.out_buf == o.in_buf || d.out_buf == o.out_buf) return false;
+  const auto& units = conv_units(c->arch);
+  const ConvUnit& ud = units[d.unit];
+  const ConvUnit& uo = units[o.unit];
+  static const std::string kSuffix = ".downsample.0";
+  if (ud.name.size() <= kSuffix.size() || ud.name.compare(ud.name.size() - kSuffix.size(), kSuffix.size(), kSuffix) != 0) return false;
+  if (ud.k != 1 || ud.pad != 0 || ud.relu || uo.k != 1 || uo.stride != 1 || uo.pad != 0) return false;
+  if (d.Ho != o.Ho || d.Wo != o.Wo || d.Co != o.Co || o.Hi != o.Ho || o.Wi != o.Wo) return false;
+  const PackedConv& pd = c->layout.convs[d.unit];
+  const PackedConv& po = c->layout.convs[o.unit];
+  return !pd.stem && !po.stem && po.ksteps <= 8;
+}
+bool fusable_downsample(const nbc_ctx* c, const Plan& P, size_t l, int tile3) {
+  return c->fuse_downsample && !c->profiling && downsample_pair(c, P, l) && conv_tile_has_dual(c->precision, tile3);
 }
 
 const char* kernel_name(OpKind k) {
@@ -455,6 +509,17 @@
   return NBC_OK;
 }
 
+int nbc_set_fuse_downsample(nbc_ctx* c, int on) {
+  if (!c) return set_error(NBC_ERR_INVALID, "null context");
+  c->fuse_downsample = on != 0;
+  return NBC_OK;
+}
+
+int nbc_fused_pairs(nbc_ctx* c) {
+  if (!c) return set_error(NBC_ERR_INVALID, "null context");
+  return c->fused_pairs;
+}
+
 int nbc_set_keep_activations(nbc_ctx* c, int on) {
   if (!c) return set_error(NBC_ERR_INVALID, "null context");
   if (c->keep != (on != 0)) stash_plan(c);
@@ -557,6 +622,7 @@
   }
   float* lowres = logits_lowres_dev ? logits_lowres_dev : c->lowres;
 
+  c->fused_pairs = 0;
   if (evs) NBC_HIP(hipEventRecord((*evs)[0], s));
   for (size_t l = 0; l < nops; ++l) {
     const Op& o = P.ops[l];
@@ -570,10 +636,19 @@
           e = launch_ingest_u8(static_cast<const uint8_t*>(x_dev), c->bufs[o.out_buf], N, H, W, c->mean, c->stdv, prec, s);
         break;
       case OP_CONV: {
-        int tile = c->conv_tile;
-        if (!conv_tile_ok(prec, tile, o.Co, o.rows)) tile = o.tile;
-        rc = launch_conv_op(c, o, N, tile, s, &e);
+        const auto tile_of = [&](const Op& q) {
+          return conv_tile_ok(prec, c->conv_tile, q.Co, q.rows) ? c->conv_tile : q.tile;
+        };
+        if (l + 1 < nops && P.ops[l + 1].kind == OP_CONV && fusable_downsample(c, P, l, tile_of(P.ops[l + 1])))
+          break;
+        const Op* ds = l > 0 && fusable_downsample(c, P, l - 1, tile_of(o)) ? &P.ops[l - 1] : nullptr;
+        rc = launch_conv_op(c, o, N, tile_of(o), s, &e, ds);
         if (rc != NBC_OK) return rc;
+        if (ds && e == hipSuccess) {
+          ++c->fused_pairs;
+          std::swap(c->bufs[o.out_buf], c->bufs[ds->out_buf]);
+          std::swap(c->buf_cap[o.out_buf], c->buf_cap[ds->out_buf]);
+        }
         break;
       }
       case OP_MAXPOOL:
diff --git a/neuralbarkcalculator_amd/csrc/nbc_kernels.hpp b/neuralbarkcalculator_amd/csrc/nbc_kernels.hpp
--- a/neuralbarkcalculator_amd/csrc/nbc_kernels.hpp
+++ b/neuralbarkcalculator_amd/csrc/nbc_kernels.hpp
@@ -23,6 +23,12 @@
   int stem;
   int wo_shift;
   int hw_shift;
+  const void* x2;
+  const void* w2;
+  const float* scale2;
+  const float* shift2;
+  unsigned x2_bytes, w2_bytes;
+  int Ci2, Hi2, Wi2, stride2, ksteps2;
 #ifdef NBC_STAMPS
   unsigned long long* stamps;
 #endif
@@ -34,6 +40,7 @@
 int conv_tile_cols(int tile);
 int conv_rows_kind(int precision, int k, int stride, int pad, int dil, int Hi, int Wi, int Ho, int Wo, int Ci, int Co, bool has_res);
 bool conv_tile_ok(int precision, int tile, int Co, int rows_kind);
+bool conv_tile_has_dual(int precision, int tile);
 int choose_conv_tile(int M, int Co, int K, int precision, int rows_kind);
 hipError_t launch_conv_dma(const ConvArgs& a, int precision, int tile, hipStream_t s);
 hipError_t launch_conv3x3_rows(const ConvArgs& a, int rows_tile, hipStream_t s);
diff --git a/neuralbarkcalculator_amd/model.py b/neuralbarkcalculator_amd/model.py
--- a/neuralbarkcalculator_amd/model.py
+++ b/neuralbarkcalculator_amd/model.py
@@ -464,6 +464,15 @@
         with self._on_stream() as cur:
             _lib.check(self._lib.nbc_nonfinite_peek_async(self._require_ctx(), host_word.data_ptr(), cur.cuda_stream), "nbc_nonfinite_peek_async")
 
+    def set_fuse_downsample(self, on: bool = True):
+        _lib.check(self._lib.nbc_set_fuse_downsample(self._require_ctx(), int(on)), "nbc_set_fuse_downsample")
+
+    def fused_pairs(self) -> int:
+        n = self._lib.nbc_fused_pairs(self._require_ctx())
+        if n < 0:
+            _lib.check(n, "nbc_fused_pairs")
+        return int(n)
+
     def set_conv_tile(self, tile: int = -1):
         _lib.check(self._lib.nbc_set_conv_tile(self._require_ctx(), int(tile)), "nbc_set_conv_tile")
 
```

New measurement: 345.5 (median of 6 runs). 1.02x the previous value.
